# Fanchuana/OPUS-PLLM

Measured on AMD Instinct MI355X. Metric: proteins_per_sec, higher is better.
Workload: dtype f16; 1 GPU; OPUS-PLLM-llama3_8b shape: batch 64/GPU, 512-residue proteins, 89-id prompt (+8 protein tokens = 96 positions), 32 new tokens, greedy (BASELINE configs[3] per-GPU shard: batch 512 over 8 GPUs); batch_per_gpu=64, residues=512, parallelism=replicas x1 (batch-sharded), all-gather of ids

## Files before the change

include/opus_pllm.h:

```cpp
#ifndef OPUS_PLLM_H
#define OPUS_PLLM_H

#include <stdint.h>

#ifdef __cplusplus
extern "C" {
#endif

#define OPUS_ABI_VERSION 10

enum opus_status {
    OPUS_OK = 0,
    OPUS_EBADARG = -1,
    OPUS_ESHAPE = -2,
    OPUS_EHIP = -3,
    OPUS_ERCCL = -4,
    OPUS_EUNSUPPORTED = -5,
    OPUS_ESTATE = -6
};

enum opus_dtype { OPUS_F16 = 0, OPUS_F32 = 1, OPUS_I32 = 2, OPUS_I64 = 3, OPUS_U8 = 4, OPUS_F8E4M3 = 5, OPUS_I8 = 6,
                  OPUS_F4E2M1X2 = 7, OPUS_E8M0 = 8 };

typedef struct opus_config {
// ... 56 lines not shown

int opus_llama_forward(opus_ctx *ctx, const void *d_embeds, const uint8_t *d_mask, int32_t B, int32_t T, const int32_t *d_rows,
                       int32_t R, const int32_t *d_targets, float *d_logprob, void *d_logits, void *d_scratch,
                       int64_t scratch_bytes, void *stream);
int64_t opus_llama_forward_scratch_bytes(const opus_config *cfg, int32_t R, int32_t with_logits);
int opus_llama_prefix(opus_ctx *ctx, const void *d_embeds, const uint8_t *d_mask, int32_t B, int32_t T, float *d_last_logits,
                      float *d_last_rows, int64_t *epoch, void *stream);
int opus_llama_score_continuations(opus_ctx *ctx, const void *d_embeds, int32_t R, int32_t n, const int32_t *h_lens,
                                   const int32_t *h_src, const float *d_last_rows, int32_t P, int64_t epoch,
                                   const int32_t *d_targets, float *d_logprob, void *d_scratch, int64_t scratch_bytes, void *stream);
int64_t opus_llama_score_scratch_bytes(const opus_config *cfg, int32_t R, int32_t n);
int opus_debug_attn_prefix(opus_ctx *ctx, const void *d_qkv, const void *d_k_hist, const void *d_v_hist, const int32_t *d_kstart,
                           int32_t P, int32_t Tp, int32_t R, int32_t n, const int32_t *h_src, void *d_out, void *stream);
int opus_llama_score_tree(opus_ctx *ctx, const void *d_embeds, int32_t rows, const int32_t *h_src, const int32_t *h_par,
                          const int32_t *h_depth, int32_t n_score, const int32_t *h_score_src, int32_t n_edges,
                          const int32_t *h_edge_row, const int32_t *h_edge_tok, const int32_t *h_edge_slot, int32_t n_stops,
                          const int32_t *h_stop_row, const int32_t *h_stop_set, const int32_t *h_stop_slot, int32_t n_stop_ids,
                          const int32_t *h_stop_ids, int32_t n_stop_sets, const int32_t *h_stop_off, const float *d_last_rows,
                          int32_t P, int64_t epoch, float *d_node_lp, float *d_stop_lp, int64_t n_slots, void *d_scratch,
                          int64_t scratch_bytes, void *stream);
int64_t opus_llama_score_tree_scratch_bytes(const opus_config *cfg, int32_t rows, int32_t n_score, int32_t n_edges, int32_t n_stops,
                                            int32_t n_stop_ids, int32_t n_stop_sets);
int64_t opus_llama_dec_rows_cap(const opus_config *cfg);
int32_t opus_llama_tree_max_depth(void);
int opus_trie_path_sums(opus_ctx *ctx, const float *d_node_lp, const int32_t *d_trie, const int32_t *d_par, const int32_t *d_depth,
                        const int32_t *d_member_node, int32_t P, int32_t M, int32_t ld_nodes, float *d_member_lp, void *stream);
int opus_debug_attn_tree(opus_ctx *ctx, const void *d_qkv, const void *d_k_hist, const void *d_v_hist, const int32_t *d_kstart,
                         int32_t P, int32_t Tp, int32_t R, const int32_t *h_src, const int32_t *h_par, const int32_t *h_depth,
                         void *d_out, void *stream);
int opus_esm2_contacts_packed(opus_ctx *ctx, const int32_t *d_tokens, const int32_t *h_cu, int32_t B, float *d_pooled, float *d_contacts,
                              void *d_scratch, int64_t scratch_bytes, void *stream);
int64_t opus_esm2_contacts_scratch_bytes(const opus_config *cfg, const int32_t *h_cu, int32_t B);
int opus_esm2_lm_head(opus_ctx *ctx, const int32_t *d_rows, int32_t R, int32_t log_softmax, float *d_out, void *stream);
int opus_debug_esm2_lm_head(opus_ctx *ctx, const float *d_hidden, int32_t R, int32_t log_softmax, float *d_out, void *stream);
int opus_debug_contacts(opus_ctx *ctx, const void *d_q, const void *d_k, int64_t ld, const int32_t *h_cu, int32_t B, int32_t heads,
                        int32_t head_dim, const float *d_w, float *d_A, float *d_rows, float *d_cols, void *d_scratch,
                        int64_t scratch_bytes, void *stream);
int opus_debug_xent(opus_ctx *ctx, const void *d_logits, int32_t R, int32_t V, const int32_t *d_targets, float *d_logprob,
                    float *d_lse, void *stream);

int opus_generate_greedy(opus_ctx *ctx, const void *d_embeds, const uint8_t *d_mask, int32_t B, int32_t T,
                         int32_t max_new, const int32_t *eos_ids, int32_t n_eos, int32_t pad_id,
                         int32_t *d_out_ids, int32_t *n_out, void *stream);

int opus_set_stop_sequence(opus_ctx *ctx, const int32_t *ids, int32_t n);

int opus_generate_sample(opus_ctx *ctx, const void *d_embeds, const uint8_t *d_mask, int32_t B, int32_t T,
                         int32_t max_new, const int32_t *eos_ids, int32_t n_eos, int32_t pad_id, float temperature,
                         float top_p, uint64_t seed, int32_t *d_out_ids, int32_t *n_out, void *stream);
int opus_debug_sample(opus_ctx *ctx, const float *d_logits, int32_t B, float temperature, float top_p, uint64_t seed,
                      int32_t step, int32_t *d_tokens, void *stream);

int opus_generate_scored(opus_ctx *ctx, const void *d_embeds, const uint8_t *d_mask, int32_t B, int32_t T, int32_t max_new,
                         const int32_t *eos_ids, int32_t n_eos, int32_t pad_id, float temperature, float top_p, uint64_t seed,
                         int32_t *d_out_ids, int32_t *n_out, float *d_token_logprobs, float *d_scores, float *d_logits,
                         void *stream);
int opus_generate_scored_fanout(opus_ctx *ctx, const void *d_embeds, const uint8_t *d_mask, int32_t B, int32_t T, int32_t nret,
                                int32_t max_new, const int32_t *eos_ids, int32_t n_eos, int32_t pad_id, float temperature,
                                float top_p, uint64_t seed, int32_t *d_out_ids, int32_t *n_out, float *d_token_logprobs,
                                float *d_scores, float *d_logits, void *stream);

int opus_generate_scored_guided(opus_ctx *ctx, const void *d_embeds, const uint8_t *d_mask, int32_t P, int32_t T, float guidance_scale,
                                int32_t max_new, const int32_t *eos_ids, int32_t n_eos, int32_t pad_id, float temperature,
                                float top_p, uint64_t seed, int32_t *d_out_ids, int32_t *n_out, float *d_token_logprobs,
                                float *d_scores, float *d_logits, void *stream);

typedef struct opus_prefix_snap {
    const void *d_k, *d_v;
    const int32_t *d_kstart, *h_kstart;
    int32_t P, Tp;
} opus_prefix_snap;
int64_t opus_llama_prefix_bytes(const opus_config *cfg, int32_t P, int32_t Tp);
int opus_llama_prefix_export(opus_ctx *ctx, int64_t epoch, int32_t R, int32_t T, void *d_k, void *d_v, int32_t *d_kstart, void *stream);
int opus_llama_prefill_behind(opus_ctx *ctx, const opus_prefix_snap *snap, const void *d_embeds, int32_t R, int32_t n,
                              const int32_t *h_lens, const int32_t *h_src, float *d_last_logits, int64_t *epoch, void *stream);
int opus_generate_scored_behind(opus_ctx *ctx, const opus_prefix_snap *snap, const void *d_embeds, int32_t R, int32_t n,
                                const int32_t *h_lens, const int32_t *h_src, int32_t max_new, const int32_t *eos_ids, int32_t n_eos,
                                int32_t pad_id, float temperature, float top_p, uint64_t seed, int32_t *d_out_ids, int32_t *n_out,
                                float *d_token_logprobs, float *d_scores, float *d_logits, void *stream);
int opus_llama_score_continuations_detached(opus_ctx *ctx, const opus_prefix_snap *snap, const void *d_embeds, int32_t R, int32_t n,
                                            const int32_t *h_lens, const int32_t *h_src, const float *d_last_rows,
                                            const int32_t *d_targets, float *d_logprob, void *d_scratch, int64_t scratch_bytes,
                                            void *stream);
int opus_llama_score_tree_detached(opus_ctx *ctx, const opus_prefix_snap *snap, const void *d_embeds, int32_t rows,
                                   const int32_t *h_src, const int32_t *h_par, const int32_t *h_depth, int32_t n_score,
                                   const int32_t *h_score_src, int32_t n_edges, const int32_t *h_edge_row, const int32_t *h_edge_tok,
                                   const int32_t *h_edge_slot, int32_t n_stops, const int32_t *h_stop_row, const int32_t *h_stop_set,
                                   const int32_t *h_stop_slot, int32_t n_stop_ids, const int32_t *h_stop_ids, int32_t n_stop_sets,
                                   const int32_t *h_stop_off, const float *d_last_rows, float *d_node_lp, float *d_stop_lp,
                                   int64_t n_slots, void *d_scratch, int64_t scratch_bytes, void *stream);

int opus_generate_lookup(opus_ctx *ctx, const void *d_embeds, const uint8_t *d_mask, int32_t B, int32_t T, int32_t max_new,
                         const int32_t *eos_ids, int32_t n_eos, int32_t pad_id, int32_t k, int32_t max_ngram, const int32_t *d_hist,
                         int32_t Lh, const int32_t *h_hist_len, int32_t *d_out_ids, int32_t *n_out, int64_t *stats, void *stream);
int opus_llama_verify_step(opus_ctx *ctx, const int32_t *d_tokens, int32_t n, const int32_t *d_draft_len, float *d_logits_all,
                           int32_t *d_argmax, int32_t *a, void *stream);
int opus_debug_lookup_draft(opus_ctx *ctx, const int32_t *d_hist, int32_t Lh, const int32_t *d_hist_len, int32_t R, int32_t k,
                            int32_t max_ngram, int32_t *d_draft, int32_t *d_draft_len, void *stream);
int opus_debug_last_qkv(opus_ctx *ctx, void *d_out, int32_t rows, void *stream);
int opus_debug_lookup_accept(opus_ctx *ctx, const int32_t *d_argmax, const int32_t *d_tokens, const int32_t *d_draft_len, int32_t R,
                             int32_t n, int32_t pre, int32_t *d_ids, int32_t stride, int32_t *d_fin, int32_t *d_step,
                             const int32_t *eos_ids, int32_t n_eos, int32_t pad_id, const int32_t *stop_ids, int32_t n_stop,
                             int32_t *d_next, int32_t *d_nunf, int32_t *h_words, void *stream);

int opus_debug_argmax_lse(opus_ctx *ctx, const float *d_logits, int32_t B, int32_t V, int32_t *d_idx, float *d_lse, void *stream);
int opus_debug_guidance(opus_ctx *ctx, float *d_logits, int32_t P, int32_t V, float guidance_scale, void *stream);

int opus_set_logits_processors(opus_ctx *ctx, float repetition_penalty, int32_t no_repeat_ngram_size, int32_t min_new_tokens,
                               const int32_t *bad_ids, const int32_t *bad_offsets, int32_t n_bad);
int opus_debug_logits_process(opus_ctx *ctx, float *d_logits, int32_t B, int32_t V, const int32_t *d_hist, int32_t hist_stride,
                              int32_t hist_len, const int32_t *eos_ids, int32_t n_eos, float repetition_penalty,
                              int32_t no_repeat_ngram_size, int32_t min_new_tokens, const int32_t *bad_ids,
                              const int32_t *bad_offsets, int32_t n_bad, void *stream);

int opus_set_token_constraint(opus_ctx *ctx, int32_t n_states, const int32_t *edge_off, const int32_t *edge_tok,
                              const int32_t *edge_next, int32_t n_edges, const uint8_t *completing, const int32_t *end_ids,
                              int32_t n_end, const int32_t *start, int32_t n_start, void *stream);
int opus_debug_token_constraint(opus_ctx *ctx, float *d_logits, int32_t B, int32_t V, const int32_t *d_hist, int32_t hist_stride,
                                int32_t hist_len, int32_t *d_state_out, void *stream);

int opus_debug_gemm(opus_ctx *ctx, const void *d_A, const void *d_W, const float *d_bias, const float *d_residual,
                    void *d_C, int32_t M, int32_t N, int32_t K, int32_t epi, int32_t out_f32, void *stream);
int opus_debug_gemm_norm(opus_ctx *ctx, const float *d_A, const void *d_W, void *d_C, int32_t M, int32_t N, int32_t K,
                         int32_t epi, int32_t out_f32, float eps, void *stream);
int opus_debug_gemm_slabs(opus_ctx *ctx, const void *d_A, const void *d_W, float *d_slabs, int32_t M, int32_t N, int32_t K,
                          int32_t *ks, void *stream);
int opus_debug_gemm_plan(opus_ctx *ctx, int32_t *plan);
int opus_debug_gemm_w8(opus_ctx *ctx, int32_t form, const void *d_A, const void *d_W, const void *d_q8, const void *d_e8,
                       const float *d_bias, const float *d_residual, void *d_C, int32_t M, int32_t N, int32_t K, int32_t epi,
                       int32_t out_f32, float eps, int32_t *ks, int32_t *ran_w8, void *stream);
int opus_debug_gemm_w4(opus_ctx *ctx, int32_t form, const void *d_A, const void *d_W, const void *d_q4, const void *d_s4,
                       const float *d_bias, const float *d_residual, void *d_C, int32_t M, int32_t N, int32_t K, int32_t epi,
                       int32_t out_f32, float eps, int32_t *ks, int32_t *ran_w4, void *stream);
int opus_debug_knob(opus_ctx *ctx, const char *name, int32_t value);
int opus_debug_gemm_rowscale(opus_ctx *ctx, const void *d_A, const void *d_W1, float *d_X, const void *d_W2, void *d_C,
                             int32_t M, int32_t N1, int32_t K1, int32_t N2, int32_t epi, float eps, int32_t *fused,
                             void *stream);
int opus_debug_gemm_rope(opus_ctx *ctx, const void *d_A, const void *d_W, const float *d_bias, void *d_out, int32_t M,
                         int32_t D, int32_t K, int32_t T, int32_t heads, int32_t allow_fuse, int32_t *fused, void *stream);
int opus_debug_gemm_ln(opus_ctx *ctx, const void *d_A, const void *d_W1, const float *d_b1, float *d_X, float *d_part, void *d_xh,
                       float *d_stat, const void *d_W2, const float *d_c2, const float *d_colsum, void *d_C, int32_t M, int32_t N1,
                       int32_t K1, int32_t N2, int32_t epi, int32_t rms, float eps, int32_t rope_T, const int32_t *d_rope_pos,
                       int32_t *produced, int32_t *plan, void *stream);
int opus_debug_attention(opus_ctx *ctx, const void *d_Q, const void *d_K, const void *d_V, void *d_O,
                         const int32_t *d_kstart, const int32_t *d_kend, int32_t B, int32_t T, int32_t heads,
                         int32_t group, int32_t head_dim, int32_t causal, float scale, void *stream);

int opus_debug_attn_prefill(opus_ctx *ctx, const void *d_Q, const void *d_K, const void *d_V, void *d_O, int64_t q_st, int64_t k_st,
                            int64_t v_st, int64_t o_st, int64_t q_sb, int64_t k_sb, int64_t v_sb, int64_t o_sb,
                            const int32_t *d_kstart, const int32_t *d_kend, const int32_t *d_cu, int32_t B, int32_t T,
                            int32_t heads, int32_t group, int32_t head_dim, int32_t causal, int32_t q_trim, float scale,
                            int32_t *qt_used, void *stream);

int opus_debug_attn_decode(opus_ctx *ctx, const void *d_qkv, const void *d_k_hist, const void *d_v_hist, const int32_t *d_kstart,
                           int32_t B, int32_t T0, int32_t step, void *d_out, void *d_k_new, void *d_v_new, void *stream);

int opus_debug_attn_decode_form(opus_ctx *ctx, const void *d_qkv, const float *d_slabs, int32_t ks, const float *d_row_ssq,
                                int32_t row_nblk, int32_t K, float eps, const float *d_bias, const void *d_k_hist,
                                const void *d_v_hist, const int32_t *d_kstart, int32_t B, int32_t T0, int32_t step,
                                int32_t out_tiled, void *d_out, void *d_k_new, void *d_v_new, void *d_k_cache, void *d_v_cache,
                                int32_t *gp_used, void *stream);

int opus_check_error(opus_ctx *ctx, void *stream);

int opus_beam_topk(opus_ctx *ctx, const float *d_run_scores, int32_t B, int32_t K, int32_t M, float *d_scores, int32_t *d_idx,
                   void *stream);
int opus_kv_reorder(opus_ctx *ctx, const int32_t *d_src_rows, int32_t R, void *stream);
int opus_beam_sample_topk(opus_ctx *ctx, const float *d_logits, const float *d_run_scores, int32_t B, int32_t K, int32_t M,
                          float temperature, float top_p, uint64_t seed, int32_t step, float *d_scores, int32_t *d_idx, void *stream);
int opus_set_sampling_top_k(opus_ctx *ctx, int32_t k);

int32_t opus_stream_lag(void);
int opus_stream_begin(opus_ctx *ctx, const void *d_embeds, const uint8_t *d_mask, int32_t B, int32_t T, int32_t max_new,
                      const int32_t *eos_ids, int32_t n_eos, int32_t pad_id, float temperature, float top_p, uint64_t seed,
                      int32_t *d_ids, void *stream);
int opus_stream_run(opus_ctx *ctx, int32_t t_min, int32_t min_free, int32_t t_max, int32_t *t_out, int32_t *h_end, void *stream);
int opus_stream_refill(opus_ctx *ctx, const opus_prefix_snap *snap, int32_t n, const int32_t *h_rows, const int32_t *h_src,
                       const float *d_last_logits, const int32_t *h_len, void *stream);
int opus_stream_end(opus_ctx *ctx, int32_t *h_end, void *stream);
int opus_debug_stream_state(opus_ctx *ctx, int32_t *h_kstart, int32_t *h_fin, int32_t *h_start, int32_t *h_end, int64_t *epoch,
                            int32_t poison, void *stream);

int opus_last_logits(opus_ctx *ctx, float *d_out, int32_t B, void *stream);

int64_t opus_stat(opus_ctx *ctx, const char *name);

int opus_timing_enable(opus_ctx *ctx, int32_t on);
int opus_timing_reset(opus_ctx *ctx);
int opus_timing_get(opus_ctx *ctx, const char *kernel_class, const char *phase, double *ms, int64_t *launches, double *bytes,
                    double *flops);
int opus_timing_names(char *buf, int32_t cap);

#ifdef __cplusplus
}
#endif
#endif
```

opus-pllm_amd/_cabi.py:

```python
from __future__ import annotations

import ctypes as C
import os
from typing import Optional

from .config import OpusConfig

_HERE = os.path.dirname(os.path.abspath(__file__))
BF16 = os.environ.get("OPUS_DTYPE", "fp16").lower() in ("bf16", "bfloat16")
LIB_PATH = os.environ.get("OPUS_LIB_PATH") or os.path.join(_HERE, "lib", "libopus_pllm_bf16.so" if BF16 else "libopus_pllm.so")
ABI_VERSION = 10

OPUS_F16, OPUS_F32, OPUS_I32, OPUS_I64, OPUS_U8 = 0, 1, 2, 3, 4
OPUS_F8E4M3, OPUS_I8 = 5, 6
OPUS_F4E2M1X2, OPUS_E8M0 = 7, 8


def operand_dtype():
    import torch
    return torch.bfloat16 if BF16 else torch.float16


class OpusError(RuntimeError):
    def __init__(self, code: int, msg: str):
        super().__init__(f"libopus_pllm error {code}: {msg}")
        self.code = code


class CConfig(C.Structure):
    _fields_ = [
        ("enc_layers", C.c_int32), ("enc_dim", C.c_int32), ("enc_heads", C.c_int32), ("enc_ffn", C.c_int32),
        ("enc_vocab", C.c_int32), ("enc_ln_eps", C.c_float), ("enc_rope_theta", C.c_float),
        ("has_protein_projector", C.c_int32), ("proj_dim", C.c_int32), ("n_prot_tokens", C.c_int32),
        ("switch_depth", C.c_int32),
        ("dec_layers", C.c_int32), ("dec_dim", C.c_int32), ("dec_heads", C.c_int32), ("dec_kv_heads", C.c_int32),
        ("dec_head_dim", C.c_int32), ("dec_ffn", C.c_int32), ("dec_vocab", C.c_int32),
        ("dec_rms_eps", C.c_float), ("dec_rope_theta", C.c_float),
        ("max_batch", C.c_int32), ("max_enc_tokens", C.c_int32), ("max_prompt", C.c_int32),
        ("max_new_tokens", C.c_int32),
        ("dec_arch", C.c_int32), ("dec_qkv_bias", C.c_int32), ("dec_act", C.c_int32), ("dec_max_pos", C.c_int32),
    ]

    @classmethod
    def from_config(cls, cfg: OpusConfig) -> "CConfig":
        return cls(**{name: getattr(cfg, name) for name, _ in cls._fields_})


_P = C.c_void_p


class CPrefixSnap(C.Structure):
    _fields_ = [("d_k", _P), ("d_v", _P), ("d_kstart", _P), ("h_kstart", C.POINTER(C.c_int32)), ("P", C.c_int32), ("Tp", C.c_int32)]


_SNAP = C.POINTER(CPrefixSnap)
_I32P = C.POINTER(C.c_int32)
SIGNATURES = {
    "opus_llama_prefix_bytes": (C.c_int64, [C.POINTER(CConfig), C.c_int32, C.c_int32]),
    "opus_llama_prefix_export": (C.c_int, [_P, C.c_int64, C.c_int32, C.c_int32, _P, _P, _P, _P]),
    "opus_llama_prefill_behind": (C.c_int, [_P, _SNAP, _P, C.c_int32, C.c_int32, _I32P, _I32P, _P, C.POINTER(C.c_int64), _P]),
    "opus_generate_scored_behind": (C.c_int, [_P, _SNAP, _P, C.c_int32, C.c_int32, _I32P, _I32P, C.c_int32, _I32P, C.c_int32, C.c_int32,
                                              C.c_float, C.c_float, C.c_uint64, _P, _I32P, _P, _P, _P, _P]),
    "opus_llama_score_continuations_detached": (C.c_int, [_P, _SNAP, _P, C.c_int32, C.c_int32, _P, _P, _P, _P, _P, _P, C.c_int64, _P]),
    "opus_llama_score_tree_detached": (C.c_int, [_P, _SNAP, _P, C.c_int32, _P, _P, _P, C.c_int32, _P, C.c_int32, _P, _P, _P, C.c_int32, _P,
                                                 _P, _P, C.c_int32, _P, C.c_int32, _P, _P, _P, _P, C.c_int64, _P, C.c_int64, _P]),
    "opus_generate_lookup": (C.c_int, [_P, _P, _P, C.c_int32, C.c_int32, C.c_int32, _I32P, C.c_int32, C.c_int32, C.c_int32, C.c_int32, _P,
                                       C.c_int32, _I32P, _P, _I32P, C.POINTER(C.c_int64), _P]),
    "opus_llama_verify_step": (C.c_int, [_P, _P, C.c_int32, _P, _P, _P, _I32P, _P]),
    "opus_debug_last_qkv": (C.c_int, [_P, _P, C.c_int32, _P]),
    "opus_debug_lookup_draft": (C.c_int, [_P, _P, C.c_int32, _P, C.c_int32, C.c_int32, C.c_int32, _P, _P, _P]),
    "opus_debug_lookup_accept": (C.c_int, [_P, _P, _P, _P, C.c_int32, C.c_int32, C.c_int32, _P, C.c_int32, _P, _P, _I32P, C.c_int32,
                                           C.c_int32, _I32P, C.c_int32, _P, _P, _I32P, _P]),
    "opus_stream_lag": (C.c_int32, []),
    "opus_stream_begin": (C.c_int, [_P, _P, _P, C.c_int32, C.c_int32, C.c_int32, _I32P, C.c_int32, C.c_int32, C.c_float, C.c_float,
                                    C.c_uint64, _P, _P]),
    "opus_stream_run": (C.c_int, [_P, C.c_int32, C.c_int32, C.c_int32, _I32P, _I32P, _P]),
    "opus_stream_refill": (C.c_int, [_P, _SNAP, C.c_int32, _I32P, _I32P, _P, _I32P, _P]),
    "opus_stream_end": (C.c_int, [_P, _I32P, _P]),
    "opus_debug_stream_state": (C.c_int, [_P, _I32P, _I32P, _I32P, _I32P, C.POINTER(C.c_int64), C.c_int32, _P]),
    "opus_abi_version": (C.c_int, []),
    "opus_operand_dtype": (C.c_int, []),
    "opus_last_error": (C.c_char_p, []),
    "opus_workspace_bytes": (C.c_int64, [C.POINTER(CConfig)]),
    "opus_ctx_create": (C.c_int, [C.POINTER(CConfig), C.c_int, C.POINTER(_P)]),
    "opus_ctx_destroy": (C.c_int, [_P]),
    "opus_bind_weight": (C.c_int, [_P, C.c_char_p, _P, C.c_int, C.c_int, C.POINTER(C.c_int64)]),
    "opus_weights_ready": (C.c_int, [_P]),
    "opus_lora_merge": (C.c_int, [_P, _P, _P, C.c_float, C.c_int64, C.c_int64, C.c_int32, _P]),
    "opus_fill_synth": (C.c_int, [_P, C.c_int, C.c_int64, C.c_int64, C.c_uint64, C.c_float, C.c_float,
                                  C.c_int64, C.c_int64, C.c_int64, C.c_int32, C.c_uint64, C.c_float, C.c_float, _P]),
    "opus_tile_weight": (C.c_int, [_P, _P, C.c_int64, C.c_int64, _P]),
    "opus_quantize_fp8": (C.c_int, [_P, C.c_int64, C.c_int64, _P, _P, _P, _P]),
    "opus_debug_gemm_w8": (C.c_int, [_P, C.c_int32, _P, _P, _P, _P, _P, _P, _P, C.c_int32, C.c_int32, C.c_int32, C.c_int32, C.c_int32,
                                     C.c_float, C.POINTER(C.c_int32), C.POINTER(C.c_int32), _P]),
    "opus_quantize_mxfp4": (C.c_int, [_P, C.c_int64, C.c_int64, _P, _P, _P, _P]),
    "opus_debug_gemm_w4": (C.c_int, [_P, C.c_int32, _P, _P, _P, _P, _P, _P, _P, C.c_int32, C.c_int32, C.c_int32, C.c_int32, C.c_int32,
                                     C.c_float, C.POINTER(C.c_int32), C.POINTER(C.c_int32), _P]),
    "opus_esm2_encode": (C.c_int, [_P, _P, _P, C.c_int32, C.c_int32, _P, _P]),
    "opus_esm2_encode_packed": (C.c_int, [_P, _P, C.POINTER(C.c_int32), C.c_int32, _P, _P]),
    "opus_esm2_last_hidden": (C.c_int, [_P, _P, C.c_int32, C.c_int32, _P]),
    "opus_projector_forward": (C.c_int, [_P, _P, C.c_int32, _P, _P, _P]),
    "opus_protein_projector": (C.c_int, [_P, _P, C.c_int32, _P, _P]),
    "opus_switch_projector": (C.c_int, [_P, _P, C.c_int32, _P, _P]),
    "opus_splice_pad": (C.c_int, [_P, _P, _P, C.c_int32, C.c_int32, _P, C.c_int32, C.c_int32, C.c_int32,
                                  _P, _P, _P, C.POINTER(C.c_int32), _P]),
    "opus_llama_prefill": (C.c_int, [_P, _P, _P, C.c_int32, C.c_int32, _P, _P]),
    "opus_llama_decode_step": (C.c_int, [_P, _P, _P, _P]),
    "opus_generate_greedy": (C.c_int, [_P, _P, _P, C.c_int32, C.c_int32, C.c_int32, C.POINTER(C.c_int32),
                                       C.c_int32, C.c_int32, _P, C.POINTER(C.c_int32), _P]),
    "opus_debug_gemm": (C.c_int, [_P, _P, _P, _P, _P, _P, C.c_int32, C.c_int32, C.c_int32, C.c_int32, C.c_int32, _P]),
    "opus_debug_gemm_norm": (C.c_int, [_P, _P, _P, _P, C.c_int32, C.c_int32, C.c_int32, C.c_int32, C.c_int32, C.c_float, _P]),
    "opus_debug_gemm_rope": (C.c_int, [_P, _P, _P, _P, _P, C.c_int32, C.c_int32, C.c_int32, C.c_int32, C.c_int32, C.c_int32, _P, _P]),
    "opus_debug_attention": (C.c_int, [_P, _P, _P, _P, _P, _P, _P, C.c_int32, C.c_int32, C.c_int32, C.c_int32,
                                       C.c_int32, C.c_int32, C.c_float, _P]),
    "opus_debug_attn_prefill": (C.c_int, [_P, _P, _P, _P, _P, C.c_int64, C.c_int64, C.c_int64, C.c_int64, C.c_int64, C.c_int64,
                                          C.c_int64, C.c_int64, _P, _P, _P, C.c_int32, C.c_int32, C.c_int32, C.c_int32, C.c_int32,
                                          C.c_int32, C.c_int32, C.c_float, C.POINTER(C.c_int32), _P]),
    "opus_generate_sample": (C.c_int, [_P, _P, _P, C.c_int32, C.c_int32, C.c_int32, C.POINTER(C.c_int32), C.c_int32, C.c_int32,
                                       C.c_float, C.c_float, C.c_uint64, _P, C.POINTER(C.c_int32), _P]),
    "opus_debug_sample": (C.c_int, [_P, _P, C.c_int32, C.c_float, C.c_float, C.c_uint64, C.c_int32, _P, _P]),
    "opus_timing_enable": (C.c_int, [_P, C.c_int32]),
    "opus_timing_reset": (C.c_int, [_P]),
    "opus_timing_get": (C.c_int, [_P, C.c_char_p, C.c_char_p, C.POINTER(C.c_double), C.POINTER(C.c_int64),
                                  C.POINTER(C.c_double), C.POINTER(C.c_double)]),
    "opus_timing_names": (C.c_int, [C.c_char_p, C.c_int32]),
    "opus_last_logits": (C.c_int, [_P, _P, C.c_int32, _P]),
    "opus_check_error": (C.c_int, [_P, _P]),
    "opus_beam_topk": (C.c_int, [_P, _P, C.c_int32, C.c_int32, C.c_int32, _P, _P, _P]),
    "opus_kv_reorder": (C.c_int, [_P, _P, C.c_int32, _P]),
    "opus_beam_sample_topk": (C.c_int, [_P, _P, _P, C.c_int32, C.c_int32, C.c_int32, C.c_float, C.c_float, C.c_uint64, C.c_int32,
                                        _P, _P, _P]),
    "opus_set_sampling_top_k": (C.c_int, [_P, C.c_int32]),
    "opus_set_stop_sequence": (C.c_int, [_P, C.POINTER(C.c_int32), C.c_int32]),
    "opus_debug_gemm_slabs": (C.c_int, [_P, _P, _P, _P, C.c_int32, C.c_int32, C.c_int32, C.POINTER(C.c_int32), _P]),
    "opus_debug_gemm_plan": (C.c_int, [_P, C.POINTER(C.c_int32)]),
    "opus_debug_knob": (C.c_int, [_P, C.c_char_p, C.c_int32]),
    "opus_stat": (C.c_int64, [_P, C.c_char_p]),
    "opus_debug_attn_decode": (C.c_int, [_P, _P, _P, _P, _P, C.c_int32, C.c_int32, C.c_int32, _P, _P, _P, _P]),
    "opus_debug_attn_decode_form": (C.c_int, [_P, _P, _P, C.c_int32, _P, C.c_int32, C.c_int32, C.c_float, _P, _P, _P, _P, C.c_int32,
                                              C.c_int32, C.c_int32, C.c_int32, _P, _P, _P, _P, _P, C.POINTER(C.c_int32), _P]),
    "opus_llama_forward": (C.c_int, [_P, _P, _P, C.c_int32, C.c_int32, _P, C.c_int32, _P, _P, _P, _P, C.c_int64, _P]),
    "opus_llama_forward_scratch_bytes": (C.c_int64, [C.POINTER(CConfig), C.c_int32, C.c_int32]),
    "opus_llama_prefix": (C.c_int, [_P, _P, _P, C.c_int32, C.c_int32, _P, _P, C.POINTER(C.c_int64), _P]),
    "opus_llama_score_continuations": (C.c_int, [_P, _P, C.c_int32, C.c_int32, _P, _P, _P, C.c_int32, C.c_int64, _P, _P, _P,
                                                 C.c_int64, _P]),
    "opus_llama_score_scratch_bytes": (C.c_int64, [C.POINTER(CConfig), C.c_int32, C.c_int32]),
    "opus_debug_attn_prefix": (C.c_int, [_P, _P, _P, _P, _P, C.c_int32, C.c_int32, C.c_int32, C.c_int32, _P, _P, _P]),
    "opus_llama_score_tree": (C.c_int, [_P, _P, C.c_int32, _P, _P, _P, C.c_int32, _P, C.c_int32, _P, _P, _P, C.c_int32, _P, _P, _P,
                                        C.c_int32, _P, C.c_int32, _P, _P, C.c_int32, C.c_int64, _P, _P, C.c_int64, _P, C.c_int64, _P]),
    "opus_llama_score_tree_scratch_bytes": (C.c_int64, [C.POINTER(CConfig), C.c_int32, C.c_int32, C.c_int32, C.c_int32, C.c_int32,
                                                        C.c_int32]),
    "opus_llama_dec_rows_cap": (C.c_int64, [C.POINTER(CConfig)]),
    "opus_llama_tree_max_depth": (C.c_int32, []),
    "opus_trie_path_sums": (C.c_int, [_P, _P, _P, _P, _P, _P, C.c_int32, C.c_int32, C.c_int32, _P, _P]),
    "opus_debug_attn_tree": (C.c_int, [_P, _P, _P, _P, _P, C.c_int32, C.c_int32, C.c_int32, _P, _P, _P, _P, _P]),
    "opus_debug_xent": (C.c_int, [_P, _P, C.c_int32, C.c_int32, _P, _P, _P, _P]),
    "opus_esm2_contacts_packed": (C.c_int, [_P, _P, C.POINTER(C.c_int32), C.c_int32, _P, _P, _P, C.c_int64, _P]),
    "opus_esm2_contacts_scratch_bytes": (C.c_int64, [C.POINTER(CConfig), C.POINTER(C.c_int32), C.c_int32]),
    "opus_debug_contacts": (C.c_int, [_P, _P, _P, C.c_int64, C.POINTER(C.c_int32), C.c_int32, C.c_int32, C.c_int32, _P, _P, _P, _P,
                                      _P, C.c_int64, _P]),
    "opus_esm2_lm_head": (C.c_int, [_P, _P, C.c_int32, C.c_int32, _P, _P]),
    "opus_debug_esm2_lm_head": (C.c_int, [_P, _P, C.c_int32, C.c_int32, _P, _P]),
    "opus_generate_scored": (C.c_int, [_P, _P, _P, C.c_int32, C.c_int32, C.c_int32, C.POINTER(C.c_int32), C.c_int32, C.c_int32,
                                       C.c_float, C.c_float, C.c_uint64, _P, C.POINTER(C.c_int32), _P, _P, _P, _P]),
    "opus_llama_prefill_fanout": (C.c_int, [_P, _P, _P, C.c_int32, C.c_int32, C.c_int32, _P, _P]),
    "opus_generate_scored_fanout": (C.c_int, [_P, _P, _P, C.c_int32, C.c_int32, C.c_int32, C.c_int32, C.POINTER(C.c_int32), C.c_int32,
                                              C.c_int32, C.c_float, C.c_float, C.c_uint64, _P, C.POINTER(C.c_int32), _P, _P, _P, _P]),
    "opus_debug_argmax_lse": (C.c_int, [_P, _P, C.c_int32, C.c_int32, _P, _P, _P]),
    "opus_generate_scored_guided": (C.c_int, [_P, _P, _P, C.c_int32, C.c_int32, C.c_float, C.c_int32, C.POINTER(C.c_int32), C.c_int32,
                                              C.c_int32, C.c_float, C.c_float, C.c_uint64, _P, C.POINTER(C.c_int32), _P, _P, _P, _P]),
    "opus_debug_guidance": (C.c_int, [_P, _P, C.c_int32, C.c_int32, C.c_float, _P]),
    "opus_set_logits_processors": (C.c_int, [_P, C.c_float, C.c_int32, C.c_int32, C.POINTER(C.c_int32), C.POINTER(C.c_int32),
                                             C.c_int32]),
    "opus_debug_logits_process": (C.c_int, [_P, _P, C.c_int32, C.c_int32, _P, C.c_int32, C.c_int32, C.POINTER(C.c_int32), C.c_int32,
                                            C.c_float, C.c_int32, C.c_int32, C.POINTER(C.c_int32), C.POINTER(C.c_int32), C.c_int32,
                                            _P]),
    "opus_set_token_constraint": (C.c_int, [_P, C.c_int32, _P, _P, _P, C.c_int32, _P, _P, C.c_int32, _P, C.c_int32, _P]),
    "opus_debug_token_constraint": (C.c_int, [_P, _P, C.c_int32, C.c_int32, _P, C.c_int32, C.c_int32, _P, _P]),
    "opus_debug_gemm_rowscale": (C.c_int, [_P, _P, _P, _P, _P, _P, C.c_int32, C.c_int32, C.c_int32, C.c_int32, C.c_int32,
                                           C.c_float, C.POINTER(C.c_int32), _P]),
    "opus_debug_gemm_ln": (C.c_int, [_P, _P, _P, _P, _P, _P, _P, _P, _P, _P, _P, _P, C.c_int32, C.c_int32, C.c_int32, C.c_int32,
                                     C.c_int32, C.c_int32, C.c_float, C.c_int32, _P, C.POINTER(C.c_int32), C.POINTER(C.c_int32), _P]),
}

_lib: Optional[C.CDLL] = None


def lib() -> C.CDLL:
    global _lib
    if _lib is not None:
        return _lib
    if not os.path.exists(LIB_PATH):
        raise OpusError(-100, f"{LIB_PATH} not found: build it with `python opus-pllm_amd/build.py` "
                              "(hipcc --offload-arch=gfx950); this package has no CPU fallback")
    l = C.CDLL(LIB_PATH)
    for name, (res, args) in SIGNATURES.items():
        fn = getattr(l, name)
        fn.restype = res
        fn.argtypes = args
    v = l.opus_abi_version()
    if v != ABI_VERSION:
        raise OpusError(-101, f"ABI version mismatch: library {v}, binding {ABI_VERSION}")
    if l.opus_operand_dtype() != (1 if BF16 else 0):
        raise OpusError(-102, f"{LIB_PATH} was not built for {'bf16' if BF16 else 'fp16'} operands")
    _lib = l
    return l


def check(code: int) -> None:
    if code != 0:
        raise OpusError(code, lib().opus_last_error().decode("utf-8", "replace"))
```

opus-pllm_amd/build.py:

```python
from __future__ import annotations

import concurrent.futures as cf
import os
import re
import subprocess
import sys

HERE = os.path.dirname(os.path.abspath(__file__))
SRC = os.path.join(HERE, "csrc")
OBJ = os.path.join(HERE, "build")
LIB = os.path.join(HERE, "lib", "libopus_pllm.so")
LIB_BF16 = os.path.join(HERE, "lib", "libopus_pllm_bf16.so")
SOURCES = ["gemm.hip", "gemm_stream.hip", "norm.hip", "elementwise.hip", "attn_prefill.hip", "attn_prefix.hip", "kv_place.hip", "stream.hip", "attn_decode.hip", "beam.hip", "score.hip", "contact.hip", "mlm.hip", "logits_proc.hip", "constraint.hip", "guidance.hip", "quant.hip", "lookup.hip", "api.cpp"]
HIPCC = os.environ.get("HIPCC", "/opt/rocm/bin/hipcc")
FLAGS = ["--offload-arch=gfx950", "-O3", "-fPIC", "-std=c++17", "-Wall", "-Wno-unused-function",
         "-Wno-unused-variable", "-Wno-unused-but-set-variable"]
EXTRA = {"attn_prefill.hip": ["-mllvm", "-amdgpu-mfma-vgpr-form", "-fno-honor-nans"],
         "attn_prefix.hip": ["-mllvm", "-amdgpu-mfma-vgpr-form", "-fno-honor-nans"],
         "attn_decode.hip": ["-mllvm", "-amdgpu-mfma-vgpr-form"]}


NO_SCRATCH = ("gemm_pp_kernel", "gemm_stream_kernel", "gemm_wide_kernel", "gemm_skinny_kernel", "attn_prefill_kernel",
              "attn_decode_kernel", "attn_prefix_kernel", "tree_path_sums_kernel", "beam_", "kv_export_kernel", "kv_place_kernel",
              "kv_append_kernel", "guidance_", "stream_finish_kernel", "stream_refill_kernel", "stream_reset_kernel")
RU_FLAG = "-Rpass-analysis=kernel-resource-usage"


def resource_usage(text: str) -> dict:
    out, cur = {}, None
    for line in text.splitlines():
        m = re.search(r"remark: Function Name: (\S+)", line)
        if m:
            cur = out.setdefault(m.group(1), {})
            continue
        m = re.search(r"remark:\s+([\w \[\]/]+?): (-?\d+)", line)
        if m and cur is not None:
            cur[m.group(1).strip()] = int(m.group(2))
    return out


def check_resources(ru_file: str) -> None:
    bad = []
    for name, f in resource_usage(open(ru_file).read()).items():
        if any(k in name for k in NO_SCRATCH) and (f.get("ScratchSize [bytes/lane]", 0) or f.get("VGPRs Spill", 0) or f.get("SGPRs Spill", 0)):
            bad.append(f"{name}: VGPRs {f.get('VGPRs')}, scratch {f.get('ScratchSize [bytes/lane]')} B/lane, "
                       f"spilled VGPRs {f.get('VGPRs Spill')}, spilled SGPRs {f.get('SGPRs Spill')}")
    if bad:
        raise RuntimeError(f"{os.path.basename(ru_file)}: hot kernels must not spill:\n  " + "\n  ".join(bad))


def sources_sha16() -> str:
    import hashlib
    h = hashlib.sha256()
    files = sorted(os.path.join(SRC, f) for f in os.listdir(SRC) if f.endswith((".hip", ".cpp", ".h")))
    files.append(os.path.join(os.path.dirname(HERE), "include", "opus_pllm.h"))
    for f in files:
        h.update(os.path.basename(f).encode() + b"\0")
        h.update(open(f, "rb").read())
    return h.hexdigest()[:16]


def _deps_mtime() -> float:
    hdrs = [os.path.join(SRC, f) for f in os.listdir(SRC) if f.endswith(".h")]
    hdrs.append(os.path.join(os.path.dirname(HERE), "include", "opus_pllm.h"))
    return max(os.path.getmtime(h) for h in hdrs)


def _compile(src: str, force: bool, bf16: bool = False) -> str:
    obj = os.path.join(OBJ, src + (".bf16.o" if bf16 else ".o"))
    path = os.path.join(SRC, src)
    ru = obj + ".ru.txt"
    if not force and os.path.exists(obj) and os.path.exists(ru) and \
            os.path.getmtime(obj) > max(os.path.getmtime(path), _deps_mtime(), os.path.getmtime(os.path.abspath(__file__))):
        check_resources(ru)
        return obj
    cmd = [HIPCC] + FLAGS + [RU_FLAG] + EXTRA.get(src, []) + (["-DOPUS_BF16"] if bf16 else []) + \
          (["-x", "hip"] if src.endswith(".cpp") else []) + ["-c", path, "-o", obj]
    r = subprocess.run(cmd, capture_output=True, text=True)
    if r.returncode != 0:
        raise RuntimeError(f"hipcc failed on {src}:\n{r.stdout}\n{r.stderr}")
    remarks = [l for l in r.stderr.splitlines() if RU_FLAG in l]
    rest = "\n".join(l for l in r.stderr.splitlines() if RU_FLAG not in l)
    with open(ru, "w") as f:
        f.write("\n".join(remarks) + "\n")
    if rest.strip():
        sys.stderr.write(rest + "\n")
    check_resources(ru)
    return obj


def build(force: bool = False, verbose: bool = True) -> str:
    os.makedirs(OBJ, exist_ok=True)
    os.makedirs(os.path.dirname(LIB), exist_ok=True)
    jobs = [(s, b) for b in (False, True) for s in SOURCES]
    with cf.ThreadPoolExecutor(max_workers=6) as ex:
        objs = list(ex.map(lambda j: _compile(j[0], force, j[1]), jobs))
    for lib, mine in ((LIB, objs[:len(SOURCES)]), (LIB_BF16, objs[len(SOURCES):])):
        if force or not os.path.exists(lib) or any(os.path.getmtime(o) > os.path.getmtime(lib) for o in mine):
            r = subprocess.run([HIPCC, "--offload-arch=gfx950", "-shared", "-fPIC", "-o", lib] + mine, capture_output=True, text=True)
            if r.returncode != 0:
                raise RuntimeError(f"link failed:\n{r.stdout}\n{r.stderr}")
        if verbose:
            print(f"built {lib} ({os.path.getsize(lib) / 1e6:.2f} MB)")
    return LIB


LIB_ASAN = os.path.join(HERE, "lib", "libopus_pllm_asan.so")
ASAN_RT = "/opt/rocm/lib/llvm/lib/clang/22/lib/linux/libclang_rt.asan-x86_64.so"


def build_asan(verbose: bool = True) -> str:
    build(verbose=False)
    obj = os.path.join(OBJ, "api.cpp.asan.o")
    src = os.path.join(SRC, "api.cpp")
    if not os.path.exists(obj) or os.path.getmtime(obj) < max(os.path.getmtime(src), _deps_mtime()):
        cmd = [HIPCC, "--offload-arch=gfx950", "-O1", "-g", "-fPIC", "-std=c++17", "-fsanitize=address", "-fno-gpu-sanitize",
               "-shared-libsan", "-fno-omit-frame-pointer", "-x", "hip", "-c", src, "-o", obj]
        r = subprocess.run(cmd, capture_output=True, text=True)
        if r.returncode != 0:
            raise RuntimeError(f"hipcc (asan) failed on api.cpp:\n{r.stdout}\n{r.stderr}")
    objs = [os.path.join(OBJ, s + ".o") for s in SOURCES if s != "api.cpp"] + [obj]
    if not os.path.exists(LIB_ASAN) or any(os.path.getmtime(o) > os.path.getmtime(LIB_ASAN) for o in objs):
        r = subprocess.run([HIPCC, "--offload-arch=gfx950", "-shared", "-fPIC", "-fsanitize=address", "-fno-gpu-sanitize",
                            "-shared-libsan", "-o", LIB_ASAN] + objs, capture_output=True, text=True)
        if r.returncode != 0:
            raise RuntimeError(f"link (asan) failed:\n{r.stdout}\n{r.stderr}")
    if verbose:
        print(f"built {LIB_ASAN} ({os.path.getsize(LIB_ASAN) / 1e6:.2f} MB); run under LD_PRELOAD={ASAN_RT}")
    return LIB_ASAN


if __name__ == "__main__":
    if "--asan" in sys.argv:
        build_asan()
    else:
        build(force="--force" in sys.argv)
```

opus-pllm_amd/csrc/api.cpp:

```cpp
#include "../../include/opus_pllm.h"
#include "common.h"

#include <cmath>
#include <cstdarg>
#include <cstdio>
#include <cstdlib>
#include <cstring>
#include <algorithm>
#include <atomic>
#include <map>
#include <string>
#include <vector>

using namespace opus;

static thread_local char g_err[512] = "";
static int fail(int code, const char *fmt, ...) {
    va_list ap;
    va_start(ap, fmt);
    vsnprintf(g_err, sizeof(g_err), fmt, ap);
    va_end(ap);
    return code;
}
#define HIPC(expr)                                                                                   \
// ... 1069 lines not shown
}

static int switch_projector_rows(opus_ctx *c, hipStream_t s, const half_t *in, int B, half_t *d_out) {
    const opus_config &g = c->cfg;
    const int SW = g.dec_dim * g.n_prot_tokens;
    int din = g.has_protein_projector ? g.proj_dim : g.enc_dim;
    for (int i = 0; i < g.switch_depth; ++i) {
        const bool last = i + 1 == g.switch_depth;
        half_t *o = last ? d_out : c->p_z[i & 1];
        OPC(gemm(c, s, in, din, c->sw_w[i], B, SW, din, c->sw_b[i], last ? EPI_NONE : EPI_GELU, nullptr, o, SW, 0));
        in = o;
        din = SW;
    }
    return OPUS_OK;
}

extern "C" int opus_protein_projector(opus_ctx *c, const float *d_pooled, int32_t B, void *d_out, void *stream) {
    OPC(need_ready(c));
    if (!d_pooled || !d_out) return fail(OPUS_EBADARG, "protein_projector: null pointer");
    if (B < 1) return fail(OPUS_ESHAPE, "protein_projector: B=%d", B);
    const opus_config &g = c->cfg;
    const int64_t din = g.enc_dim, dout = g.has_protein_projector ? g.proj_dim : g.enc_dim;
    c->phase = PH_PROJECT;
    OPC(ensure_proj_rows(c, B));
    for (int r0 = 0; r0 < B; r0 += c->proj_rows) {
        const int n = B - r0 < c->proj_rows ? B - r0 : c->proj_rows;
        OPC(protein_projector_rows(c, (hipStream_t)stream, d_pooled + r0 * din, n, (half_t *)d_out + r0 * dout));
    }
    return OPUS_OK;
}

extern "C" int opus_switch_projector(opus_ctx *c, const void *d_in, int32_t B, void *d_out, void *stream) {
    OPC(need_ready(c));
    if (!d_in || !d_out) return fail(OPUS_EBADARG, "switch_projector: null pointer");
    if (B < 1) return fail(OPUS_ESHAPE, "switch_projector: B=%d", B);
    const opus_config &g = c->cfg;
    const int64_t din = g.has_protein_projector ? g.proj_dim : g.enc_dim, SW = (int64_t)g.dec_dim * g.n_prot_tokens;
    c->phase = PH_PROJECT;
    OPC(ensure_proj_rows(c, B));
    for (int r0 = 0; r0 < B; r0 += c->proj_rows) {
        const int n = B - r0 < c->proj_rows ? B - r0 : c->proj_rows;
        OPC(switch_projector_rows(c, (hipStream_t)stream, (const half_t *)d_in + r0 * din, n, (half_t *)d_out + r0 * SW));
    }
    return OPUS_OK;
}

extern "C" int opus_projector_forward(opus_ctx *c, const float *d_pooled, int32_t B, void *d_out, void *d_proj_out,
                                      void *stream) {
    OPC(need_ready(c));
    if (!d_pooled || !d_out) return fail(OPUS_EBADARG, "projector_forward: null pointer");
    if (B < 1) return fail(OPUS_ESHAPE, "projector_forward: B=%d", B);
    const opus_config &g = c->cfg;
    hipStream_t s = (hipStream_t)stream;
    const int64_t din = g.enc_dim, dmid = g.has_protein_projector ? g.proj_dim : g.enc_dim, SW = (int64_t)g.dec_dim * g.n_prot_tokens;
    c->phase = PH_PROJECT;
    OPC(ensure_proj_rows(c, B));
    for (int r0 = 0; r0 < B; r0 += c->proj_rows) {
        const int n = B - r0 < c->proj_rows ? B - r0 : c->proj_rows;
        OPC(protein_projector_rows(c, s, d_pooled + r0 * din, n, c->p_y));
        if (d_proj_out)
            HIPC(hipMemcpyAsync((half_t *)d_proj_out + r0 * dmid, c->p_y, (size_t)n * dmid * sizeof(half_t), hipMemcpyDeviceToDevice, s));
        OPC(switch_projector_rows(c, s, c->p_y, n, (half_t *)d_out + r0 * SW));
    }
    return OPUS_OK;
}

extern "C" int opus_splice_pad(opus_ctx *c, const int64_t *d_ids, const uint8_t *d_mask, int32_t B, int32_t Tt,
                               const void *d_prot, int32_t n_prot, int32_t inference_mode, int32_t max_length,
                               void *d_embeds, uint8_t *d_mask_out, int32_t *d_pos_out, int32_t *T_out, void *stream) {
    OPC(need_ready(c));
    if (!d_ids || !d_prot || !d_embeds || !d_mask_out || !d_pos_out || !T_out) return fail(OPUS_EBADARG, "splice_pad: null pointer");
    const opus_config &g = c->cfg;
    if (B < 1 || B > g.max_batch || Tt < 1) return fail(OPUS_ESHAPE, "splice_pad: B=%d T_text=%d out of range", B, Tt);
    hipStream_t s = (hipStream_t)stream;
    c->phase = PH_SPLICE;
    KL(KC_OTHER, 9.0 * B * Tt, launch_splice_plan(d_ids, d_mask, B, Tt, g.n_prot_tokens, max_length, g.dec_vocab, c->d_plan, s));
    int32_t tail[3];
    HIPC(hipMemcpyAsync(tail, c->d_plan + 4 * B, sizeof(tail), hipMemcpyDeviceToHost, s));
    HIPC(hipStreamSynchronize(s));
    if (tail[2]) return fail(OPUS_EBADARG, "splice_pad: token id outside [0, vocab) (and not -200)");
    if (tail[1] > n_prot) return fail(OPUS_ESHAPE, "splice_pad: rows consume %d protein blocks, %d supplied", tail[1], n_prot);
    if (tail[0] > g.max_prompt) return fail(OPUS_ESHAPE, "splice_pad: spliced length %d exceeds max_prompt=%d", tail[0], g.max_prompt);
    if (tail[0] < 1) return fail(OPUS_ESHAPE, "splice_pad: every row is empty");
    *T_out = tail[0];
    KL(KC_OTHER, 2.0 * B * tail[0] * g.dec_dim * 2,
       launch_splice_fill(d_ids, d_mask, B, Tt, (const half_t *)d_prot, g.n_prot_tokens, g.dec_dim, g.dec_vocab, c->dec_emb,
                          c->d_plan, tail[0], inference_mode ? 1 : 0, (half_t *)d_embeds, d_mask_out, d_pos_out, s));
    return OPUS_OK;
}

static int lm_head(opus_ctx *c, hipStream_t s, ResidShadow &sh, int B, float *out = nullptr) {
    const opus_config &g = c->cfg;
    return gemm_norm(c, s, sh, c->d_xl, g.dec_rms_eps, c->d_xln, c->lm_head, B, g.dec_vocab, g.dec_dim, EPI_NONE, out ? out : c->d_logits,
                     g.dec_vocab, 1);
}

static int fanout_rows(opus_ctx *c, hipStream_t s, int B, int nret) {
    const opus_config &g = c->cfg;
    KL(KC_OTHER, 4.0 * (B + B * nret) * g.dec_vocab, launch_row_fanout(c->d_probs, c->d_logits, g.dec_vocab, B, nret, c->d_kstart, s));
    return OPUS_OK;
}


static int reset_step(opus_ctx *c, hipStream_t s, int T0, int step = 0) {
    const int32_t v[2] = {step, T0};
    HIPC(launch_upload_i32(v, 2, c->d_step, s));
    return OPUS_OK;
}

template <class Head>
static int finish_prefill(opus_ctx *c, hipStream_t s, int B, int T, int nret, bool have_last, Head head) {
    const int H = c->cfg.dec_dim;
    if (!have_last) KL(KC_OTHER, 8.0 * B * H, launch_take_last(c->d_x, B, T, H, c->d_xl, s));
    OPC(head(nret > 1 ? c->d_probs : nullptr));
    if (nret > 1) OPC(fanout_rows(c, s, B, nret));
    OPC(reset_step(c, s, T));
    c->cur_B = B * nret;
    c->cur_T = T;
    c->prefilled = true;
    return OPUS_OK;
}

static int attn_decode(opus_ctx *c, hipStream_t s, const ResidShadow &sh, int l, int B, int T, int slab_ks = 0, const float *bias = nullptr,
                       int out_tiled = 0) {
    const opus_config &g = c->cfg;
    AttnDecodeParams a;
    a.qkv = c->d_qkv; a.slabs = nullptr; a.ks = 0; a.slab_stride = 0; a.row_ssq = nullptr; a.row_nblk = 0; a.eps = 0.f; a.K = 0;
    a.bias = nullptr;
    if (slab_ks > 0) {
        const int64_t QKVd = (int64_t)(g.dec_heads + 2 * g.dec_kv_heads) * g.dec_head_dim;
        a.qkv = nullptr; a.slabs = c->gemm_ws; a.ks = slab_ks; a.slab_stride = (int64_t)B * QKVd;
        a.row_ssq = c->d_ssq; a.row_nblk = sh.ssq_nblk; a.eps = g.dec_rms_eps; a.K = g.dec_dim; a.bias = bias;
    }
    a.cs_row = c->cs_row; a.kstart = c->d_kstart; a.step = c->d_step; a.T0 = -1; a.nh = g.dec_heads; a.nkv = g.dec_kv_heads;
    a.kc = c->kc + l * c->cache_sl; a.vc = c->vc + l * c->cache_sl; a.cache_sb = c->cache_sb; a.cache_sh = c->cache_sh;
    a.ctx_cap = g.max_prompt + g.max_new_tokens; a.scale = 1.0f / sqrtf((float)g.dec_head_dim); a.out = c->d_ctx;
    a.out_tiled = out_tiled;
    const double bytes = 4.0 * B * g.dec_kv_heads * g.dec_head_dim * (T + 1) + 2.0 * B * (2.0 * g.dec_heads + 2.0 * g.dec_kv_heads) * g.dec_head_dim;
    KL(KC_ATTN_DECODE, bytes, launch_attn_decode(a, B, g.dec_head_dim, s));
    return OPUS_OK;
}

static int attn_prefix(opus_ctx *c, hipStream_t s, const ContRows &cr, int l, int M) {
    const opus_config &g = c->cfg;
    AttnPrefixParams a = cr.attn;
    a.kc = cr.snap_k ? cr.snap_k + l * cr.snap_sl : c->kc + l * c->cache_sl;
    a.vc = cr.snap_v ? cr.snap_v + l * cr.snap_sl : c->vc + l * c->cache_sl;
    const int QKV = (g.dec_heads + 2 * g.dec_kv_heads) * g.dec_head_dim, QD = g.dec_heads * g.dec_head_dim;
    KLF(KC_ATTN_PREFILL, 2.0 * M * (QKV + QD) + 4.0 * cr.nblocks * g.dec_kv_heads * g.dec_head_dim * a.Tp,
        4.0 * M * (double)QD * (a.Tp + a.n), launch_attn_prefix(a, cr.nblocks, s));
    return OPUS_OK;
}

static int attn_prefill(opus_ctx *c, hipStream_t s, int l, int B, int T, const ContRows *cont, int nret) {
    const opus_config &g = c->cfg;
    const int nh = g.dec_heads, nkv = g.dec_kv_heads, hd = g.dec_head_dim, QKV = (nh + 2 * nkv) * hd, QD = nh * hd, M = B * T;
    if (cont) {
        KL(KC_OTHER, 4.0 * M * QKV, launch_dec_rope_cache(c->d_qkv, c->cs_dec, cont->nkst, B, T, nh, nkv, hd, nullptr, nullptr, 0, 0, s));
        if (cont->app_lens)
            KL(KC_OTHER, 8.0 * M * nkv * hd, launch_kv_append(c->d_qkv, cont->app_lens, B, T, nh, nkv, hd, cont->attn.Tp, c->kc + l * c->cache_sl,
                                                              c->vc + l * c->cache_sl, c->cache_sb, c->cache_sh, s));
        return attn_prefix(c, s, *cont, l, M);
    }
    KL(KC_OTHER, 4.0 * M * QKV,
       launch_dec_rope_cache(c->d_qkv, c->cs_dec, c->d_kstart, B, T, nh, nkv, hd, c->kc + l * c->cache_sl,
                             c->vc + l * c->cache_sl, c->cache_sb, c->cache_sh, s, nret));
    AttnParams a;
    a.Q = c->d_qkv; a.K = c->d_qkv + QD; a.V = c->d_qkv + QD + nkv * hd;
    a.q_sb = a.k_sb = a.v_sb = (int64_t)T * QKV;
    a.q_st = a.k_st = a.v_st = QKV;
    a.O = c->d_ctx; a.o_sb = (int64_t)T * QD; a.o_st = QD;
    a.kstart = c->d_kstart; a.kend = nullptr;
    a.B = B; a.T = T; a.heads = nh; a.group = nh / nkv; a.head_dim = hd; a.causal = 1;
    a.scale = 1.0f / sqrtf((float)hd);
    KLF(KC_ATTN_PREFILL, 2.0 * M * (QKV + QD), 2.0 * B * (double)T * T * QD, launch_attn_prefill(a, s));
    return OPUS_OK;
}

static int opt_layer(opus_ctx *c, hipStream_t s, const DecLayer &L, int l, float *x, half_t *xn, int M, int B, int T, bool decode,
                     const ContRows *cont = nullptr, int nret = 1) {
    const opus_config &g = c->cfg;
    const int H = g.dec_dim, F = g.dec_ffn;
    const int QKV = (g.dec_heads + 2 * g.dec_kv_heads) * g.dec_head_dim, QD = g.dec_heads * g.dec_head_dim;
    KL(KC_NORM, 6.0 * M * H, launch_layernorm(x, L.ln1w, L.ln1b, g.dec_rms_eps, M, H, xn, nullptr, s));
    OPC(gemm(c, s, xn, H, L.wqkv, M, QKV, H, L.bqkv, EPI_NONE, nullptr, c->d_qkv, QKV, 0));
    if (decode) OPC(attn_decode(c, s, ResidShadow(), l, B, T));
    else OPC(attn_prefill(c, s, l, B, T, cont, nret));
    OPC(gemm(c, s, c->d_ctx, QD, L.wo, M, H, QD, L.bo, EPI_NONE, x, x, H, 1));
    KL(KC_NORM, 6.0 * M * H, launch_layernorm(x, L.ln2w, L.ln2b, g.dec_rms_eps, M, H, xn, nullptr, s));
    if (g.dec_act == 0) {
        OPC(gemm(c, s, xn, H, L.w1, M, F, H, L.b1, EPI_GELU, nullptr, c->d_act, F, 0));
    } else {
        OPC(gemm(c, s, xn, H, L.w1, M, F, H, L.b1, EPI_NONE, nullptr, c->d_act, F, 0));
        KL(KC_OTHER, 4.0 * M * F, launch_relu_h(c->d_act, (int64_t)M * F, s));
    }
    OPC(gemm(c, s, c->d_act, F, L.w2, M, H, F, L.b2, EPI_NONE, x, x, H, 1));
    return OPUS_OK;
}

static int lm_head_opt(opus_ctx *c, hipStream_t s, int B, float *out = nullptr) {
    const opus_config &g = c->cfg;
    KL(KC_NORM, 6.0 * B * g.dec_dim, launch_layernorm(c->d_xl, c->dec_lnfw, c->dec_lnfb, g.dec_rms_eps, B, g.dec_dim, c->d_xln, nullptr, s));
    return gemm(c, s, c->d_xln, g.dec_dim, c->lm_head, B, g.dec_vocab, g.dec_dim, nullptr, EPI_NONE, nullptr, out ? out : c->d_logits,
                g.dec_vocab, 1);
}

static int prefill_opt(opus_ctx *c, hipStream_t s, const half_t *embeds, const uint8_t *mask, int B, int T, bool all_rows,
                       const ContRows *cont, int nret) {
    const opus_config &g = c->cfg;
    const int H = g.dec_dim, M = B * T;
    HIPC(hipMemsetAsync(c->d_cnt, 0, HANDOFF_ERR * sizeof(int32_t), s));
    if (!cont) KL(KC_OTHER, 1.0 * M, launch_mask_to_kstart(mask, B, T, c->d_kstart, s));
    KL(KC_OTHER, 6.0 * M * H, launch_h2f(embeds, c->d_x, (int64_t)M * H, s));
    KL(KC_OTHER, 10.0 * M * H, launch_add_pos(c->d_x, c->dec_pos, cont ? cont->nkst : c->d_kstart, nullptr, 0, B, T, H, g.dec_max_pos + 1, s));
    for (int l = 0; l < g.dec_layers; ++l) OPC(opt_layer(c, s, c->dec[l], l, c->d_x, c->d_xn, M, B, T, false, cont, nret));
    if (all_rows) return OPUS_OK;
    return finish_prefill(c, s, B, T, nret, false, [&](float *out) { return lm_head_opt(c, s, B, out); });
}

static int decode_step_opt(opus_ctx *c, hipStream_t s) {
    const opus_config &g = c->cfg;
    const int B = c->cur_B, T = c->cur_T, H = g.dec_dim;
    KL(KC_OTHER, 10.0 * B * H, launch_add_pos(c->d_xl, c->dec_pos, c->d_kstart, c->d_step, -1, B, 1, H, g.dec_max_pos + 1, s));
    for (int l = 0; l < g.dec_layers; ++l) OPC(opt_layer(c, s, c->dec[l], l, c->d_xl, c->d_xln, B, B, T, true));
    OPC(lm_head_opt(c, s, B));
    KL(KC_OTHER, 8.0, launch_step_advance(c->d_step, s));
    return OPUS_OK;
}

static int prefill(opus_ctx *c, hipStream_t s, const half_t *embeds, const uint8_t *mask, int B, int T, bool all_rows = false,
                   const ContRows *cont = nullptr, int nret = 1) {
    c->phase = cont && !cont->app_lens ? PH_SCORE : PH_PREFILL;
    if (cont && cont->w8) c->phase = PH_DECODE;
    if (cont) {
        all_rows = true;
    } else {
        new_epoch(c);
        if (all_rows) {
            c->prefilled = false;
            c->cur_B = 0;
        }
    }
    if (c->cfg.dec_arch == 1) return prefill_opt(c, s, embeds, mask, B, T, all_rows, cont, nret);
    const opus_config &g = c->cfg;
    const int H = g.dec_dim, F = g.dec_ffn, nh = g.dec_heads, nkv = g.dec_kv_heads, hd = g.dec_head_dim;
    const int QKV = (nh + 2 * nkv) * hd, QD = nh * hd;
    const int M = B * T;
    HIPC(hipMemsetAsync(c->d_cnt, 0, HANDOFF_ERR * sizeof(int32_t), s));
    if (!cont) KL(KC_OTHER, 1.0 * M, launch_mask_to_kstart(mask, B, T, c->d_kstart, s));
    KL(KC_OTHER, 6.0 * M * H, launch_h2f(embeds, c->d_x, (int64_t)M * H, s));
    static const bool no_ln_env = getenv("OPUS_NO_LN_FUSION") != nullptr;
    const bool no_ln_fusion = no_ln_env || g_knobs.no_ln_fusion;
    const bool qkv_pp = !no_ln_fusion && (H & 255) == 0 && (QKV & 255) == 0 && gemm_goes_pp(M, QKV);
    const bool gu_pp = !no_ln_fusion && (H & 255) == 0 && (F & 127) == 0 && gemm_goes_pp(M, 2 * F);
    bool have_stat = false, last_rows_done = false;
    auto finalize = [&]() -> int {
        KL(KC_NORM, 8.0 * M * (H / 64) + 8.0 * M, launch_ln_finalize(c->d_part, M, H / 64, H, g.dec_rms_eps, 1, c->d_stat, s));
        return OPUS_OK;
    };
    ResidShadow sh;
    GemmGot got;
    const bool w8 = cont && cont->w8;
    auto ask8 = [&](GemmAsk a, const uint8_t *q, const int8_t *e, const uint8_t *q4, const uint8_t *s4) { return w8 ? a.w8(q, e).w4(q4, s4) : a; };
    for (int l = 0; l < g.dec_layers; ++l) {
        const DecLayer &L = c->dec[l];
        if (have_stat && qkv_pp) {
            OPC(gemm(c, s, c->d_xn, H, L.wqkv, M, QKV, H, L.bqkv, EPI_NONE, nullptr, c->d_qkv, QKV, 0, GemmAsk().ln_consume(c->d_stat, nullptr)));
        } else {
            OPC(gemm_norm(c, s, sh, c->d_x, g.dec_rms_eps, c->d_xn, L.wqkv, M, QKV, H, EPI_NONE, c->d_qkv, QKV, 0, L.bqkv,
                          ask8(GemmAsk(), L.q8_qkv, L.e8_qkv, L.q4_qkv, L.s4_qkv)));
        }
        OPC(attn_prefill(c, s, l, B, T, cont, nret));
        if (l + 1 == g.dec_layers && T > 1 && !all_rows && !g_knobs.misc[7]) {
            half_t *ctx_last = c->d_qkv;
            KL(KC_OTHER, 4.0 * B * QD, launch_take_last(reinterpret_cast<const float *>(c->d_ctx), B, T, QD / 2, reinterpret_cast<float *>(ctx_last), s));
            KL(KC_OTHER, 8.0 * B * H, launch_take_last(c->d_x, B, T, H, c->d_xl, s));
            const GemmAsk copy_xl = GemmAsk().copy16(fuse_rows() && B <= 96 ? c->d_xln : nullptr);
            OPC(gemm(c, s, ctx_last, QD, L.wo, B, H, QD, nullptr, EPI_NONE, c->d_xl, c->d_xl, H, 1, copy_xl, &got));
            sh.produced(c->d_xl, got);
            OPC(gemm_norm(c, s, sh, c->d_xl, g.dec_rms_eps, c->d_xln, L.wgu, B, 2 * F, H, EPI_SILU_GU16, c->d_act, F, 0));
            OPC(gemm(c, s, c->d_act, F, L.wd, B, H, F, nullptr, EPI_NONE, c->d_xl, c->d_xl, H, 1, copy_xl, &got));
            sh.produced(c->d_xl, got);
            last_rows_done = true;
            break;
        }
        GemmAsk wo;
        if (gu_pp) wo.ln_produce(c->d_part, c->d_xn);
        else if (fuse_rows() && M <= 96) wo.copy16(c->d_xn);
        OPC(gemm(c, s, c->d_ctx, QD, L.wo, M, H, QD, nullptr, EPI_NONE, c->d_x, c->d_x, H, 1, ask8(wo, L.q8_o, L.e8_o, L.q4_o, L.s4_o), &got));
        sh.produced(c->d_x, got);
        have_stat = got.ln_done != 0;
        if (have_stat) {
            OPC(finalize());
            OPC(gemm(c, s, c->d_xn, H, L.wgu, M, 2 * F, H, nullptr, EPI_SILU_GU16, nullptr, c->d_act, F, 0, GemmAsk().ln_consume(c->d_stat, nullptr)));
        } else {
            OPC(gemm_norm(c, s, sh, c->d_x, g.dec_rms_eps, c->d_xn, L.wgu, M, 2 * F, H, EPI_SILU_GU16, c->d_act, F, 0, nullptr,
                          ask8(GemmAsk(), L.q8_gu, L.e8_gu, L.q4_gu, L.s4_gu)));
        }
        const bool next_pp = qkv_pp && l + 1 < g.dec_layers;
        OPC(gemm(c, s, c->d_act, F, L.wd, M, H, F, nullptr, EPI_NONE, c->d_x, c->d_x, H, 1, ask8(GemmAsk().ln_produce(next_pp ? c->d_part : nullptr, c->d_xn), L.q8_d, L.e8_d, L.q4_d, L.s4_d), &got));
        have_stat = got.ln_done != 0;
        if (have_stat) OPC(finalize());
    }
    if (all_rows) return OPUS_OK;
    return finish_prefill(c, s, B, T, nret, last_rows_done, [&](float *out) { return lm_head(c, s, sh, B, out); });
}

static int decode_step(opus_ctx *c, hipStream_t s, const int32_t *d_tok) {
    c->phase = PH_DECODE;
    const opus_config &g = c->cfg;
    const int B = c->cur_B, T = c->cur_T;
    const int H = g.dec_dim, F = g.dec_ffn, nh = g.dec_heads, nkv = g.dec_kv_heads, hd = g.dec_head_dim;
    const int QKV = (nh + 2 * nkv) * hd, QD = nh * hd;
    const int ctx_cap = g.max_prompt + g.max_new_tokens;
    const bool rowscale = g.dec_arch == 0 && fuse_rows() && B > SKINNY_MAX_M && B <= MID_MAX_M && (H & 255) == 0;
    const bool qkv_tiled = rowscale && gemm_stream_would(B, QKV, H, 1, 1, 1, c->gemm_ws_bytes);
    const bool wo_tiled = rowscale && gemm_stream_would(B, H, QD, 0, 1, 0, c->gemm_ws_bytes);
    const bool down_tiled = rowscale && (F & 63) == 0 && gemm_stream_would(B, H, F, 0, 1, 0, c->gemm_ws_bytes);
    KL(KC_OTHER, 6.0 * B * H, launch_embed_tokens(d_tok, c->dec_emb, B, H, g.dec_vocab, c->d_xl, rowscale ? c->d_xln : nullptr,
                                                  rowscale ? c->d_ssq : nullptr, qkv_tiled ? 1 : 0, c->cs_dec, c->d_kstart, c->d_step, -1,
                                                  hd / 2, c->cs_row, c->d_cnt, HANDOFF_ERR, s));
    if (g.dec_arch == 1) return decode_step_opt(c, s);
    ResidShadow sh;
    if (rowscale) { sh.xh_src = c->d_xl; sh.ssq_nblk = H >> 8; sh.xln_tiled = qkv_tiled; }
    GemmGot got;
    half_t *const copy_xl = fuse_rows() && B <= 96 ? c->d_xln : nullptr;
    for (int l = 0; l < g.dec_layers; ++l) {
        const DecLayer &L = c->dec[l];
        if (rowscale && sh.xh_src == c->d_xl) {
// ... 1894 lines not shown
        if (got.ks > 1 && Cp)
            HIPC(hipMemcpyAsync(Cp, c->gemm_ws, (size_t)got.ks * M * N * sizeof(float), hipMemcpyDeviceToDevice, s));
    }
    *ran_w8 = *ran;
    return OPUS_OK;
}
extern "C" int opus_debug_gemm_w8(opus_ctx *c, int32_t form, const void *A, const void *W, const void *q8, const void *e8,
                                  const float *bias, const float *residual, void *Cp, int32_t M, int32_t N, int32_t K, int32_t epi,
                                  int32_t out_f32, float eps, int32_t *ks, int32_t *ran_w8, void *stream) {
    if (!c || !A || !W || !q8 || !e8 || !ran_w8) return fail(OPUS_EBADARG, "debug_gemm_w8: null pointer");
    if (form < 0 || form > 2) return fail(OPUS_EBADARG, "debug_gemm_w8: form 0, 1 or 2");
    if ((((uintptr_t)q8) & 15) || (((uintptr_t)e8) & 3)) return fail(OPUS_EBADARG, "debug_gemm_w8: d_q8 must be 16-byte, d_e8 4-byte aligned");
    return debug_gemm_wq(c, form, A, W, GemmAsk().w8((const uint8_t *)q8, (const int8_t *)e8), &c->gemm_w8, bias, residual, Cp, M, N, K,
                         epi, out_f32, eps, ks, ran_w8, stream);
}
extern "C" int opus_debug_gemm_w4(opus_ctx *c, int32_t form, const void *A, const void *W, const void *q4, const void *s4,
                                  const float *bias, const float *residual, void *Cp, int32_t M, int32_t N, int32_t K, int32_t epi,
                                  int32_t out_f32, float eps, int32_t *ks, int32_t *ran_w4, void *stream) {
    if (!c || !A || !W || !q4 || !s4 || !ran_w4) return fail(OPUS_EBADARG, "debug_gemm_w4: null pointer");
    if (form < 0 || form > 2) return fail(OPUS_EBADARG, "debug_gemm_w4: form 0, 1 or 2");
    if ((((uintptr_t)q4) & 15) || (((uintptr_t)s4) & 15)) return fail(OPUS_EBADARG, "debug_gemm_w4: d_q4 and d_s4 must be 16-byte aligned");
    return debug_gemm_wq(c, form, A, W, GemmAsk().w4((const uint8_t *)q4, (const uint8_t *)s4), &c->gemm_w4, bias, residual, Cp, M, N, K,
                         epi, out_f32, eps, ks, ran_w4, stream);
}

extern "C" int opus_debug_gemm_plan(opus_ctx *c, int32_t *plan) {
    if (!c || !plan) return fail(OPUS_EBADARG, "debug_gemm_plan: null pointer");
    for (int i = 0; i < GEMM_PLAN_WORDS; ++i) plan[i] = c->gemm_plan[i];
    return OPUS_OK;
}

extern "C" int opus_beam_topk(opus_ctx *c, const float *d_run_scores, int32_t B, int32_t K, int32_t M, float *d_scores,
                              int32_t *d_idx, void *stream) {
    if (!c || !d_run_scores || !d_scores || !d_idx) return fail(OPUS_EBADARG, "beam_topk: null pointer");
    if (!c->prefilled) return fail(OPUS_ESTATE, "beam_topk before prefill");
    if (B < 1 || K < 1 || B * K != c->cur_B) return fail(OPUS_ESHAPE, "beam_topk: B=%d x K=%d rows, the last step had %d", B, K, c->cur_B);
    if (M < 1 || M > 16) return fail(OPUS_ESHAPE, "beam_topk: 1 <= M <= 16 candidates per row (got %d)", M);
    HIPC(hipSetDevice(c->device));
    hipStream_t s = (hipStream_t)stream;
    c->phase = PH_DECODE;
    KL(KC_OTHER, 12.0 * c->cur_B * c->cfg.dec_vocab,
       launch_beam_topk(c->d_logits, d_run_scores, B, K, c->cfg.dec_vocab, M, c->d_zpart, d_scores, d_idx, s));
    return OPUS_OK;
}

extern "C" int opus_beam_sample_topk(opus_ctx *c, const float *d_logits, const float *d_run_scores, int32_t B, int32_t K, int32_t M,
                                     float temperature, float top_p, uint64_t seed, int32_t step, float *d_scores, int32_t *d_idx,
                                     void *stream) {
    if (!c || !d_run_scores || !d_scores || !d_idx) return fail(OPUS_EBADARG, "beam_sample_topk: null pointer");
    if (!d_logits && !c->prefilled) return fail(OPUS_ESTATE, "beam_sample_topk before prefill");
    if (B < 1 || K < 1 || B * K > c->cfg.max_batch || (!d_logits && B * K != c->cur_B))
        return fail(OPUS_ESHAPE, "beam_sample_topk: B=%d x K=%d rows (the last step had %d, the context holds %d)", B, K, c->cur_B, c->cfg.max_batch);
    if (M < 1 || M > 16) return fail(OPUS_ESHAPE, "beam_sample_topk: 1 <= M <= 16 candidates per row (got %d)", M);
    if (!(temperature > 0.f) || top_p <= 0.f || top_p > 1.f) return fail(OPUS_EBADARG, "beam_sample_topk: temperature > 0, 0 < top_p <= 1");
    HIPC(hipSetDevice(c->device));
    hipStream_t s = (hipStream_t)stream;
    const float *lg = d_logits ? d_logits : c->d_logits;
    const int V = c->cfg.dec_vocab, R = B * K;
    c->phase = PH_DECODE;
    const int min_keep = M / K > 1 ? M / K : 1;
    const int top_k = c->samp_top_k > 0 && c->samp_top_k < min_keep ? min_keep : c->samp_top_k;
    KL(KC_OTHER, 4.0 * 4 * R * V,
       launch_sample_select(lg, R, V, temperature, top_p, top_k, nullptr, nullptr, c->d_pval, c->d_pidx, c->d_probs, c->d_cand_i,
                            c->d_cand_n, c->d_zpart, c->d_spart, nullptr, c->d_bthr, nullptr, nullptr, s));
    KL(KC_OTHER, 12.0 * R * V,
       launch_beam_sample(lg, d_run_scores, B, K, V, M, temperature, c->d_pval, c->d_bthr, min_keep, c->d_probs, c->d_cand_i, seed, step,
                          c->d_blse, d_scores, d_idx, s));
    return OPUS_OK;
}

extern "C" int opus_set_sampling_top_k(opus_ctx *c, int32_t k) {
    if (!c || k < 0) return fail(OPUS_EBADARG, "set_sampling_top_k: k >= 0");
    if (k != c->samp_top_k) drop_graphs(c);
    c->samp_top_k = k;
    return OPUS_OK;
}

extern "C" int opus_kv_reorder(opus_ctx *c, const int32_t *d_src_rows, int32_t R, void *stream) {
    if (!c || !d_src_rows) return fail(OPUS_EBADARG, "kv_reorder: null pointer");
    if (!c->prefilled || R != c->cur_B) return fail(OPUS_ESHAPE, "kv_reorder: R=%d but the last prefill had %d rows", R, c->prefilled ? c->cur_B : 0);
    HIPC(hipSetDevice(c->device));
    hipStream_t s = (hipStream_t)stream;
    const opus_config &g = c->cfg;
    const size_t row = (size_t)c->cache_sb, layer = row * g.max_batch;
    if (!c->kv_tmp) HIPC(hipMalloc((void **)&c->kv_tmp, 2 * layer * sizeof(half_t)));
    c->phase = PH_DECODE;
    new_epoch(c);
    const int nkv = g.dec_kv_heads, hd = g.dec_head_dim, T0 = c->cur_T;
    for (int l = 0; l < g.dec_layers; ++l) {
        half_t *kc = c->kc + l * c->cache_sl, *vc = c->vc + l * c->cache_sl;
        KL(KC_OTHER, 8.0 * R * nkv * hd * T0, launch_kv_gather_rows(kc, c->kv_tmp, d_src_rows, R, (int64_t)row, nkv, c->cache_sh, c->d_step, T0, hd, 0, s));
        HIPC(launch_kv_gather_rows(vc, c->kv_tmp + layer, d_src_rows, R, (int64_t)row, nkv, c->cache_sh, c->d_step, T0, hd, 0, s));
        HIPC(launch_kv_gather_rows(kc, c->kv_tmp, d_src_rows, R, (int64_t)row, nkv, c->cache_sh, c->d_step, T0, hd, 1, s));
        HIPC(launch_kv_gather_rows(vc, c->kv_tmp + layer, d_src_rows, R, (int64_t)row, nkv, c->cache_sh, c->d_step, T0, hd, 1, s));
    }
    return OPUS_OK;
}

extern "C" int opus_last_logits(opus_ctx *c, float *d_out, int32_t B, void *stream) {
    if (!c || !d_out) return fail(OPUS_EBADARG, "last_logits: null pointer");
    if (!c->prefilled) return fail(OPUS_ESTATE, "last_logits before prefill");
    if (B < 1 || B > c->cur_B) return fail(OPUS_ESHAPE, "last_logits: B=%d but the last prefill had %d rows", B, c->cur_B);
    HIPC(hipSetDevice(c->device));
    HIPC(hipMemcpyAsync(d_out, c->d_logits, (size_t)B * c->cfg.dec_vocab * sizeof(float), hipMemcpyDeviceToDevice, (hipStream_t)stream));
    return OPUS_OK;
}

extern "C" int opus_debug_attention(opus_ctx *c, const void *Q, const void *K, const void *V, void *O,
                                    const int32_t *kstart, const int32_t *kend, int32_t B, int32_t T, int32_t heads,
                                    int32_t group, int32_t hd, int32_t causal, float scale, void *stream) {
    if (!c || !Q || !K || !V || !O) return fail(OPUS_EBADARG, "debug_attention: null pointer");
    if (B < 1 || T < 1 || heads < 1 || group < 1 || heads % group) return fail(OPUS_ESHAPE, "debug_attention: shape");
    HIPC(hipSetDevice(c->device));
    hipStream_t s = (hipStream_t)stream;
    AttnParams a;
    const int kvh = heads / group;
    a.Q = (const half_t *)Q; a.K = (const half_t *)K; a.V = (const half_t *)V; a.O = (half_t *)O;
    a.q_st = (int64_t)heads * hd; a.q_sb = a.q_st * T;
    a.k_st = a.v_st = (int64_t)kvh * hd; a.k_sb = a.v_sb = a.k_st * T;
    a.o_st = a.q_st; a.o_sb = a.q_sb;
    a.kstart = kstart; a.kend = kend; a.B = B; a.T = T; a.heads = heads; a.group = group; a.head_dim = hd;
    a.causal = causal; a.scale = scale;
    KLF(KC_ATTN_PREFILL, 2.0 * B * T * hd * (2.0 * heads + 2.0 * kvh), (causal ? 2.0 : 4.0) * B * (double)T * T * heads * hd,
        launch_attn_prefill(a, s));
    return OPUS_OK;
}

extern "C" int opus_debug_attn_prefill(opus_ctx *c, const void *Q, const void *K, const void *V, void *O, int64_t q_st, int64_t k_st,
                                       int64_t v_st, int64_t o_st, int64_t q_sb, int64_t k_sb, int64_t v_sb, int64_t o_sb,
                                       const int32_t *kstart, const int32_t *kend, const int32_t *cu, int32_t B, int32_t T,
                                       int32_t heads, int32_t group, int32_t hd, int32_t causal, int32_t q_trim, float scale,
                                       int32_t *qt_used, void *stream) {
    if (qt_used) *qt_used = 0;
    if (!c || !Q || !K || !V || !O || !qt_used) return fail(OPUS_EBADARG, "debug_attn_prefill: null pointer");
    if (B < 1 || T < 1 || heads < 1 || group < 1 || heads % group || hd < 1) return fail(OPUS_ESHAPE, "debug_attn_prefill: shape");
    if (q_st < 1 || k_st < 1 || v_st < 1 || o_st < 1) return fail(OPUS_ESHAPE, "debug_attn_prefill: token strides must be positive");
    if (causal && cu) return fail(OPUS_EUNSUPPORTED, "debug_attn_prefill: no causal token-packed form");
    if (q_trim && (!cu || T <= 2)) return fail(OPUS_ESHAPE, "debug_attn_prefill: q_trim needs cu and T > 2");
    HIPC(hipSetDevice(c->device));
    hipStream_t s = (hipStream_t)stream;
    AttnParams a;
    a.Q = (const half_t *)Q; a.K = (const half_t *)K; a.V = (const half_t *)V; a.O = (half_t *)O;
    a.q_st = q_st; a.k_st = k_st; a.v_st = v_st; a.o_st = o_st;
    a.q_sb = cu ? 0 : q_sb; a.k_sb = cu ? 0 : k_sb; a.v_sb = cu ? 0 : v_sb; a.o_sb = cu ? 0 : o_sb;
    a.kstart = kstart; a.kend = kend; a.cu = cu; a.q_trim = q_trim ? 1 : 0;
    a.B = B; a.T = T; a.heads = heads; a.group = group; a.head_dim = hd; a.causal = causal ? 1 : 0; a.scale = scale;
    const int kvh = heads / group;
    KLF(KC_ATTN_PREFILL, 2.0 * B * T * hd * (2.0 * heads + 2.0 * kvh), (causal ? 2.0 : 4.0) * B * (double)T * T * heads * hd,
        launch_attn_prefill(a, s));
    *qt_used = attn_prefill_query_tiles(a);
    return OPUS_OK;
}

struct DecodeForm {
    const void *qkv = nullptr;
    const float *slabs = nullptr, *row_ssq = nullptr, *bias = nullptr;
    int ks = 0, row_nblk = 0, K = 0, out_tiled = 0;
    float eps = 0.f;
    void *k_cache = nullptr, *v_cache = nullptr;
    int32_t *gp_used = nullptr;
};
static int debug_attn_decode_check(opus_ctx *c, const char *who, const void *d_k_hist, const void *d_v_hist, int B, int T0, int step) {
    const opus_config &g = c->cfg;
    if (B < 1 || B > g.max_batch || T0 < 1 || T0 > g.max_prompt || step < 0 || step >= g.max_new_tokens)
        return fail(OPUS_ESHAPE, "%s: B=%d T0=%d step=%d exceed the context (%d, %d, %d)", who, B, T0, step, g.max_batch,
                    g.max_prompt, g.max_new_tokens);
    if (T0 + step > 0 && (!d_k_hist || !d_v_hist)) return fail(OPUS_EBADARG, "%s: history is null", who);
    return OPUS_OK;
}
static int debug_attn_decode_launch(opus_ctx *c, const DecodeForm &f, const void *d_k_hist, const void *d_v_hist, const int32_t *d_kstart,
                                    int B, int T0, int step, void *d_out, void *d_k_new, void *d_v_new, void *stream) {
    const opus_config &g = c->cfg;
    const int L = T0 + step, nkv = g.dec_kv_heads, hd = g.dec_head_dim, ctx_cap = g.max_prompt + g.max_new_tokens;
    HIPC(hipSetDevice(c->device));
    hipStream_t s = (hipStream_t)stream;
    const size_t pitch = (size_t)c->cache_sh * sizeof(half_t);
    OPC(seed_cache(c, s, d_k_hist, d_v_hist, d_kstart, B, L));
    OPC(reset_step(c, s, T0, step));
    HIPC(launch_embed_tokens(c->d_next, nullptr, B, 0, 1, c->d_xl, nullptr, nullptr, 0, c->cs_dec, c->d_kstart, c->d_step, -1, hd / 2,
                             c->cs_row, nullptr, 0, s));
    AttnDecodeParams a;
    a.qkv = (const half_t *)f.qkv; a.slabs = nullptr; a.ks = 0; a.slab_stride = 0; a.row_ssq = nullptr; a.row_nblk = 0; a.eps = 0.f; a.K = 0;
    a.bias = nullptr;
    if (f.slabs) {
        a.qkv = nullptr; a.slabs = f.slabs; a.ks = f.ks; a.slab_stride = (int64_t)B * (g.dec_heads + 2 * nkv) * hd;
        a.row_ssq = f.row_ssq; a.row_nblk = f.row_nblk; a.eps = f.eps; a.K = f.K; a.bias = f.bias;
    }
    a.cs_row = c->cs_row; a.kstart = c->d_kstart; a.step = c->d_step; a.T0 = -1; a.nh = g.dec_heads; a.nkv = nkv;
    a.kc = c->kc; a.vc = c->vc; a.cache_sb = c->cache_sb; a.cache_sh = c->cache_sh;
    a.ctx_cap = ctx_cap; a.scale = 1.0f / sqrtf((float)hd); a.out = (half_t *)d_out; a.out_tiled = f.out_tiled;
    c->phase = PH_DECODE;
    KL(KC_ATTN_DECODE, 4.0 * B * nkv * hd * (L + 1), launch_attn_decode(a, B, hd, s));
    if (f.gp_used) *f.gp_used = attn_decode_group(B, g.dec_heads, nkv);
    const size_t one = (size_t)hd * sizeof(half_t);
    if (d_k_new) HIPC(hipMemcpy2DAsync(d_k_new, one, c->kc + (size_t)L * hd, pitch, one, (size_t)B * nkv, hipMemcpyDeviceToDevice, s));
    if (d_v_new) HIPC(hipMemcpy2DAsync(d_v_new, one, c->vc + (size_t)L * hd, pitch, one, (size_t)B * nkv, hipMemcpyDeviceToDevice, s));
    const size_t all = (size_t)ctx_cap * hd * sizeof(half_t);
    if (f.k_cache) HIPC(hipMemcpy2DAsync(f.k_cache, all, c->kc, pitch, all, (size_t)B * nkv, hipMemcpyDeviceToDevice, s));
    if (f.v_cache) HIPC(hipMemcpy2DAsync(f.v_cache, all, c->vc, pitch, all, (size_t)B * nkv, hipMemcpyDeviceToDevice, s));
    c->prefilled = false;
    new_epoch(c);
    return OPUS_OK;
}

extern "C" int opus_debug_attn_decode(opus_ctx *c, const void *d_qkv, const void *d_k_hist, const void *d_v_hist,
                                      const int32_t *d_kstart, int32_t B, int32_t T0, int32_t step, void *d_out, void *d_k_new,
                                      void *d_v_new, void *stream) {
    if (!c || !d_qkv || !d_kstart || !d_out) return fail(OPUS_EBADARG, "debug_attn_decode: null pointer");
    OPC(debug_attn_decode_check(c, "debug_attn_decode", d_k_hist, d_v_hist, B, T0, step));
    DecodeForm f;
    f.qkv = d_qkv;
    return debug_attn_decode_launch(c, f, d_k_hist, d_v_hist, d_kstart, B, T0, step, d_out, d_k_new, d_v_new, stream);
}

extern "C" int opus_debug_attn_decode_form(opus_ctx *c, const void *d_qkv, const float *d_slabs, int32_t ks, const float *d_row_ssq,
                                           int32_t row_nblk, int32_t K, float eps, const float *d_bias, const void *d_k_hist,
                                           const void *d_v_hist, const int32_t *d_kstart, int32_t B, int32_t T0, int32_t step,
                                           int32_t out_tiled, void *d_out, void *d_k_new, void *d_v_new, void *d_k_cache,
                                           void *d_v_cache, int32_t *gp_used, void *stream) {
    if (gp_used) *gp_used = 0;
    if (!c || !d_kstart || !d_out || !gp_used) return fail(OPUS_EBADARG, "debug_attn_decode_form: null pointer");
    if ((d_qkv != nullptr) == (d_slabs != nullptr))
        return fail(OPUS_EBADARG, "debug_attn_decode_form: exactly one of d_qkv and d_slabs must be given");
    OPC(debug_attn_decode_check(c, "debug_attn_decode_form", d_k_hist, d_v_hist, B, T0, step));
    if (d_slabs) {
        if (ks < 1 || ks > 8) return fail(OPUS_ESHAPE, "debug_attn_decode_form: ks=%d outside 1 .. 8", ks);
        if (row_nblk < 1 || K < 1) return fail(OPUS_ESHAPE, "debug_attn_decode_form: row_nblk=%d K=%d must be positive", row_nblk, K);
        if (!d_row_ssq) return fail(OPUS_ESHAPE, "debug_attn_decode_form: slabs come with the rows' sums of squares (d_row_ssq)");
    }
    if (out_tiled && (int64_t)c->cfg.dec_heads * c->cfg.dec_head_dim % 64)
        return fail(OPUS_ESHAPE, "debug_attn_decode_form: out_tiled needs heads * head_dim = %d to be a multiple of 64",
                    c->cfg.dec_heads * c->cfg.dec_head_dim);
    DecodeForm f;
    f.qkv = d_qkv; f.slabs = d_slabs; f.row_ssq = d_row_ssq; f.bias = d_slabs ? d_bias : nullptr;
    f.ks = ks; f.row_nblk = row_nblk; f.K = K; f.eps = eps; f.out_tiled = out_tiled ? 1 : 0;
    f.k_cache = d_k_cache; f.v_cache = d_v_cache; f.gp_used = gp_used;
    return debug_attn_decode_launch(c, f, d_k_hist, d_v_hist, d_kstart, B, T0, step, d_out, d_k_new, d_v_new, stream);
}

extern "C" int opus_debug_knob(opus_ctx *c, const char *name, int32_t value) {
    if (!name) return fail(OPUS_EBADARG, "debug_knob: null name");
    if (c) drop_graphs(c);
    if (!strcmp(name, "no_stream")) g_knobs.no_stream = value;
    else if (!strcmp(name, "debug_a_tiled")) g_knobs.debug_a_tiled = value;
    else if (!strcmp(name, "no_ln_fusion")) g_knobs.no_ln_fusion = value;
    else if (!strcmp(name, "enc_full_last_layer")) g_knobs.enc_full_last_layer = value;
    else if (!strcmp(name, "poison_handoff")) {
        if (!c) return fail(OPUS_EBADARG, "poison_handoff needs a context");
        std::vector<int32_t> h(HANDOFF_ERR, 0);
        if (value) for (int i = 0; i < HANDOFF_ERR; ++i) h[i] = i < 512 ? value : ((i & 1) ? 0 : 1);
        HIPC(hipSetDevice(c->device));
        HIPC(hipDeviceSynchronize());
        HIPC(hipMemcpy(c->d_cnt, h.data(), h.size() * sizeof(int32_t), hipMemcpyHostToDevice));
    }
    else if (!strcmp(name, "pp_gm")) { if (value < 1 || value > 64) return fail(OPUS_EBADARG, "pp_gm out of range"); g_knobs.pp_gm = value; }
    else if (!strncmp(name, "misc", 4) && name[4] >= '0' && name[4] <= '7' && !name[5]) g_knobs.misc[name[4] - '0'] = value;
    else return fail(OPUS_EBADARG, "debug_knob: unknown knob '%s'", name);
    return OPUS_OK;
}

extern "C" int64_t opus_stat(opus_ctx *c, const char *name) {
    if (!c || !name) return -1;
    if (!strcmp(name, "graph_instantiations")) return c->graph_instantiations;
    if (!strcmp(name, "graph_replays")) return c->graph_replays;
    if (!strcmp(name, "graphs_cached")) return (int64_t)c->graphs.size();
    if (!strcmp(name, "decode_steps")) return c->decode_steps;
    if (!strcmp(name, "w8_gemms")) return c->w8_gemms;
    if (!strcmp(name, "w4_gemms")) return c->w4_gemms;
    if (!strcmp(name, "prefills_behind")) return c->prefills_behind;
    if (!strcmp(name, "stream_steps")) return c->stream_steps;
    if (!strcmp(name, "stream_refills")) return c->stream_refills;
    if (!strcmp(name, "stream_graph")) return c->stream_graph.exec ? 1 : 0;
    if (!strcmp(name, "lookup_passes")) return c->lookup_passes;
    return -1;
}

extern "C" int opus_timing_enable(opus_ctx *c, int32_t on) {
    if (!c) return fail(OPUS_EBADARG, "ctx is null");
    c->timing = on != 0;
    return OPUS_OK;
}
extern "C" int opus_timing_reset(opus_ctx *c) {
    if (!c) return fail(OPUS_EBADARG, "ctx is null");
    HIPC(hipDeviceSynchronize());
    timing_clear(c);
    return OPUS_OK;
}
static const char *kclass_names[KC_COUNT] = {"gemm_skinny", "gemm_mid", "gemm_wide", "gemm_ring", "gemm_pp", "gemm_tile", "splitk_reduce",
                                            "attn_prefill", "attn_decode", "norm", "other", "gemm_stream", "contact", "constraint", "guidance", "mlm", "logitproc",
                                            "xent"};
static const char *phase_names[PH_COUNT] = {"encode", "project", "splice", "prefill", "decode", "other", "score"};

extern "C" int opus_timing_get(opus_ctx *c, const char *kernel_class, const char *phase, double *ms, int64_t *launches,
                               double *bytes, double *flops) {
    if (!c || !kernel_class || !phase || !ms || !launches || !bytes || !flops) return fail(OPUS_EBADARG, "null argument");
    int k = -1, ph = -1;
    const bool any_k = !strcmp(kernel_class, "*"), any_p = !strcmp(phase, "*");
    for (int i = 0; i < KC_COUNT; ++i) if (!strcmp(kclass_names[i], kernel_class)) k = i;
    for (int i = 0; i < PH_COUNT; ++i) if (!strcmp(phase_names[i], phase)) ph = i;
    if (k < 0 && !any_k) return fail(OPUS_EBADARG, "unknown kernel class '%s'", kernel_class);
    if (ph < 0 && !any_p) return fail(OPUS_EBADARG, "unknown phase '%s'", phase);
    HIPC(hipDeviceSynchronize());
    double t = 0, b = 0, f = 0;
    int64_t n = 0;
    for (auto &r : c->recs) {
        if ((!any_k && r.klass != k) || (!any_p && r.phase != ph)) continue;
        float e = 0;
        HIPC(hipEventElapsedTime(&e, r.e0, r.e1));
        t += e;
        b += r.bytes;
        f += r.flops;
        ++n;
    }
    *ms = t;
    *launches = n;
    *bytes = b;
    *flops = f;
    return OPUS_OK;
}

extern "C" int opus_timing_names(char *buf, int32_t cap) {
    if (!buf || cap < 1) return fail(OPUS_EBADARG, "null buffer");
    std::string out;
    for (int i = 0; i < KC_COUNT; ++i) { out += kclass_names[i]; out += i + 1 < KC_COUNT ? "," : ";"; }
    for (int i = 0; i < PH_COUNT; ++i) { out += phase_names[i]; if (i + 1 < PH_COUNT) out += ","; }
    if ((int)out.size() + 1 > cap) return fail(OPUS_ESHAPE, "buffer too small (%zu needed)", out.size() + 1);
    memcpy(buf, out.c_str(), out.size() + 1);
    return OPUS_OK;
}
```

opus-pllm_amd/csrc/attn_prefill.hip:

```cpp
#include "common.h"
#include <type_traits>

namespace opus {

constexpr int KB = 64;

template <int HDP>
__device__ __forceinline__ int kswz(int row, int chunk) {
    if (HDP == 128) return chunk ^ (row & 15);
    if (HDP == 64) return chunk ^ ((row >> 1) & 7);
    return chunk;
}
template <int HD>
__device__ __forceinline__ int vswz(int row) {
    if (HD == 128) return (row & 7) << 1;
    if (HD == 64) return ((row >> 1) & 3) << 1;
    if (HD == 32) return ((row >> 2) & 1) << 1;
    return 0;
}

typedef float f2 __attribute__((ext_vector_type(2)));
__device__ __forceinline__ float max3(float a, float b, float c) {
    float r;
    asm("v_max3_f32 %0, %1, %2, %3" : "=v"(r) : "v"(a), "v"(b), "v"(c));
    return r;
}
__device__ __forceinline__ float xor16_max(float x) {
    float a = x, b = x, r;
    asm volatile("s_nop 1\n\tv_permlane16_swap_b32 %0, %1" : "+v"(a), "+v"(b));
    asm("v_max_f32 %0, %1, %2" : "=v"(r) : "v"(a), "v"(b));
    return r;
}
__device__ __forceinline__ void xor32_pair(float x, float &a, float &b) {
    a = x;
    b = x;
    asm volatile("s_nop 1\n\tv_permlane32_swap_b32 %0, %1" : "+v"(a), "+v"(b));
}

typedef short s4v __attribute__((ext_vector_type(4)));
typedef short s8v __attribute__((ext_vector_type(8)));

template <int HD, bool CAUSAL, int QT>
__global__ __launch_bounds__(256) void attn_prefill_kernel(AttnParams p) {
    constexpr int QW = 16 * QT, QB = 4 * QW;
    constexpr int HDP = HD < 32 ? 32 : HD;
    constexpr int KS = HDP / 32;
    constexpr int NO = HD / 16;
    constexpr int CH = HDP / 8;
    constexpr int VC = HD / 8;
    __shared__ __attribute__((aligned(16))) half_t sK[2][KB * HDP];
    __shared__ __attribute__((aligned(16))) half_t sV[2][KB * HD];

    const int tid = threadIdx.x, lane = tid & 63;
    const int wave = __builtin_amdgcn_readfirstlane(tid >> 6);
    const int g = lane >> 4, li = lane & 15;
    const int qtrim = (p.q_trim && p.cu) ? 1 : 0;
    const int nqb = (p.T - 2 * qtrim + QB - 1) / QB;
    const int id = blockIdx.x, slot = id >> 3;
    const int bh = (slot / nqb) * 8 + (id & 7);
    if (bh >= p.B * p.heads) return;
    const int b = bh / p.heads, h = bh % p.heads, hk = h / p.group;
    const int q0 = (slot % nqb) * QB + qtrim, qw = q0 + wave * QW;
    int T = p.T, Tq = p.T;
    int64_t qb_off = (int64_t)b * p.q_sb, kb_off = (int64_t)b * p.k_sb, vb_off = (int64_t)b * p.v_sb, ob_off = (int64_t)b * p.o_sb;
    if (p.cu) {
        const int r0 = p.cu[b];
        T = p.cu[b + 1] - r0;
        Tq = T - qtrim;
        if (q0 >= Tq) return;
        qb_off = (int64_t)r0 * p.q_st; kb_off = (int64_t)r0 * p.k_st; vb_off = (int64_t)r0 * p.v_st; ob_off = (int64_t)r0 * p.o_st;
    }
    const int kstart = (p.kstart && !p.cu) ? p.kstart[b] : 0;
    const int kend = (p.kend && !p.cu) ? p.kend[b] : T;

    const half_t *Qb = p.Q + qb_off + (int64_t)h * HD;
    const half_t *Kb = p.K + kb_off + (int64_t)hk * HD;
    const half_t *Vb = p.V + vb_off + (int64_t)hk * HD;

    h8 qf[QT][KS];
#pragma unroll
    for (int t = 0; t < QT; ++t) {
        int qr = qw + 16 * t + li;
        qr = qr < Tq ? qr : Tq - 1;
        const half_t *src = Qb + (int64_t)qr * p.q_st;
#pragma unroll
        for (int s = 0; s < KS; ++s) {
            const int d = 32 * s + 8 * g;
            qf[t][s] = d < HD ? *reinterpret_cast<const h8 *>(src + d) : h8{0, 0, 0, 0, 0, 0, 0, 0};
        }
    }
    f4 o[QT][NO];
    float mrow[QT], lrow[QT];
#pragma unroll
    for (int t = 0; t < QT; ++t) {
        mrow[t] = -INFINITY;
        lrow[t] = 0.f;
#pragma unroll
        for (int n = 0; n < NO; ++n) o[t][n] = f4{0.f, 0.f, 0.f, 0.f};
    }

    int k_lo = kstart / KB * KB;
    int k_hi = kend;
    if (CAUSAL) {
        const int last_q = (q0 + QB - 1 < T - 1 ? q0 + QB - 1 : T - 1);
        k_hi = k_hi < last_q + 1 ? k_hi : last_q + 1;
    }
    const float sc = p.scale * 1.4426950408889634f;
    const bool wave_live = qw < Tq;

    constexpr int KL = KB * CH / 256;
    constexpr int VN = KB * VC;
    constexpr int VL = VN >= 256 ? VN / 256 : 1;
    static_assert(KL >= 1, "tile too small for 256 threads");
    h8 kreg[KL], vreg[VL];
    const __amdgpu_buffer_rsrc_t krs = __builtin_amdgcn_make_buffer_rsrc((void *)Kb, 0, (int)(((int64_t)(T - 1) * p.k_st + HD) * 2), 0x00020000);
    const __amdgpu_buffer_rsrc_t vrs = __builtin_amdgcn_make_buffer_rsrc((void *)Vb, 0, (int)(((int64_t)(T - 1) * p.v_st + HD) * 2), 0x00020000);
    int koff[KL], voff[VL];
#pragma unroll
    for (int u = 0; u < KL; ++u) {
        const int i = tid + 256 * u, r = i / CH, c = i % CH;
        koff[u] = c * 8 < HD ? (int)((r * p.k_st + c * 8) * 2) : 0x7ffffff0;
    }
#pragma unroll
    for (int u = 0; u < VL; ++u) {
        const int i = tid + 256 * u, r = i / VC, c = i % VC;
        voff[u] = i < VN ? (int)((r * p.v_st + c * 8) * 2) : 0x7ffffff0;
    }
    auto load_tile = [&](int kt) {
        const int kb = kt * (int)p.k_st * 2, vb = kt * (int)p.v_st * 2;
#pragma unroll
        for (int u = 0; u < KL; ++u) kreg[u] = __builtin_bit_cast(h8, __builtin_amdgcn_raw_buffer_load_b128(krs, koff[u] + kb, 0, 0));
#pragma unroll
        for (int u = 0; u < VL; ++u) vreg[u] = __builtin_bit_cast(h8, __builtin_amdgcn_raw_buffer_load_b128(vrs, voff[u] + vb, 0, 0));
    };
    auto store_tile = [&](int buf) {
#pragma unroll
        for (int u = 0; u < KL; ++u) {
            const int i = tid + 256 * u, r = i / CH, c = i % CH;
            *reinterpret_cast<h8 *>(&sK[buf][r * HDP + kswz<HDP>(r, c) * 8]) = kreg[u];
        }
#pragma unroll
        for (int u = 0; u < VL; ++u) {
            const int i = tid + 256 * u, r = i / VC, c = i % VC;
            if (i < VN) *reinterpret_cast<h8 *>(&sV[buf][r * HD + (c ^ vswz<HD>(r)) * 8]) = vreg[u];
        }
    };

    if (k_lo < k_hi) {
        load_tile(k_lo);
        store_tile(0);
        if (k_lo + KB < k_hi) load_tile(k_lo + KB);
    }
    __syncthreads();
    auto tile_body = [&](auto nsub_tag, int kt, int buf) {
        {
            constexpr int NSUB = decltype(nsub_tag)::value, NJ = (NSUB + 1) / 2;
            const half_t *tK = sK[buf], *tV = sV[buf];
            f4 s[QT][4];
#pragma unroll
            for (int n = 0; n < NSUB; ++n) {
                const int r = 16 * n + li;
                h8 kf[KS];
#pragma unroll
                for (int ks = 0; ks < KS; ++ks) kf[ks] = *reinterpret_cast<const h8 *>(tK + r * HDP + kswz<HDP>(r, 4 * ks + g) * 8);
#pragma unroll
                for (int t = 0; t < QT; ++t) {
                    s[t][n] = f4{0.f, 0.f, 0.f, 0.f};
#pragma unroll
                    for (int ks = 0; ks < KS; ++ks) s[t][n] = mfma16(kf[ks], qf[t][ks], s[t][n]);
                }
            }
            const bool interior = kt >= kstart && kt + KB <= kend && (!CAUSAL || kt + KB - 1 <= qw);
            if (__builtin_expect(!interior, 0)) {
#pragma unroll
                for (int t = 0; t < QT; ++t) {
                    const int qi = qw + 16 * t + li;
#pragma unroll
                    for (int n = 0; n < NSUB; ++n)
#pragma unroll
                        for (int r = 0; r < 4; ++r) {
                            const int kj = kt + 16 * n + 4 * g + r;
                            bool vis = kj >= kstart && kj < kend;
                            if (CAUSAL) vis = vis && kj <= qi;
                            s[t][n][r] = vis ? s[t][n][r] : -INFINITY;
                        }
                }
            }
            h8 pf[QT][2];
#pragma unroll
            for (int t = 0; t < QT; ++t) {
                float mx = fmaxf(fmaxf(s[t][0][0], s[t][0][1]), fmaxf(s[t][0][2], s[t][0][3]));
#pragma unroll
                for (int n = 1; n < NSUB; ++n) mx = fmaxf(fmaxf(mx, fmaxf(s[t][n][0], s[t][n][1])), fmaxf(s[t][n][2], s[t][n][3]));
                float ma, mb;
                mx = xor16_max(mx);
                xor32_pair(mx, ma, mb);
                const float mnew = max3(mrow[t], ma, mb);
                const float msafe = mnew == -INFINITY ? 0.f : mnew;
                const float msc = msafe * sc;
                if (!__all(mnew == mrow[t])) {
                    const float alpha = __builtin_amdgcn_exp2f((mrow[t] - msafe) * sc);
                    lrow[t] *= alpha;
#pragma unroll
                    for (int n = 0; n < NO; ++n) o[t][n] *= alpha;
                    mrow[t] = mnew;
                }
                const f2 sc2 = f2{sc, sc}, msc2 = f2{msc, msc};
                f2 rs2 = f2{0.f, 0.f};
#pragma unroll
                for (int n = 0; n < NSUB; ++n)
#pragma unroll
                    for (int r = 0; r < 4; r += 2) {
                        const f2 a = f2{s[t][n][r], s[t][n][r + 1]} * sc2 - msc2;
                        const f2 e = f2{__builtin_amdgcn_exp2f(a[0]), __builtin_amdgcn_exp2f(a[1])};
                        s[t][n][r] = e[0];
                        s[t][n][r + 1] = e[1];
                        rs2 += e;
                    }
                lrow[t] += rs2[0] + rs2[1];
#pragma unroll
                for (int j = 0; j < NJ; ++j) {
                    const bool two = 2 * j + 1 < NSUB;
                    pf[t][j] = h8{(half_t)s[t][2 * j][0], (half_t)s[t][2 * j][1], (half_t)s[t][2 * j][2], (half_t)s[t][2 * j][3],
                                  two ? (half_t)s[t][two ? 2 * j + 1 : 0][0] : (half_t)0.f, two ? (half_t)s[t][two ? 2 * j + 1 : 0][1] : (half_t)0.f,
                                  two ? (half_t)s[t][two ? 2 * j + 1 : 0][2] : (half_t)0.f, two ? (half_t)s[t][two ? 2 * j + 1 : 0][3] : (half_t)0.f};
                }
            }
#pragma unroll
            for (int n = 0; n < NO; ++n)
#pragma unroll
                for (int j = 0; j < NJ; ++j) {
                    const int r0 = 16 * (2 * j) + 4 * g + (li >> 2), r1 = r0 + 16;
                    const int cc = 2 * n + ((li & 3) >> 1), off = (li & 1) * 4;
                    const s4v lo = __builtin_amdgcn_ds_read_tr16_b64_v4i16(
                        (__attribute__((address_space(3))) s4v *)(tV + r0 * HD + (cc ^ vswz<HD>(r0)) * 8 + off));
                    const s4v hi = __builtin_amdgcn_ds_read_tr16_b64_v4i16(
                        (__attribute__((address_space(3))) s4v *)(tV + r1 * HD + (cc ^ vswz<HD>(r1)) * 8 + off));
                    const s8v both = s8v{lo[0], lo[1], lo[2], lo[3], hi[0], hi[1], hi[2], hi[3]};
                    const h8 vf = __builtin_bit_cast(h8, both);
#pragma unroll
                    for (int t = 0; t < QT; ++t) o[t][n] = mfma16(vf, pf[t][j], o[t][n]);
                }
        }
    };
    auto run = [&](auto live_tag) {
        constexpr bool LIVE = decltype(live_tag)::value;
        int kt = k_lo, buf = 0;
        for (; k_hi - kt > 32; kt += KB, buf ^= 1) {
            if constexpr (LIVE) tile_body(std::integral_constant<int, 4>{}, kt, buf);
            if (kt + KB < k_hi) {
                store_tile(buf ^ 1);
                if (kt + 2 * KB < k_hi) load_tile(kt + 2 * KB);
            }
            __syncthreads();
        }
        if constexpr (LIVE) {
            if (kt < k_hi) {
                if (k_hi - kt > 16) tile_body(std::integral_constant<int, 2>{}, kt, buf);
                else tile_body(std::integral_constant<int, 1>{}, kt, buf);
            }
        }
    };
    if (wave_live) run(std::true_type{});
    else run(std::false_type{});

    if (!wave_live) return;
#pragma unroll
    for (int t = 0; t < QT; ++t) {
        float l = lrow[t];
        l += __shfl_xor(l, 16, 64);
        l += __shfl_xor(l, 32, 64);
        const int qi = qw + 16 * t + li;
        if (qi >= Tq) continue;
        const float inv = l > 0.f ? 1.0f / l : 0.f;
        half_t *dst = p.O + ob_off + (int64_t)qi * p.o_st + (int64_t)h * HD;
#pragma unroll
        for (int n = 0; n < NO; ++n)
            *reinterpret_cast<h4 *>(dst + 16 * n + 4 * g) =
                h4{(half_t)(o[t][n][0] * inv), (half_t)(o[t][n][1] * inv), (half_t)(o[t][n][2] * inv), (half_t)(o[t][n][3] * inv)};
    }
}

template <int HD, int QT>
static hipError_t launch_qt(const AttnParams &p, hipStream_t s) {
    const int nqb = cdiv(p.T - ((p.q_trim && p.cu) ? 2 : 0), 64 * QT);
    dim3 grid(((p.B * p.heads + 7) / 8) * 8 * nqb);
    if (p.causal) OPUS_LAUNCH(KC_ATTN_PREFILL, (attn_prefill_kernel<HD, true, QT>), grid, dim3(256), 0, s, p);
    else OPUS_LAUNCH(KC_ATTN_PREFILL, (attn_prefill_kernel<HD, false, QT>), grid, dim3(256), 0, s, p);
    return hipGetLastError();
}
int attn_prefill_query_tiles(const AttnParams &p) {
    bool one = !(p.head_dim <= 64 && (int64_t)p.B * p.heads * cdiv(p.T, 128) >= 512);
    if (g_knobs.misc[3]) one = !one;
    return one ? 1 : 2;
}
template <int HD>
static hipError_t launch_hd(const AttnParams &p, hipStream_t s) {
    return attn_prefill_query_tiles(p) == 1 ? launch_qt<HD, 1>(p, s) : launch_qt<HD, 2>(p, s);
}

hipError_t launch_attn_prefill(const AttnParams &p, hipStream_t s) {
    if (p.T <= 0 || p.B <= 0) return hipErrorInvalidValue;
    if ((p.o_st & 3) || (p.o_sb & 3) || (p.q_st & 7) || (p.k_st & 7) || (p.v_st & 7) || (p.q_sb & 7) || (p.k_sb & 7) || (p.v_sb & 7))
        return hipErrorInvalidValue;
    if ((int64_t)p.T * (p.k_st > p.v_st ? p.k_st : p.v_st) * 2 >= (1ll << 31)) return hipErrorInvalidValue;
    switch (p.head_dim) {
        case 16: return launch_hd<16>(p, s);
        case 32: return launch_hd<32>(p, s);
        case 64: return launch_hd<64>(p, s);
        case 128: return launch_hd<128>(p, s);
    }
    return hipErrorInvalidValue;
}

}
```

opus-pllm_amd/csrc/common.h:

```cpp
#pragma once
#include <hip/hip_runtime.h>
#include <hip/hip_ext.h>
#include <stdint.h>

namespace opus {

#ifdef OPUS_BF16
typedef __bf16 half_t;
typedef __bf16 h8 __attribute__((ext_vector_type(8)));
typedef __bf16 h4 __attribute__((ext_vector_type(4)));
typedef __bf16 h2 __attribute__((ext_vector_type(2)));
#else
typedef _Float16 half_t;
typedef _Float16 h8 __attribute__((ext_vector_type(8)));
typedef _Float16 h4 __attribute__((ext_vector_type(4)));
typedef _Float16 h2 __attribute__((ext_vector_type(2)));
#endif
typedef float f4 __attribute__((ext_vector_type(4)));
__device__ __forceinline__ f4 mfma16(h8 a, h8 b, f4 c) {
#ifdef OPUS_BF16
    return __builtin_amdgcn_mfma_f32_16x16x32_bf16(a, b, c, 0, 0, 0);
#else
    return __builtin_amdgcn_mfma_f32_16x16x32_f16(a, b, c, 0, 0, 0);
#endif
}

enum Epi { EPI_NONE = 0, EPI_GELU = 1, EPI_SILU_GU16 = 2 };
__device__ __forceinline__ int kpart_begin(int n, int part, int parts) {
    return parts == 1 ? (part ? n : 0) : (int)((unsigned)(n * part) / (unsigned)parts);
}
#define OPUS_ARGS_ONE_BATCH(p)                                                                                                        \
    asm volatile("" ::"s"((p).A), "s"((p).Af), "s"((p).W), "s"((p).C), "s"((p).bias), "s"((p).residual), "s"((p).ws), "s"((p).xh_out),  \
                 "s"((p).ssq_out), "s"((p).row_ssq), "s"((p).lda), "s"((p).ldc), "s"((p).ldr), "s"((p).M), "s"((p).N), "s"((p).K),     \
                 "s"((p).out_f32), "s"((p).norm_eps), "s"((p).row_nblk), "s"((p).no_rot), "s"((p).c_tiled))
constexpr int SKINNY_MAX_M_CAP = 16;
int skinny_max_m();
#define SKINNY_MAX_M skinny_max_m()
constexpr int MID_MAX_M = 64;
enum KClass { KC_SKINNY = 0, KC_MID, KC_WIDE, KC_RING, KC_PP, KC_TILE, KC_REDUCE, KC_ATTN_PREFILL, KC_ATTN_DECODE, KC_NORM,
              KC_OTHER, KC_STREAM, KC_CONTACT, KC_CONSTRAINT, KC_GUIDANCE, KC_MLM, KC_LOGITPROC, KC_XENT, KC_COUNT };
enum Phase { PH_ENCODE = 0, PH_PROJECT, PH_SPLICE, PH_PREFILL, PH_DECODE, PH_OTHER, PH_SCORE, PH_COUNT };

struct LaunchEvents {
    hipEvent_t main0 = nullptr, main1 = nullptr, aux0 = nullptr, aux1 = nullptr;
    int main_class = -1;
    bool main_used = false, aux_used = false;
    double aux_bytes = 0.0;
};
extern thread_local LaunchEvents *tl_launch_ev;
#define OPUS_LAUNCH(klass, kernel, grid, block, lds, stream, ...)                                                        \
    do {                                                                                                                  \
        ::opus::LaunchEvents *ev_ = ::opus::tl_launch_ev;                                                                 \
        if (ev_ && (klass) != ::opus::KC_REDUCE && !ev_->main_used) {                                                     \
            ev_->main_used = true;                                                                                        \
            ev_->main_class = (klass);                                                                                    \
            hipExtLaunchKernelGGL(kernel, grid, block, lds, stream, ev_->main0, ev_->main1, 0, __VA_ARGS__);              \
        } else if (ev_ && (klass) == ::opus::KC_REDUCE && !ev_->aux_used) {                                               \
            ev_->aux_used = true;                                                                                         \
            hipExtLaunchKernelGGL(kernel, grid, block, lds, stream, ev_->aux0, ev_->aux1, 0, __VA_ARGS__);                \
        } else {                                                                                                          \
            hipLaunchKernelGGL(kernel, grid, block, lds, stream, __VA_ARGS__);                                            \
        }                                                                                                                 \
    } while (0)
hipError_t ensure_dyn_lds(const void *fn, size_t bytes);

__device__ __forceinline__ void rotate_pair(float a, float b, float c, float sn, float &lo, float &hi) {
    lo = __builtin_fmaf(a, c, -__fmul_rn(b, sn));
    hi = __builtin_fmaf(b, c, __fmul_rn(a, sn));
    asm volatile("" : "+v"(lo), "+v"(hi));
}

__host__ __device__ __forceinline__ int64_t tiled_off(int row, int k, int K) {
    return ((int64_t)(row >> 4) * (K >> 6) + (k >> 6)) * 1024 + ((k & 63) >> 5) * 512 + ((((k & 31) >> 3) << 4) + (row & 15)) * 8 + (k & 7);
}

__host__ __device__ __forceinline__ int64_t fp8_tiled_off(int64_t n, int64_t k, int64_t K) {
    return ((n >> 4) * (K >> 6) + (k >> 6)) * 1024 + ((((k & 31) >> 3) << 4) + (n & 15)) * 16 + ((k & 63) >> 5) * 8 + (k & 7);
}
constexpr int W8_EXP_MIN = -120;
#ifdef OPUS_BF16
constexpr int OPERAND_MIN_EXP = -126, OPERAND_MAX_EXP = 127;
#else
constexpr int OPERAND_MIN_EXP = -14, OPERAND_MAX_EXP = 15;
#endif
typedef unsigned int u32x4 __attribute__((ext_vector_type(4)));
__device__ __forceinline__ void fp8x16_to_h8(u32x4 q, h8 &lo, h8 &hi) {
#ifdef OPUS_BF16
#define OPUS_CVT_FP8(w, sel) __builtin_amdgcn_cvt_scalef32_pk_bf16_fp8((int)(w), 1.0f, sel)
#else
#define OPUS_CVT_FP8(w, sel) __builtin_amdgcn_cvt_scalef32_pk_f16_fp8((int)(w), 1.0f, sel)
#endif
    const h2 a0 = OPUS_CVT_FP8(q[0], false), a1 = OPUS_CVT_FP8(q[0], true), a2 = OPUS_CVT_FP8(q[1], false), a3 = OPUS_CVT_FP8(q[1], true);
    const h2 b0 = OPUS_CVT_FP8(q[2], false), b1 = OPUS_CVT_FP8(q[2], true), b2 = OPUS_CVT_FP8(q[3], false), b3 = OPUS_CVT_FP8(q[3], true);
#undef OPUS_CVT_FP8
    lo = h8{a0[0], a0[1], a1[0], a1[1], a2[0], a2[1], a3[0], a3[1]};
    hi = h8{b0[0], b0[1], b1[0], b1[1], b2[0], b2[1], b3[0], b3[1]};
}
__device__ __forceinline__ float exp2_i8(int e) { return __builtin_bit_cast(float, (uint32_t)(e + 127) << 23); }
hipError_t launch_quantize_fp8(const half_t *src, int64_t N, int64_t K, uint8_t *q8, int8_t *e8, half_t *dq, int *bad, hipStream_t s);

__host__ __device__ __forceinline__ int64_t mx4_code_off(int64_t n, int64_t k, int64_t K) {
    return ((n >> 4) * (K >> 6) + (k >> 6)) * 512 + ((((k & 31) >> 3) << 4) + (n & 15)) * 8 + ((k & 63) >> 5) * 4 + ((k & 7) >> 1);
}
__host__ __device__ __forceinline__ int64_t mx4_scale_off(int64_t n, int64_t kb, int64_t K) {
    return ((n >> 4) * (K >> 6) + (kb >> 1)) * 32 + (n & 15) * 2 + (kb & 1);
}
constexpr int W4_EXP_MIN = W8_EXP_MIN;
typedef unsigned int u32x2 __attribute__((ext_vector_type(2)));
__device__ __forceinline__ void mx4x16_to_h8(u32x2 q, uint32_t s2, h8 &lo, h8 &hi) {
    const float s0 = __builtin_bit_cast(float, (s2 & 0xffu) << 23), s1 = __builtin_bit_cast(float, (s2 & 0xff00u) << 15);
#ifdef OPUS_BF16
#define OPUS_CVT_FP4(w, sc, sel) __builtin_amdgcn_cvt_scalef32_pk_bf16_fp4((w), (sc), sel)
#else
#define OPUS_CVT_FP4(w, sc, sel) __builtin_amdgcn_cvt_scalef32_pk_f16_fp4((w), (sc), sel)
#endif
    const h2 a0 = OPUS_CVT_FP4(q[0], s0, 0), a1 = OPUS_CVT_FP4(q[0], s0, 1), a2 = OPUS_CVT_FP4(q[0], s0, 2), a3 = OPUS_CVT_FP4(q[0], s0, 3);
    const h2 b0 = OPUS_CVT_FP4(q[1], s1, 0), b1 = OPUS_CVT_FP4(q[1], s1, 1), b2 = OPUS_CVT_FP4(q[1], s1, 2), b3 = OPUS_CVT_FP4(q[1], s1, 3);
#undef OPUS_CVT_FP4
    lo = h8{a0[0], a0[1], a1[0], a1[1], a2[0], a2[1], a3[0], a3[1]};
    hi = h8{b0[0], b0[1], b1[0], b1[1], b2[0], b2[1], b3[0], b3[1]};
}
struct mx4reg { u32x2 q; uint32_t s; };
struct mx4ptr { const uint8_t *q, *s; };
__device__ __forceinline__ mx4reg q_load(mx4ptr qp, int64_t c) {
    return mx4reg{__builtin_nontemporal_load(reinterpret_cast<const u32x2 *>(qp.q + c * 512)),
                  __builtin_nontemporal_load(reinterpret_cast<const uint16_t *>(qp.s + c * 32))};
}
__device__ __forceinline__ void q_to_h8(mx4reg q, h8 &lo, h8 &hi) { mx4x16_to_h8(q.q, q.s, lo, hi); }
hipError_t launch_quantize_mxfp4(const half_t *src, int64_t N, int64_t K, uint8_t *q4, uint8_t *s4, half_t *dq, int *bad, hipStream_t s);

constexpr int HANDOFF_WORDS = 1024, HANDOFF_ERR = 1023;
constexpr int HANDOFF_SPIN_LIMIT = 1 << 19;

struct GemmParams {
    const half_t *A;
    const float *Af;
    float norm_eps;
    int64_t lda;
    const half_t *W;
    int M, N, K;
    const float *bias;
    const float *residual;
    int64_t ldr;
    void *C;
    int64_t ldc;
    int out_f32;
    int epi;
    float *ws;
    int64_t ws_bytes;
    half_t *xh_out;
    float *ssq_out;
    int *fused_done;
    const float *row_ssq;
    int row_nblk;
    int64_t ssq_cap = 0;
    int *nblk_out = nullptr;
    int slab_only = 0;
    int *ks_out = nullptr;
    int force_wide = 0;
    const float *rope_cs = nullptr;
    const int32_t *rope_pos = nullptr;
    int rope_T = 0, rope_cols = 0, rope_qcols = 0;
    float rope_qscale = 1.0f;
    int *rope_done = nullptr;
    int a_tiled = 0, xh_tiled = 0, c_tiled = 0;
    int *combine_cnt = nullptr;
    float *ln_part = nullptr;
    int *ln_done = nullptr;
    const float *ln_stat = nullptr;
    const float *ln_colsum = nullptr;
    int pp_gm = 8;
    int stagger = 0;
    int no_rot = 0;
    long long *trace = nullptr;
    int *pp_plan = nullptr;
    int *plan = nullptr;
    const uint8_t *q8 = nullptr;
    const int8_t *e8 = nullptr;
    int *ran_w8 = nullptr;
    const uint8_t *q4 = nullptr;
    const uint8_t *s4 = nullptr;
    int *ran_w4 = nullptr;
};
constexpr int PP_PLAN_WORDS = 5;
enum PpTail { PP_TAIL_NONE = 0, PP_TAIL_PAIR = 1, PP_TAIL_REDUCE = 2 };
constexpr int GEMM_PLAN_WORDS = 8;
enum GemmCombine { GC_NONE = 0, GC_REDUCE = 1, GC_REDUCE4 = 2, GC_IN_LAUNCH = 3, GC_PP_PAIR = 4, GC_PP_REDUCE = 5, GC_SLABS = 6 };
inline void gemm_plan_set(const GemmParams &p, int klass, int mt, int tn, int ns, int alds, int P, int ks, int combine) {
    if (!p.plan) return;
    const int v[GEMM_PLAN_WORDS] = {klass, mt, tn, ns, alds, P, ks, combine};
    for (int i = 0; i < GEMM_PLAN_WORDS; ++i) p.plan[i] = v[i];
}

struct AttnParams {
    const half_t *Q, *K, *V;
    int64_t q_sb, q_st, k_sb, k_st, v_sb, v_st;
    half_t *O;
    int64_t o_sb, o_st;
    const int32_t *kstart;
    const int32_t *kend;
    int B, T, heads, group, head_dim, causal;
    float scale;
    const int32_t *cu = nullptr;
    int q_trim = 0;
};

hipError_t launch_gemm(const GemmParams &p, hipStream_t s, int *klass);
hipError_t launch_splitk_reduce(const GemmParams &p, int ks, hipStream_t s);
bool gemm_stream_ok(const GemmParams &p);
bool gemm_stream_would(int M, int N, int K, int slab_only, int a_tiled, int row_scale, int64_t ws_bytes);
hipError_t launch_gemm_stream(const GemmParams &p, hipStream_t s);
struct Knobs {
    int no_stream = 0;
    int no_ln_fusion = 0;
    int debug_a_tiled = 0;
    int pp_gm = 8;
    int enc_full_last_layer = 0;
    int misc[8] = {0, 0, 0, 0, 0, 0, 0, 0};
};
extern Knobs g_knobs;
template <int NWAVES, int ROWS>
__device__ __forceinline__ void block_row_rstd(const float *__restrict__ ssq, int M, int nblk, float inv_k, float eps, float *out,
                                               int wave, int lane) {
    constexpr int RW = (ROWS + NWAVES - 1) / NWAVES;
    float part[RW];
#pragma unroll
    for (int r = 0; r < RW; ++r) part[r] = 0.f;
    for (int j0 = 0; j0 < nblk; j0 += 256) {
        float t[RW][4];
#pragma unroll
        for (int r = 0; r < RW; ++r) {
            int row = wave + NWAVES * r;
            row = row < M ? row : M - 1;
#pragma unroll
            for (int u = 0; u < 4; ++u) {
                const int j = j0 + 64 * u + lane;
                t[r][u] = ssq[(int64_t)row * nblk + (j < nblk ? j : nblk - 1)];
                t[r][u] = j < nblk ? t[r][u] : 0.f;
            }
        }
#pragma unroll
        for (int r = 0; r < RW; ++r) part[r] += (t[r][0] + t[r][1]) + (t[r][2] + t[r][3]);
    }
#pragma unroll
    for (int r = 0; r < RW; ++r) {
        float q = part[r];
#pragma unroll
        for (int o = 32; o > 0; o >>= 1) q += __shfl_xor(q, o, 64);
        const int row = wave + NWAVES * r;
        if (lane == 0 && row < ROWS) out[row] = rsqrtf(q * inv_k + eps);
    }
}
bool gemm_goes_wide(int M, int N);
bool gemm_goes_pp(int M, int N);
hipError_t launch_attn_prefill(const AttnParams &p, hipStream_t s);
int attn_prefill_query_tiles(const AttnParams &p);
struct AttnPrefixParams {
    const half_t *kc, *vc;
    int64_t cache_sb, cache_sh;
    const int32_t *kstart;
    int Tp;
    const half_t *qkv;
    int n;
    const int32_t *list, *off, *blocks;
    half_t *out;
    int nh, nkv, hd;
    float scale;
    const int32_t *par = nullptr;
};
int attn_prefix_blocks(const int32_t *off, int P, int G, int n, int32_t *blocks);
int attn_prefix_max_blocks(int R, int P, int G, int n);
hipError_t launch_attn_prefix(const AttnPrefixParams &p, int nblocks, hipStream_t s);

hipError_t launch_kv_export(const half_t *kc, const half_t *vc, int64_t cache_sl, int64_t cache_sb, int64_t cache_sh, int layers, int R,
                            int nkv, int T, int hd, half_t *snap_k, half_t *snap_v, hipStream_t s);
struct KvPlaceParams {
    const half_t *snap_k, *snap_v;
    const int32_t *kstart;
    int P, Tp;
    half_t *kc, *vc;
    int64_t cache_sl, cache_sb, cache_sh;
    const int32_t *list, *off;
    const int32_t *new_kstart;
    int layers, nkv, hd;
};
hipError_t launch_kv_place(const KvPlaceParams &p, hipStream_t s);
hipError_t launch_kv_append(const half_t *qkv, const int32_t *lens, int R, int n, int nh, int nkv, int hd, int Tp, half_t *kc, half_t *vc,
                            int64_t cache_sb, int64_t cache_sh, hipStream_t s);

hipError_t launch_stream_finish(const int32_t *step, const int32_t *start, int32_t *fin, int32_t *poll, int B, int max_new, hipStream_t s);
hipError_t launch_stream_refill(const int32_t *rows, const int32_t *src, const int32_t *nks, int n, const float *logits_in, float *logits,
                                int V, int32_t *kstart, int32_t *start, int32_t *fin, int32_t *poll, int32_t *ids, int S, int t,
                                hipStream_t s);
hipError_t launch_stream_reset(int32_t *start, int32_t *poll, int B, hipStream_t s);

struct ContactParams {
    const half_t *Q, *K;
    int64_t ld;
    const int32_t *cu;
    int B, heads;
    const float *w;
    float *A;
    int accumulate;
    float *rows;
    int64_t vld;
    int c0;
    float *part;
};
size_t contact_accum_lds(int heads);
hipError_t launch_esm_contact_accum(const ContactParams &p, int head_dim, int max_n, hipStream_t s);
hipError_t launch_esm_contact_colsum(const float *part, const int32_t *cu, int B, int heads, int max_n, float *vec, int64_t vld, int c0,
                                     int add, hipStream_t s);
hipError_t launch_esm_contact_scale(const float *vec, const int32_t *cu, int B, int C, const float *w, float *sw, hipStream_t s);
hipError_t launch_esm_contact_finish(const float *A, const float *vec, const float *sw, const int32_t *cu, int B, int C, int max_n,
                                     const float *bias, float *out, hipStream_t s);

hipError_t launch_mlm_gather(const float *src, int64_t src_rows, const int32_t *idx, int R, int Mg, int D, half_t *dst, hipStream_t s);
hipError_t launch_mlm_head(const half_t *y, const float *lnw, const float *lnb, float eps, const half_t *We, const float *bias,
                           int64_t R, int D, int V, int log_softmax, float *out, hipStream_t s);
hipError_t launch_layernorm(const float *x, const float *w, const float *b, float eps, int64_t rows, int D,
                            half_t *out_h, float *out_f, hipStream_t s);
hipError_t launch_ln_finalize(const float *part, int64_t rows, int nslab, int D, float eps, int rms, float *stat, hipStream_t s);
hipError_t launch_rmsnorm(const float *x, const float *w, float eps, int64_t rows, int D, half_t *out,
                          hipStream_t s);
hipError_t launch_l2norm(const float *x, int64_t rows, int D, half_t *out, hipStream_t s);
hipError_t launch_f2h(const float *x, int64_t n, half_t *out, hipStream_t s);
hipError_t launch_masked_mean(const float *h, const int32_t *lens, int B, int T, int D, float *out,
                              hipStream_t s);
hipError_t launch_masked_mean_packed(const float *h, const int32_t *cu, int B, int D, float *out, hipStream_t s);
hipError_t launch_esm_embed_packed(const int32_t *tok, const half_t *emb, const int32_t *cu, int B, int Tmax, int D, float *x,
                                   int32_t *pos, hipStream_t s);

hipError_t launch_esm_embed(const int32_t *tok, const half_t *emb, int B, int T, int D, float *x, hipStream_t s);
hipError_t launch_esm_rope(half_t *qkv, const float *cs, int B, int T, int heads, int hd, float qscale,
                           hipStream_t s, const int32_t *pos = nullptr);
hipError_t launch_dec_rope_cache(half_t *qkv, const float *cs, const int32_t *kstart, int B, int T, int nh,
                                 int nkv, int hd, half_t *kc, half_t *vc, int64_t cache_sb, int64_t cache_sh,
                                 hipStream_t s, int nret = 1);
hipError_t launch_row_fanout(const float *src, float *dst, int V, int B, int nret, int32_t *kstart, hipStream_t s);
hipError_t launch_h2f(const half_t *in, float *out, int64_t n, hipStream_t s);
hipError_t launch_embed_tokens(const int32_t *tok, const half_t *emb, int B, int H, int V, float *x, half_t *xh, float *ssq,
                               int xh_tiled, const float *cs, const int32_t *kstart, const int32_t *step, int T0, int half,
                               float *cs_row, int *cnt, int ncnt, hipStream_t s);
hipError_t launch_add_pos(float *x, const half_t *pos, const int32_t *kstart, const int32_t *step, int t0, int B, int Tq,
                          int H, int max_idx, hipStream_t s);
hipError_t launch_take_last(const float *x, int B, int T, int H, float *out, hipStream_t s);
hipError_t launch_gather_rows(const float *x, const int32_t *rows, int R, int64_t n_src, int H, float *out, hipStream_t s);
hipError_t launch_gather_rows2(const float *x, int64_t n_x, const float *y, int64_t n_y, const int32_t *rows, int R, int H, float *out,
                               hipStream_t s);
hipError_t launch_xent(const half_t *logits, int64_t ld, int R, int V, const int32_t *targets, float *logprob, float *lse,
                       hipStream_t s);
hipError_t launch_tree_edges(const half_t *logits, int64_t ld, const float *lse, int row0, const int32_t *erow, const int32_t *etok,
                             const int32_t *eslot, int n_edges, float *node_lp, const int32_t *srow, const int32_t *sset,
                             const int32_t *sslot, int n_stops, const int32_t *ids, const int32_t *soff, float *stop_lp, hipStream_t s);
hipError_t launch_tree_path_sums(const float *node_lp, const int32_t *trie, const int32_t *par, const int32_t *depth,
                                 const int32_t *mnode, int P, int M, int ld_nodes, float *member_lp, hipStream_t s);
hipError_t launch_relu_h(half_t *x, int64_t n, hipStream_t s);
hipError_t launch_fill_synth(void *dst, int dtype, int64_t rows, int64_t cols, uint64_t seed, float std,
                             float mean, int64_t rb, int64_t rs, int64_t ro, int tiled, uint64_t fold_seed,
                             float fold_std, float fold_mean, hipStream_t s);
hipError_t launch_argmax_partial(const float *logits, int B, int V, float *pval, int32_t *pidx, hipStream_t s);
hipError_t launch_tile_weight(const half_t *src, half_t *dst, int64_t N, int64_t K, hipStream_t s);
hipError_t launch_lora_merge(half_t *W, const half_t *A, const half_t *B, float scale, int64_t out_f,
                             int64_t in_f, int r, hipStream_t s);
hipError_t launch_splice_plan(const int64_t *ids, const uint8_t *mask, int B, int Tt, int n_tok, int max_len,
                              int V, int32_t *plan, hipStream_t s);
hipError_t launch_splice_fill(const int64_t *ids, const uint8_t *mask, int B, int Tt, const half_t *prot,
                              int n_tok, int H, int V, const half_t *emb, const int32_t *plan, int Tout,
                              int left_pad, half_t *out, uint8_t *mask_out, int32_t *pos_out, hipStream_t s);
hipError_t launch_sample_select(const float *logits, int B, int V, float temperature, float top_p, int top_k, const uint64_t *seed,
                                const int32_t *step, float *pmax, int32_t *pidx, float *cand_p, int32_t *cand_i,
                                int32_t *cand_n, float *zpart, float *spart, int32_t *chosen, float *thr_out, float *psum,
                                float *thr_keep, hipStream_t s);
constexpr int APART = 64;
__device__ __forceinline__ uint64_t splitmix64(uint64_t x) {
    x += 0x9E3779B97F4A7C15ull;
    x = (x ^ (x >> 30)) * 0xBF58476D1CE4E5B9ull;
    x = (x ^ (x >> 27)) * 0x94D049BB133111EBull;
    return x ^ (x >> 31);
}
hipError_t launch_argmax_step(const float *pval, const int32_t *pidx, const int32_t *chosen, int B, const int32_t *eos, int n_eos, int pad_id,
                              int32_t *finished, int32_t *out_ids, int max_new, const int32_t *step,
                              int32_t *next_tok, int32_t *n_unfinished, const int32_t *stop, int n_stop, hipStream_t s);
hipError_t launch_step_advance(int32_t *step, hipStream_t s);
struct GenOutDesc {
    float *token_lp;
    float *scores;
    float *logits;
    float *unused;
};
hipError_t launch_argmax_lse_partial(const float *logits, int B, int V, float *pval, int32_t *pidx, float *psum, hipStream_t s);
hipError_t launch_argmax_lse_step(const float *pval, const int32_t *pidx, const float *psum, const int32_t *chosen, int B,
                                  const int32_t *eos, int n_eos, int pad_id, int32_t *finished, int32_t *out_ids, int max_new,
                                  const int32_t *step, int32_t *next_tok, int32_t *n_unfinished, const int32_t *stop, int n_stop,
                                  const float *logits, int V, const GenOutDesc *out, hipStream_t s);
hipError_t launch_argmax_lse_final(const float *pval, const int32_t *pidx, const float *psum, int B, int32_t *idx, float *lse,
                                   hipStream_t s);
hipError_t launch_argmax_rawlp_step(const float *pval, const int32_t *pidx, const float *lse, const float *raw_hist,
                                    const int32_t *chosen, int B, const int32_t *eos, int n_eos, int pad_id, int32_t *finished,
                                    int32_t *out_ids, int max_new, const int32_t *step, int32_t *next_tok, int32_t *n_unfinished,
                                    const int32_t *stop, int n_stop, const float *logits, int V, const GenOutDesc *out,
                                    hipStream_t s);
hipError_t launch_gen_scores(const float *logits, int B, int V, const GenOutDesc *out, const int32_t *step, int max_new,
                             float temperature, float top_p, const float *pmax, const float *thr, hipStream_t s);
constexpr int LP_MAX_BAD = 256, LP_MAX_BAD_LEN = 8, LP_MAX_BAD_IDS = 1024, LP_MAX_HIST = 2048;
struct LogitsProcDesc {
    float penalty;
    int32_t ngram;
// ... 90 lines not shown
```

opus-pllm_amd/csrc/elementwise.hip:

```cpp
#include "common.h"

namespace opus {

__global__ __launch_bounds__(256) void esm_embed_kernel(const int32_t *__restrict__ tok, const half_t *__restrict__ emb,
                                                        int T, int D, float *__restrict__ x, const int32_t *__restrict__ cu,
                                                        int32_t *__restrict__ pos) {
    __shared__ int s_cnt[2];
    const int b = blockIdx.y;
    int64_t r0 = (int64_t)b * T;
    if (cu) {
        r0 = cu[b];
        T = cu[b + 1] - cu[b];
        if ((int)blockIdx.x * 16 >= T) return;
    }
    const int32_t *row = tok + r0;
    if (threadIdx.x < 2) s_cnt[threadIdx.x] = 0;
    __syncthreads();
    int nm = 0, nv = 0;
    for (int t = threadIdx.x; t < T; t += 256) {
        const int v = row[t];
        nm += (v == 32);
        nv += (v != 1);
    }
    atomicAdd(&s_cnt[0], nm);
    atomicAdd(&s_cnt[1], nv);
    __syncthreads();
    const float scale = (1.0f - 0.15f * 0.8f) / (1.0f - (float)s_cnt[0] / (float)s_cnt[1]);
    const int t0 = blockIdx.x * 16;
    const int nvec = D >> 3;
    for (int i = threadIdx.x; i < 16 * nvec; i += 256) {
        const int t = t0 + i / nvec, c = i % nvec;
        if (t >= T) break;
        const int v = row[t];
        float o[8];
        if (v == 1 || v == 32) {
#pragma unroll
            for (int j = 0; j < 8; ++j) o[j] = 0.f;
        } else {
            const h8 e = *reinterpret_cast<const h8 *>(emb + (int64_t)v * D + c * 8);
#pragma unroll
            for (int j = 0; j < 8; ++j) o[j] = (float)e[j] * scale;
        }
        float4 *dst = reinterpret_cast<float4 *>(x + (r0 + t) * D + c * 8);
        dst[0] = make_float4(o[0], o[1], o[2], o[3]);
        dst[1] = make_float4(o[4], o[5], o[6], o[7]);
        if (pos && c == 0) pos[r0 + t] = t;
    }
}

hipError_t launch_esm_embed(const int32_t *tok, const half_t *emb, int B, int T, int D, float *x, hipStream_t s) {
    hipLaunchKernelGGL(esm_embed_kernel, dim3(cdiv(T, 16), B), dim3(256), 0, s, tok, emb, T, D, x, nullptr, nullptr);
    return hipGetLastError();
}
hipError_t launch_esm_embed_packed(const int32_t *tok, const half_t *emb, const int32_t *cu, int B, int Tmax, int D, float *x,
                                   int32_t *pos, hipStream_t s) {
    if (!cu || !pos) return hipErrorInvalidValue;
    hipLaunchKernelGGL(esm_embed_kernel, dim3(cdiv(Tmax, 16), B), dim3(256), 0, s, tok, emb, Tmax, D, x, cu, pos);
    return hipGetLastError();
}

__device__ __forceinline__ void rope8(half_t *base, int half, const float *cs, float scale) {
    h8 lo = *reinterpret_cast<h8 *>(base);
    h8 hi = *reinterpret_cast<h8 *>(base + half);
    h8 olo, ohi;
#pragma unroll
    for (int j = 0; j < 8; ++j) {
        const float c = cs[2 * j], sn = cs[2 * j + 1];
        const float a = (float)lo[j] * scale, b = (float)hi[j] * scale;
        float rl, rh;
        rotate_pair(a, b, c, sn, rl, rh);
        olo[j] = (half_t)rl;
        ohi[j] = (half_t)rh;
    }
    *reinterpret_cast<h8 *>(base) = olo;
    *reinterpret_cast<h8 *>(base + half) = ohi;
}

__global__ __launch_bounds__(256) void esm_rope_kernel(half_t *__restrict__ qkv, const float *__restrict__ cs, int T,
                                                       int heads, int hd, float qscale, int64_t total, const int32_t *__restrict__ pos) {
    const int64_t i = (int64_t)blockIdx.x * 256 + threadIdx.x;
    if (i >= total) return;
    const int half = hd >> 1, vph = half >> 3;
    const int v = (int)(i % vph);
    int64_t r = i / vph;
    const int h = (int)(r % heads); r /= heads;
    const int which = (int)(r & 1);
    const int64_t row = r >> 1;
    const int t = pos ? pos[row] : (int)(row % T);
    const int D = heads * hd;
    half_t *base = qkv + row * (3 * (int64_t)D) + which * D + h * hd + v * 8;
    rope8(base, half, cs + ((int64_t)t * half + v * 8) * 2, which == 0 ? qscale : 1.0f);
}

hipError_t launch_esm_rope(half_t *qkv, const float *cs, int B, int T, int heads, int hd, float qscale, hipStream_t s, const int32_t *pos) {
    if (hd & 15) return hipErrorInvalidValue;
    const int64_t total = (int64_t)B * T * 2 * heads * (hd >> 4);
    hipLaunchKernelGGL(esm_rope_kernel, dim3(cdiv(total, 256)), dim3(256), 0, s, qkv, cs, T, heads, hd, qscale, total, pos);
    return hipGetLastError();
}

template <bool FAN>
__device__ __forceinline__ void dec_rope_cache_body(half_t *__restrict__ qkv, const float *__restrict__ cs,
                                                    const int32_t *__restrict__ kstart, int T, int nh, int nkv, int hd,
                                                    half_t *__restrict__ kc, half_t *__restrict__ vc, int64_t cache_sb,
                                                    int64_t cache_sh, int64_t total, int nret) {
    const int64_t i = (int64_t)blockIdx.x * 256 + threadIdx.x;
    if (i >= total) return;
    const int half = hd >> 1, vph = half >> 3;
    const int v = (int)(i % vph);
    int64_t r = i / vph;
    const int hh = (int)(r % (nh + nkv)); r /= (nh + nkv);
    const int64_t row = r;
    const int b = (int)(row / T), t = (int)(row % T);
    int pos = t - kstart[b];
    pos = pos < 0 ? 0 : pos;
    const int64_t ld = (int64_t)(nh + 2 * nkv) * hd;
    half_t *base = qkv + row * ld + (int64_t)hh * hd + v * 8;
    rope8(base, half, cs + ((int64_t)pos * half + v * 8) * 2, 1.0f);
    if (hh >= nh && kc) {
        const int kh = hh - nh;
        const half_t *vs = base + (int64_t)nkv * hd;
        if constexpr (!FAN) {
            half_t *kd = kc + b * cache_sb + kh * cache_sh + (int64_t)t * hd + v * 8;
            half_t *vd = vc + b * cache_sb + kh * cache_sh + (int64_t)t * hd + v * 8;
            *reinterpret_cast<h8 *>(kd) = *reinterpret_cast<h8 *>(base);
            *reinterpret_cast<h8 *>(kd + half) = *reinterpret_cast<h8 *>(base + half);
            *reinterpret_cast<h8 *>(vd) = *reinterpret_cast<const h8 *>(vs);
            *reinterpret_cast<h8 *>(vd + half) = *reinterpret_cast<const h8 *>(vs + half);
        } else {
            const h8 k0 = *reinterpret_cast<h8 *>(base), k1 = *reinterpret_cast<h8 *>(base + half);
            const h8 v0 = *reinterpret_cast<const h8 *>(vs), v1 = *reinterpret_cast<const h8 *>(vs + half);
            const int64_t off = kh * cache_sh + (int64_t)t * hd + v * 8;
            for (int j = 0; j < nret; ++j) {
                const int64_t o = ((int64_t)b * nret + j) * cache_sb + off;
                *reinterpret_cast<h8 *>(kc + o) = k0;
                *reinterpret_cast<h8 *>(kc + o + half) = k1;
                *reinterpret_cast<h8 *>(vc + o) = v0;
                *reinterpret_cast<h8 *>(vc + o + half) = v1;
            }
        }
    }
}

__global__ __launch_bounds__(256) void dec_rope_cache_kernel(half_t *__restrict__ qkv, const float *__restrict__ cs,
                                                             const int32_t *__restrict__ kstart, int T, int nh, int nkv,
                                                             int hd, half_t *__restrict__ kc, half_t *__restrict__ vc,
                                                             int64_t cache_sb, int64_t cache_sh, int64_t total) {
    dec_rope_cache_body<false>(qkv, cs, kstart, T, nh, nkv, hd, kc, vc, cache_sb, cache_sh, total, 1);
}

__global__ __launch_bounds__(256) void dec_rope_cache_fan_kernel(half_t *__restrict__ qkv, const float *__restrict__ cs,
                                                                 const int32_t *__restrict__ kstart, int T, int nh, int nkv,
                                                                 int hd, half_t *__restrict__ kc, half_t *__restrict__ vc,
                                                                 int64_t cache_sb, int64_t cache_sh, int64_t total, int nret) {
    dec_rope_cache_body<true>(qkv, cs, kstart, T, nh, nkv, hd, kc, vc, cache_sb, cache_sh, total, nret);
}

hipError_t launch_dec_rope_cache(half_t *qkv, const float *cs, const int32_t *kstart, int B, int T, int nh, int nkv,
                                 int hd, half_t *kc, half_t *vc, int64_t cache_sb, int64_t cache_sh, hipStream_t s, int nret) {
    if (hd & 15) return hipErrorInvalidValue;
    const int64_t total = (int64_t)B * T * (nh + nkv) * (hd >> 4);
    if (nret > 1 && kc)
        hipLaunchKernelGGL(dec_rope_cache_fan_kernel, dim3(cdiv(total, 256)), dim3(256), 0, s, qkv, cs, kstart, T, nh, nkv, hd,
                           kc, vc, cache_sb, cache_sh, total, nret);
    else
        hipLaunchKernelGGL(dec_rope_cache_kernel, dim3(cdiv(total, 256)), dim3(256), 0, s, qkv, cs, kstart, T, nh, nkv, hd,
                           kc, vc, cache_sb, cache_sh, total);
    return hipGetLastError();
}

__global__ __launch_bounds__(256) void h2f_kernel(const half_t *__restrict__ in, float *__restrict__ out, int64_t n8) {
    const int64_t i = (int64_t)blockIdx.x * 256 + threadIdx.x;
    if (i >= n8) return;
    const h8 v = reinterpret_cast<const h8 *>(in)[i];
    float4 *o = reinterpret_cast<float4 *>(out) + 2 * i;
    o[0] = make_float4((float)v[0], (float)v[1], (float)v[2], (float)v[3]);
    o[1] = make_float4((float)v[4], (float)v[5], (float)v[6], (float)v[7]);
}
hipError_t launch_h2f(const half_t *in, float *out, int64_t n, hipStream_t s) {
    if (n & 7) return hipErrorInvalidValue;
    hipLaunchKernelGGL(h2f_kernel, dim3(cdiv(n >> 3, 256)), dim3(256), 0, s, in, out, n >> 3);
    return hipGetLastError();
}

__global__ __launch_bounds__(256) void add_pos_kernel(float *__restrict__ x, const half_t *__restrict__ pos,
                                                      const int32_t *__restrict__ kstart, const int32_t *__restrict__ step,
                                                      int t0, int Tq, int H, int max_idx) {
    const int row = blockIdx.x, b = row / Tq, tq = row % Tq;
    const int slot = (t0 >= 0 ? t0 : step[1]) + (step ? step[0] : 0) + tq;
    int idx = slot >= kstart[b] ? slot - kstart[b] + 2 : 1;
    idx = idx > max_idx ? max_idx : idx;
    for (int c = threadIdx.x; c < (H >> 3); c += 256) {
        const h8 e = *reinterpret_cast<const h8 *>(pos + (int64_t)idx * H + c * 8);
        float4 *o = reinterpret_cast<float4 *>(x + (int64_t)row * H + c * 8);
        float4 a = o[0], d = o[1];
        a.x += (float)e[0]; a.y += (float)e[1]; a.z += (float)e[2]; a.w += (float)e[3];
        d.x += (float)e[4]; d.y += (float)e[5]; d.z += (float)e[6]; d.w += (float)e[7];
        o[0] = a;
        o[1] = d;
    }
}
hipError_t launch_add_pos(float *x, const half_t *pos, const int32_t *kstart, const int32_t *step, int t0, int B, int Tq,
                          int H, int max_idx, hipStream_t s) {
    if (H & 7) return hipErrorInvalidValue;
    hipLaunchKernelGGL(add_pos_kernel, dim3(B * Tq), dim3(256), 0, s, x, pos, kstart, step, t0, Tq, H, max_idx);
    return hipGetLastError();
}

__global__ __launch_bounds__(256) void embed_tokens_kernel(const int32_t *__restrict__ tok, const half_t *__restrict__ emb,
                                                           int H, int V, float *__restrict__ x, half_t *__restrict__ xh,
                                                           float *__restrict__ ssq, int xh_tiled, const float *__restrict__ cs,
                                                           const int32_t *__restrict__ kstart, const int32_t *__restrict__ step,
                                                           int T0, int half, float *__restrict__ cs_row, int *__restrict__ cnt, int ncnt) {
    const int b = blockIdx.x;
    if (cnt && b == 0)
        for (int i = threadIdx.x; i < ncnt; i += 256) cnt[i] = 0;
    if (cs) {
        const int pos = (T0 >= 0 ? T0 : step[1]) + step[0] - kstart[b];
        for (int d = threadIdx.x; d < half; d += 256)
            reinterpret_cast<float2 *>(cs_row)[(int64_t)b * half + d] = reinterpret_cast<const float2 *>(cs)[(int64_t)pos * half + d];
    }
    int id = tok[b];
    id = id < 0 ? 0 : (id >= V ? V - 1 : id);
    for (int c = threadIdx.x; c < (H >> 3); c += 256) {
        const h8 e = *reinterpret_cast<const h8 *>(emb + (int64_t)id * H + c * 8);
        float4 *o = reinterpret_cast<float4 *>(x + (int64_t)b * H + c * 8);
// ... 887 lines not shown
```

opus-pllm_amd/csrc/gemm.hip:

```cpp
#include "common.h"
#include <cstdlib>
#include <map>
#include <type_traits>
#include <mutex>
#include <utility>

namespace opus {

thread_local LaunchEvents *tl_launch_ev = nullptr;
static Knobs knobs_from_env() {
    Knobs k;
    for (int i = 0; i < 8; ++i) {
        char name[32];
        snprintf(name, sizeof(name), "OPUS_KNOB_MISC%d", i);
        if (const char *v = getenv(name)) k.misc[i] = atoi(v);
    }
    return k;
}
Knobs g_knobs = knobs_from_env();

hipError_t ensure_dyn_lds(const void *fn, size_t bytes) {
    static std::mutex mu;
    static std::map<std::pair<int, const void *>, size_t> done;
    int dev = 0;
    hipError_t e = hipGetDevice(&dev);
    if (e != hipSuccess) return e;
    std::lock_guard<std::mutex> lock(mu);
    size_t &have = done[std::make_pair(dev, fn)];
    if (bytes <= have) return hipSuccess;
    e = hipFuncSetAttribute(fn, hipFuncAttributeMaxDynamicSharedMemorySize, (int)bytes);
    if (e == hipSuccess) have = bytes;
    return e;
}

__device__ __forceinline__ float gelu_erf(float x) {
    const float z = fabsf(x) * 0.70710678118654752f;
    const float t = __builtin_amdgcn_rcpf(1.0f + 0.3275911f * z);
    const float poly = t * (0.254829592f + t * (-0.284496736f + t * (1.421413741f + t * (-1.453152027f + t * 1.061405429f))));
    const float erf_abs = 1.0f - poly * __expf(-z * z);
    return 0.5f * x * (1.0f + copysignf(erf_abs, x));
}
__device__ __forceinline__ float silu(float x) { return x * __builtin_amdgcn_rcpf(1.0f + __expf(-x)); }

template <int MT, int EPI, bool NORM, bool ALDS, bool W8 = false, bool W4 = false>
__global__ __launch_bounds__(1024) void gemm_skinny_kernel(GemmParams p) {
    static_assert(!(W8 && W4), "one quantised form at a time");
    extern __shared__ __attribute__((aligned(16))) float red[];
    OPUS_ARGS_ONE_BATCH(p);
    constexpr int PB = EPI == EPI_SILU_GU16 ? 2 : 1;
    const int tid = threadIdx.x;
    const int lane = tid & 63;
    const int wave = __builtin_amdgcn_readfirstlane(tid >> 6);
    const int nwaves = blockDim.x >> 6;
    const int wpp = nwaves / PB;
    const int pl = PB == 1 ? 0 : wave / wpp, kpart = wave - pl * wpp;
    const int chunks = p.K >> 6;
    const int npanels = (p.N + 15) >> 4;
    int panel = blockIdx.x * PB + pl;
    panel = panel < npanels ? panel : npanels - 1;
    const int c0 = kpart_begin(chunks, kpart, wpp);
    const int c1 = kpart_begin(chunks, kpart + 1, wpp);
    const int g = lane >> 4, li = lane & 15;
    float *rss = red + nwaves * MT * 256;
    float *wss = rss + nwaves * MT * 16;
    half_t *xs = reinterpret_cast<half_t *>(wss + 256);

    const half_t *wp = p.W + ((int64_t)panel * chunks) * 1024 + lane * 8;
    f4 acc[MT];
    float ssq[MT];
#pragma unroll
    for (int i = 0; i < MT; ++i) { acc[i] = f4{0.f, 0.f, 0.f, 0.f}; ssq[i] = 0.f; }

    if constexpr (W4) {
        static_assert(!W4 || MT == 1, "the MXFP4 form is built for M <= 16");
        constexpr int U = (NORM && !ALDS) ? 2 : 4;
        typedef mx4reg qreg_t;
        const mx4ptr qp{p.q4 + ((int64_t)panel * chunks) * 512 + lane * 8, p.s4 + ((int64_t)panel * chunks) * 32 + li * 2};
        const int nck = c1 - c0;
        const int rot = (ALDS && !p.no_rot && nck >= 2) ? (int)((wave * 3u) % (unsigned)nck) : 0;
        auto phys = [&](int c) { const int q = c + rot; return q < c1 ? q : q - nck; };
        auto qload = [&](qreg_t (&q)[U], int c) {
#pragma unroll
            for (int u = 0; u < U; ++u) {
                if (c + u < c1) q[u] = q_load(qp, phys(c + u));
                else q[u] = qreg_t{};
            }
        };
        if constexpr (ALDS) {
            qreg_t qA[U], qB[U];
            qload(qA, c0);
            const int nthr = blockDim.x;
            for (int m = 0; m < p.M; ++m) {
                if (NORM) {
                    const float4 *src = reinterpret_cast<const float4 *>(p.Af + (int64_t)m * p.lda);
                    float s = 0.f;
                    for (int i = tid; i < (p.K >> 2); i += nthr) {
                        const float4 v = src[i];
                        s += (v.x * v.x + v.y * v.y) + (v.z * v.z + v.w * v.w);
                        *reinterpret_cast<h4 *>(xs + (int64_t)m * p.K + 4 * i) = h4{(half_t)v.x, (half_t)v.y, (half_t)v.z, (half_t)v.w};
                    }
#pragma unroll
                    for (int o = 32; o > 0; o >>= 1) s += __shfl_xor(s, o, 64);
                    if (lane == 0) wss[m * 16 + wave] = s;
                } else {
                    const h8 *src = reinterpret_cast<const h8 *>(p.A + (int64_t)m * p.lda);
                    for (int i = tid; i < (p.K >> 3); i += nthr)
                        *reinterpret_cast<h8 *>(xs + (int64_t)m * p.K + 8 * i) = src[i];
                }
            }
            __syncthreads();
            const int mr = li < p.M ? li : p.M - 1;
            const h8 *xr = reinterpret_cast<const h8 *>(xs + (int64_t)mr * p.K + g * 8);
            auto compute = [&](const qreg_t (&q)[U], int c) {
#pragma unroll
                for (int u = 0; u < U; ++u) {
                    const int cc = phys(c + u < c1 ? c + u : c1 - 1);
                    const h8 al = xr[cc * 8], ah = xr[cc * 8 + 4];
                    h8 wl, wh;
                    q_to_h8(q[u], wl, wh);
                    acc[0] = mfma16(al, wl, acc[0]);
                    acc[0] = mfma16(ah, wh, acc[0]);
                }
            };
            for (int c = c0; c < c1; c += 2 * U) {
                if (c + U < c1) qload(qB, c + U);
                compute(qA, c);
                if (c + U < c1) {
                    if (c + 2 * U < c1) qload(qA, c + 2 * U);
                    compute(qB, c + U);
                }
            }
        } else {
            constexpr int ESZ = NORM ? 4 : 2;
            const __amdgpu_buffer_rsrc_t arsrc = __builtin_amdgcn_make_buffer_rsrc(
                NORM ? (void *)p.Af : (void *)p.A, 0, (int)((int64_t)((p.M - 1) * p.lda + p.K) * ESZ), 0x00020000);
            const int aoff = li < p.M ? (int)((li * p.lda + g * 8) * ESZ) : 0x40000000;
            struct ARaw { u32x4 v[NORM ? 4 : 2]; };
            auto load_a = [&](int c, ARaw &r) {
                const int o = aoff + c * 64 * ESZ;
                if (NORM) {
                    r.v[0] = __builtin_amdgcn_raw_buffer_load_b128(arsrc, o, 0, 0);
                    r.v[1] = __builtin_amdgcn_raw_buffer_load_b128(arsrc, o + 16, 0, 0);
                    r.v[2] = __builtin_amdgcn_raw_buffer_load_b128(arsrc, o + 128, 0, 0);
                    r.v[3] = __builtin_amdgcn_raw_buffer_load_b128(arsrc, o + 144, 0, 0);
                } else {
                    r.v[0] = __builtin_amdgcn_raw_buffer_load_b128(arsrc, o, 0, 0);
                    r.v[1] = __builtin_amdgcn_raw_buffer_load_b128(arsrc, o + 64, 0, 0);
                }
            };
            auto conv_a = [&](const ARaw &r, h8 &lo, h8 &hi) {
                if (NORM) {
                    const float4 a0 = __builtin_bit_cast(float4, r.v[0]), a1 = __builtin_bit_cast(float4, r.v[1]);
                    const float4 b0 = __builtin_bit_cast(float4, r.v[2]), b1 = __builtin_bit_cast(float4, r.v[3]);
                    ssq[0] += (a0.x * a0.x + a0.y * a0.y) + (a0.z * a0.z + a0.w * a0.w) + (a1.x * a1.x + a1.y * a1.y) +
                              (a1.z * a1.z + a1.w * a1.w) + (b0.x * b0.x + b0.y * b0.y) + (b0.z * b0.z + b0.w * b0.w) +
                              (b1.x * b1.x + b1.y * b1.y) + (b1.z * b1.z + b1.w * b1.w);
                    lo = h8{(half_t)a0.x, (half_t)a0.y, (half_t)a0.z, (half_t)a0.w, (half_t)a1.x, (half_t)a1.y, (half_t)a1.z, (half_t)a1.w};
                    hi = h8{(half_t)b0.x, (half_t)b0.y, (half_t)b0.z, (half_t)b0.w, (half_t)b1.x, (half_t)b1.y, (half_t)b1.z, (half_t)b1.w};
                } else {
                    lo = __builtin_bit_cast(h8, r.v[0]);
                    hi = __builtin_bit_cast(h8, r.v[1]);
                }
            };
            auto step = [&](qreg_t q, const ARaw &r) {
                h8 al, ah, wl, wh;
                conv_a(r, al, ah);
                q_to_h8(q, wl, wh);
                acc[0] = mfma16(al, wl, acc[0]);
                acc[0] = mfma16(ah, wh, acc[0]);
// ... 2378 lines not shown
```

Before: 258.9 proteins/s.

## Fuse RoPE, KV-cache write and GQA prefill attention into one kernel

Adds a prefill attention kernel that runs one block per (batch, kv-head). It applies RoPE to K and Q in-kernel, writes K/V to the cache, stages the whole K/V sequence in LDS, and serves every query head in the GQA group from that shared copy. This replaces the separate rope+cache kernel and the per-head attention kernel for single-return prefill, cutting a launch and the repeated K/V global reads. The trade-off is up to 128KB of dynamic LDS per block, which limits occupancy, and grid parallelism of only B*nkv blocks.

After: 260.5 proteins/s (median of 6 runs). No clear change (+0.6%).

```diff
diff --git a/include/opus_pllm.h b/include/opus_pllm.h
--- a/include/opus_pllm.h
+++ b/include/opus_pllm.h
@@ -232,6 +232,10 @@
                             int32_t heads, int32_t group, int32_t head_dim, int32_t causal, int32_t q_trim, float scale,
                             int32_t *qt_used, void *stream);
 
+int opus_debug_attn_prefill_gqa(opus_ctx *ctx, const void *d_qkv, const float *d_cs, const int32_t *d_kstart, int32_t B, int32_t T,
+                                int32_t heads, int32_t group, int32_t head_dim, float scale, void *d_out, void *d_k_new,
+                                void *d_v_new, int32_t *fused_used, void *stream);
+
 int opus_debug_attn_decode(opus_ctx *ctx, const void *d_qkv, const void *d_k_hist, const void *d_v_hist, const int32_t *d_kstart,
                            int32_t B, int32_t T0, int32_t step, void *d_out, void *d_k_new, void *d_v_new, void *stream);
 
diff --git a/opus-pllm_amd/_cabi.py b/opus-pllm_amd/_cabi.py
--- a/opus-pllm_amd/_cabi.py
+++ b/opus-pllm_amd/_cabi.py
@@ -116,6 +116,8 @@
     "opus_debug_attn_prefill": (C.c_int, [_P, _P, _P, _P, _P, C.c_int64, C.c_int64, C.c_int64, C.c_int64, C.c_int64, C.c_int64,
                                           C.c_int64, C.c_int64, _P, _P, _P, C.c_int32, C.c_int32, C.c_int32, C.c_int32, C.c_int32,
                                           C.c_int32, C.c_int32, C.c_float, C.POINTER(C.c_int32), _P]),
+    "opus_debug_attn_prefill_gqa": (C.c_int, [_P, _P, _P, _P, C.c_int32, C.c_int32, C.c_int32, C.c_int32, C.c_int32, C.c_float, _P, _P,
+                                              _P, C.POINTER(C.c_int32), _P]),
     "opus_generate_sample": (C.c_int, [_P, _P, _P, C.c_int32, C.c_int32, C.c_int32, C.POINTER(C.c_int32), C.c_int32, C.c_int32,
                                        C.c_float, C.c_float, C.c_uint64, _P, C.POINTER(C.c_int32), _P]),
     "opus_debug_sample": (C.c_int, [_P, _P, C.c_int32, C.c_float, C.c_float, C.c_uint64, C.c_int32, _P, _P]),
diff --git a/opus-pllm_amd/build.py b/opus-pllm_amd/build.py
--- a/opus-pllm_amd/build.py
+++ b/opus-pllm_amd/build.py
@@ -20,7 +20,7 @@
          "attn_decode.hip": ["-mllvm", "-amdgpu-mfma-vgpr-form"]}
 
 
-NO_SCRATCH = ("gemm_pp_kernel", "gemm_stream_kernel", "gemm_wide_kernel", "gemm_skinny_kernel", "attn_prefill_kernel",
+NO_SCRATCH = ("gemm_pp_kernel", "gemm_stream_kernel", "gemm_wide_kernel", "gemm_skinny_kernel", "attn_prefill_kernel", "attn_prefill_gqa_kernel",
               "attn_decode_kernel", "attn_prefix_kernel", "tree_path_sums_kernel", "beam_", "kv_export_kernel", "kv_place_kernel",
               "kv_append_kernel", "guidance_", "stream_finish_kernel", "stream_refill_kernel", "stream_reset_kernel")
 RU_FLAG = "-Rpass-analysis=kernel-resource-usage"
diff --git a/opus-pllm_amd/csrc/api.cpp b/opus-pllm_amd/csrc/api.cpp
--- a/opus-pllm_amd/csrc/api.cpp
+++ b/opus-pllm_amd/csrc/api.cpp
@@ -1245,9 +1245,43 @@
     return OPUS_OK;
 }
 
+static int attn_prefill_plain(opus_ctx *c, hipStream_t s, int l, int B, int T, int nret, half_t *qkv, const float *cs, float scale,
+                              half_t *O, int *fused) {
+    const opus_config &g = c->cfg;
+    const int nh = g.dec_heads, nkv = g.dec_kv_heads, hd = g.dec_head_dim, QKV = (nh + 2 * nkv) * hd, QD = nh * hd, M = B * T;
+    if (fused) *fused = 0;
+    if (nret == 1) {
+        AttnGqaParams f;
+        f.qkv = qkv; f.ld = QKV; f.cs = cs; f.kstart = c->d_kstart;
+        f.kc = c->kc + l * c->cache_sl; f.vc = c->vc + l * c->cache_sl; f.cache_sb = c->cache_sb; f.cache_sh = c->cache_sh;
+        f.O = O; f.o_st = QD; f.B = B; f.T = T; f.nh = nh; f.nkv = nkv; f.head_dim = hd; f.scale = scale;
+        if (attn_prefill_gqa_takes(f)) {
+            bool taken = false;
+            KLF(KC_ATTN_PREFILL, 2.0 * M * QKV + 4.0 * M * nkv * hd + 2.0 * M * QD, 2.0 * B * (double)T * T * QD,
+                launch_attn_prefill_gqa(f, s, &taken));
+            if (!taken) return fail(OPUS_EHIP, "attn_prefill: the fused launcher refused a shape it had accepted");
+            if (fused) *fused = 1;
+            return OPUS_OK;
+        }
+    }
+    KL(KC_OTHER, 4.0 * M * QKV,
+       launch_dec_rope_cache(qkv, cs, c->d_kstart, B, T, nh, nkv, hd, c->kc + l * c->cache_sl,
+                             c->vc + l * c->cache_sl, c->cache_sb, c->cache_sh, s, nret));
+    AttnParams a;
+    a.Q = qkv; a.K = qkv + QD; a.V = qkv + QD + nkv * hd;
+    a.q_sb = a.k_sb = a.v_sb = (int64_t)T * QKV;
+    a.q_st = a.k_st = a.v_st = QKV;
+    a.O = O; a.o_sb = (int64_t)T * QD; a.o_st = QD;
+    a.kstart = c->d_kstart; a.kend = nullptr;
+    a.B = B; a.T = T; a.heads = nh; a.group = nh / nkv; a.head_dim = hd; a.causal = 1;
+    a.scale = scale;
+    KLF(KC_ATTN_PREFILL, 2.0 * M * (QKV + QD), 2.0 * B * (double)T * T * QD, launch_attn_prefill(a, s));
+    return OPUS_OK;
+}
+
 static int attn_prefill(opus_ctx *c, hipStream_t s, int l, int B, int T, const ContRows *cont, int nret) {
     const opus_config &g = c->cfg;
-    const int nh = g.dec_heads, nkv = g.dec_kv_heads, hd = g.dec_head_dim, QKV = (nh + 2 * nkv) * hd, QD = nh * hd, M = B * T;
+    const int nh = g.dec_heads, nkv = g.dec_kv_heads, hd = g.dec_head_dim, QKV = (nh + 2 * nkv) * hd, M = B * T;
     if (cont) {
         KL(KC_OTHER, 4.0 * M * QKV, launch_dec_rope_cache(c->d_qkv, c->cs_dec, cont->nkst, B, T, nh, nkv, hd, nullptr, nullptr, 0, 0, s));
         if (cont->app_lens)
@@ -1255,19 +1289,7 @@
                                                               c->vc + l * c->cache_sl, c->cache_sb, c->cache_sh, s));
         return attn_prefix(c, s, *cont, l, M);
     }
-    KL(KC_OTHER, 4.0 * M * QKV,
-       launch_dec_rope_cache(c->d_qkv, c->cs_dec, c->d_kstart, B, T, nh, nkv, hd, c->kc + l * c->cache_sl,
-                             c->vc + l * c->cache_sl, c->cache_sb, c->cache_sh, s, nret));
-    AttnParams a;
-    a.Q = c->d_qkv; a.K = c->d_qkv + QD; a.V = c->d_qkv + QD + nkv * hd;
-    a.q_sb = a.k_sb = a.v_sb = (int64_t)T * QKV;
-    a.q_st = a.k_st = a.v_st = QKV;
-    a.O = c->d_ctx; a.o_sb = (int64_t)T * QD; a.o_st = QD;
-    a.kstart = c->d_kstart; a.kend = nullptr;
-    a.B = B; a.T = T; a.heads = nh; a.group = nh / nkv; a.head_dim = hd; a.causal = 1;
-    a.scale = 1.0f / sqrtf((float)hd);
-    KLF(KC_ATTN_PREFILL, 2.0 * M * (QKV + QD), 2.0 * B * (double)T * T * QD, launch_attn_prefill(a, s));
-    return OPUS_OK;
+    return attn_prefill_plain(c, s, l, B, T, nret, c->d_qkv, c->cs_dec, 1.0f / sqrtf((float)hd), c->d_ctx, nullptr);
 }
 
 static int opt_layer(opus_ctx *c, hipStream_t s, const DecLayer &L, int l, float *x, half_t *xn, int M, int B, int T, bool decode,
@@ -3468,6 +3490,35 @@
     return OPUS_OK;
 }
 
+extern "C" int opus_debug_attn_prefill_gqa(opus_ctx *c, const void *d_qkv, const float *d_cs, const int32_t *d_kstart, int32_t B, int32_t T,
+                                           int32_t heads, int32_t group, int32_t hd, float scale, void *d_out, void *d_k_new,
+                                           void *d_v_new, int32_t *fused_used, void *stream) {
+    if (fused_used) *fused_used = 0;
+    if (!c || !d_qkv || !d_kstart || !d_out || !fused_used) return fail(OPUS_EBADARG, "debug_attn_prefill_gqa: null pointer");
+    const opus_config &g = c->cfg;
+    if (group < 1 || heads != g.dec_heads || heads != group * g.dec_kv_heads || hd != g.dec_head_dim)
+        return fail(OPUS_ESHAPE, "debug_attn_prefill_gqa: heads=%d group=%d hd=%d, the context has %d / %d / %d", heads, group, hd,
+                    g.dec_heads, g.dec_heads / g.dec_kv_heads, g.dec_head_dim);
+    if (B < 1 || B > g.max_batch || T < 1 || T > g.max_prompt)
+        return fail(OPUS_ESHAPE, "debug_attn_prefill_gqa: B=%d T=%d exceed the context (%d, %d)", B, T, g.max_batch, g.max_prompt);
+    HIPC(hipSetDevice(c->device));
+    hipStream_t s = (hipStream_t)stream;
+    const int nkv = g.dec_kv_heads;
+    const size_t QKV = (size_t)(heads + 2 * nkv) * hd;
+    HIPC(hipMemcpyAsync(c->d_qkv, d_qkv, (size_t)B * T * QKV * sizeof(half_t), hipMemcpyDeviceToDevice, s));
+    HIPC(hipMemcpyAsync(c->d_kstart, d_kstart, (size_t)B * sizeof(int32_t), hipMemcpyDeviceToDevice, s));
+    c->phase = PH_PREFILL;
+    int fused = 0;
+    OPC(attn_prefill_plain(c, s, 0, B, T, 1, c->d_qkv, d_cs ? d_cs : c->cs_dec, scale, (half_t *)d_out, &fused));
+    *fused_used = fused;
+    const size_t pitch = (size_t)c->cache_sh * sizeof(half_t), roww = (size_t)T * hd * sizeof(half_t);
+    if (d_k_new) HIPC(hipMemcpy2DAsync(d_k_new, roww, c->kc, pitch, roww, (size_t)B * nkv, hipMemcpyDeviceToDevice, s));
+    if (d_v_new) HIPC(hipMemcpy2DAsync(d_v_new, roww, c->vc, pitch, roww, (size_t)B * nkv, hipMemcpyDeviceToDevice, s));
+    c->prefilled = false;
+    new_epoch(c);
+    return OPUS_OK;
+}
+
 struct DecodeForm {
     const void *qkv = nullptr;
     const float *slabs = nullptr, *row_ssq = nullptr, *bias = nullptr;
@@ -3561,6 +3612,7 @@
     else if (!strcmp(name, "debug_a_tiled")) g_knobs.debug_a_tiled = value;
     else if (!strcmp(name, "no_ln_fusion")) g_knobs.no_ln_fusion = value;
     else if (!strcmp(name, "enc_full_last_layer")) g_knobs.enc_full_last_layer = value;
+    else if (!strcmp(name, "no_prefill_attn_fusion")) g_knobs.no_prefill_attn_fusion = value;
     else if (!strcmp(name, "poison_handoff")) {
         if (!c) return fail(OPUS_EBADARG, "poison_handoff needs a context");
         std::vector<int32_t> h(HANDOFF_ERR, 0);
diff --git a/opus-pllm_amd/csrc/attn_prefill.hip b/opus-pllm_amd/csrc/attn_prefill.hip
--- a/opus-pllm_amd/csrc/attn_prefill.hip
+++ b/opus-pllm_amd/csrc/attn_prefill.hip
@@ -39,6 +39,99 @@
 
 typedef short s4v __attribute__((ext_vector_type(4)));
 typedef short s8v __attribute__((ext_vector_type(8)));
+
+template <int HD, bool CAUSAL, int QT, int NSUB>
+__device__ __forceinline__ void attn_tile(const half_t *tK, const half_t *tV, const h8 (&qf)[QT][(HD < 32 ? 32 : HD) / 32],
+                                          f4 (&o)[QT][HD / 16], float (&mrow)[QT], float (&lrow)[QT], int kt, int kstart, int kend,
+                                          int qw, float sc, int g, int li) {
+    constexpr int HDP = HD < 32 ? 32 : HD, KS = HDP / 32, NO = HD / 16;
+    constexpr int NJ = (NSUB + 1) / 2;
+    f4 s[QT][4];
+#pragma unroll
+    for (int n = 0; n < NSUB; ++n) {
+        const int r = 16 * n + li;
+        h8 kf[KS];
+#pragma unroll
+        for (int ks = 0; ks < KS; ++ks) kf[ks] = *reinterpret_cast<const h8 *>(tK + r * HDP + kswz<HDP>(r, 4 * ks + g) * 8);
+#pragma unroll
+        for (int t = 0; t < QT; ++t) {
+            s[t][n] = f4{0.f, 0.f, 0.f, 0.f};
+#pragma unroll
+            for (int ks = 0; ks < KS; ++ks) s[t][n] = mfma16(kf[ks], qf[t][ks], s[t][n]);
+        }
+    }
+    const bool interior = kt >= kstart && kt + KB <= kend && (!CAUSAL || kt + KB - 1 <= qw);
+    if (__builtin_expect(!interior, 0)) {
+#pragma unroll
+        for (int t = 0; t < QT; ++t) {
+            const int qi = qw + 16 * t + li;
+#pragma unroll
+            for (int n = 0; n < NSUB; ++n)
+#pragma unroll
+                for (int r = 0; r < 4; ++r) {
+                    const int kj = kt + 16 * n + 4 * g + r;
+                    bool vis = kj >= kstart && kj < kend;
+                    if (CAUSAL) vis = vis && kj <= qi;
+                    s[t][n][r] = vis ? s[t][n][r] : -INFINITY;
+                }
+        }
+    }
+    h8 pf[QT][2];
+#pragma unroll
+    for (int t = 0; t < QT; ++t) {
+        float mx = fmaxf(fmaxf(s[t][0][0], s[t][0][1]), fmaxf(s[t][0][2], s[t][0][3]));
+#pragma unroll
+        for (int n = 1; n < NSUB; ++n) mx = fmaxf(fmaxf(mx, fmaxf(s[t][n][0], s[t][n][1])), fmaxf(s[t][n][2], s[t][n][3]));
+        float ma, mb;
+        mx = xor16_max(mx);
+        xor32_pair(mx, ma, mb);
+        const float mnew = max3(mrow[t], ma, mb);
+        const float msafe = mnew == -INFINITY ? 0.f : mnew;
+        const float msc = msafe * sc;
+        if (!__all(mnew == mrow[t])) {
+            const float alpha = __builtin_amdgcn_exp2f((mrow[t] - msafe) * sc);
+            lrow[t] *= alpha;
+#pragma unroll
+            for (int n = 0; n < NO; ++n) o[t][n] *= alpha;
+            mrow[t] = mnew;
+        }
+        const f2 sc2 = f2{sc, sc}, msc2 = f2{msc, msc};
+        f2 rs2 = f2{0.f, 0.f};
+#pragma unroll
+        for (int n = 0; n < NSUB; ++n)
+#pragma unroll
+            for (int r = 0; r < 4; r += 2) {
+                const f2 a = f2{s[t][n][r], s[t][n][r + 1]} * sc2 - msc2;
+                const f2 e = f2{__builtin_amdgcn_exp2f(a[0]), __builtin_amdgcn_exp2f(a[1])};
+                s[t][n][r] = e[0];
+                s[t][n][r + 1] = e[1];
+                rs2 += e;
+            }
+        lrow[t] += rs2[0] + rs2[1];
+#pragma unroll
+        for (int j = 0; j < NJ; ++j) {
+            const bool two = 2 * j + 1 < NSUB;
+            pf[t][j] = h8{(half_t)s[t][2 * j][0], (half_t)s[t][2 * j][1], (half_t)s[t][2 * j][2], (half_t)s[t][2 * j][3],
+                          two ? (half_t)s[t][two ? 2 * j + 1 : 0][0] : (half_t)0.f, two ? (half_t)s[t][two ? 2 * j + 1 : 0][1] : (half_t)0.f,
+                          two ? (half_t)s[t][two ? 2 * j + 1 : 0][2] : (half_t)0.f, two ? (half_t)s[t][two ? 2 * j + 1 : 0][3] : (half_t)0.f};
+        }
+    }
+#pragma unroll
+    for (int n = 0; n < NO; ++n)
+#pragma unroll
+        for (int j = 0; j < NJ; ++j) {
+            const int r0 = 16 * (2 * j) + 4 * g + (li >> 2), r1 = r0 + 16;
+            const int cc = 2 * n + ((li & 3) >> 1), off = (li & 1) * 4;
+            const s4v lo = __builtin_amdgcn_ds_read_tr16_b64_v4i16(
+                (__attribute__((address_space(3))) s4v *)(tV + r0 * HD + (cc ^ vswz<HD>(r0)) * 8 + off));
+            const s4v hi = __builtin_amdgcn_ds_read_tr16_b64_v4i16(
+                (__attribute__((address_space(3))) s4v *)(tV + r1 * HD + (cc ^ vswz<HD>(r1)) * 8 + off));
+            const s8v both = s8v{lo[0], lo[1], lo[2], lo[3], hi[0], hi[1], hi[2], hi[3]};
+            const h8 vf = __builtin_bit_cast(h8, both);
+#pragma unroll
+            for (int t = 0; t < QT; ++t) o[t][n] = mfma16(vf, pf[t][j], o[t][n]);
+        }
+}
 
 template <int HD, bool CAUSAL, int QT>
 __global__ __launch_bounds__(256) void attn_prefill_kernel(AttnParams p) {
@@ -153,95 +246,7 @@
     }
     __syncthreads();
     auto tile_body = [&](auto nsub_tag, int kt, int buf) {
-        {
-            constexpr int NSUB = decltype(nsub_tag)::value, NJ = (NSUB + 1) / 2;
-            const half_t *tK = sK[buf], *tV = sV[buf];
-            f4 s[QT][4];
-#pragma unroll
-            for (int n = 0; n < NSUB; ++n) {
-                const int r = 16 * n + li;
-                h8 kf[KS];
-#pragma unroll
-                for (int ks = 0; ks < KS; ++ks) kf[ks] = *reinterpret_cast<const h8 *>(tK + r * HDP + kswz<HDP>(r, 4 * ks + g) * 8);
-#pragma unroll
-                for (int t = 0; t < QT; ++t) {
-                    s[t][n] = f4{0.f, 0.f, 0.f, 0.f};
-#pragma unroll
-                    for (int ks = 0; ks < KS; ++ks) s[t][n] = mfma16(kf[ks], qf[t][ks], s[t][n]);
-                }
-            }
-            const bool interior = kt >= kstart && kt + KB <= kend && (!CAUSAL || kt + KB - 1 <= qw);
-            if (__builtin_expect(!interior, 0)) {
-#pragma unroll
-                for (int t = 0; t < QT; ++t) {
-                    const int qi = qw + 16 * t + li;
-#pragma unroll
-                    for (int n = 0; n < NSUB; ++n)
-#pragma unroll
-                        for (int r = 0; r < 4; ++r) {
-                            const int kj = kt + 16 * n + 4 * g + r;
-                            bool vis = kj >= kstart && kj < kend;
-                            if (CAUSAL) vis = vis && kj <= qi;
-                            s[t][n][r] = vis ? s[t][n][r] : -INFINITY;
-                        }
-                }
-            }
-            h8 pf[QT][2];
-#pragma unroll
-            for (int t = 0; t < QT; ++t) {
-                float mx = fmaxf(fmaxf(s[t][0][0], s[t][0][1]), fmaxf(s[t][0][2], s[t][0][3]));
-#pragma unroll
-                for (int n = 1; n < NSUB; ++n) mx = fmaxf(fmaxf(mx, fmaxf(s[t][n][0], s[t][n][1])), fmaxf(s[t][n][2], s[t][n][3]));
-                float ma, mb;
-                mx = xor16_max(mx);
-                xor32_pair(mx, ma, mb);
-                const float mnew = max3(mrow[t], ma, mb);
-                const float msafe = mnew == -INFINITY ? 0.f : mnew;
-                const float msc = msafe * sc;
-                if (!__all(mnew == mrow[t])) {
-                    const float alpha = __builtin_amdgcn_exp2f((mrow[t] - msafe) * sc);
-                    lrow[t] *= alpha;
-#pragma unroll
-                    for (int n = 0; n < NO; ++n) o[t][n] *= alpha;
-                    mrow[t] = mnew;
-                }
-                const f2 sc2 = f2{sc, sc}, msc2 = f2{msc, msc};
-                f2 rs2 = f2{0.f, 0.f};
-#pragma unroll
-                for (int n = 0; n < NSUB; ++n)
-#pragma unroll
-                    for (int r = 0; r < 4; r += 2) {
-                        const f2 a = f2{s[t][n][r], s[t][n][r + 1]} * sc2 - msc2;
-                        const f2 e = f2{__builtin_amdgcn_exp2f(a[0]), __builtin_amdgcn_exp2f(a[1])};
-                        s[t][n][r] = e[0];
-                        s[t][n][r + 1] = e[1];
-                        rs2 += e;
-                    }
-                lrow[t] += rs2[0] + rs2[1];
-#pragma unroll
-                for (int j = 0; j < NJ; ++j) {
-                    const bool two = 2 * j + 1 < NSUB;
-                    pf[t][j] = h8{(half_t)s[t][2 * j][0], (half_t)s[t][2 * j][1], (half_t)s[t][2 * j][2], (half_t)s[t][2 * j][3],
-                                  two ? (half_t)s[t][two ? 2 * j + 1 : 0][0] : (half_t)0.f, two ? (half_t)s[t][two ? 2 * j + 1 : 0][1] : (half_t)0.f,
-                                  two ? (half_t)s[t][two ? 2 * j + 1 : 0][2] : (half_t)0.f, two ? (half_t)s[t][two ? 2 * j + 1 : 0][3] : (half_t)0.f};
-                }
-            }
-#pragma unroll
-            for (int n = 0; n < NO; ++n)
-#pragma unroll
-                for (int j = 0; j < NJ; ++j) {
-                    const int r0 = 16 * (2 * j) + 4 * g + (li >> 2), r1 = r0 + 16;
-                    const int cc = 2 * n + ((li & 3) >> 1), off = (li & 1) * 4;
-                    const s4v lo = __builtin_amdgcn_ds_read_tr16_b64_v4i16(
-                        (__attribute__((address_space(3))) s4v *)(tV + r0 * HD + (cc ^ vswz<HD>(r0)) * 8 + off));
-                    const s4v hi = __builtin_amdgcn_ds_read_tr16_b64_v4i16(
-                        (__attribute__((address_space(3))) s4v *)(tV + r1 * HD + (cc ^ vswz<HD>(r1)) * 8 + off));
-                    const s8v both = s8v{lo[0], lo[1], lo[2], lo[3], hi[0], hi[1], hi[2], hi[3]};
-                    const h8 vf = __builtin_bit_cast(h8, both);
-#pragma unroll
-                    for (int t = 0; t < QT; ++t) o[t][n] = mfma16(vf, pf[t][j], o[t][n]);
-                }
-        }
+        attn_tile<HD, CAUSAL, QT, decltype(nsub_tag)::value>(sK[buf], sV[buf], qf, o, mrow, lrow, kt, kstart, kend, qw, sc, g, li);
     };
     auto run = [&](auto live_tag) {
         constexpr bool LIVE = decltype(live_tag)::value;
@@ -313,4 +318,161 @@
     return hipErrorInvalidValue;
 }
 
-}
+constexpr int GQA_WAVES = 6, GQA_THREADS = 64 * GQA_WAVES;
+template <int HD, int GP>
+__global__ __launch_bounds__(GQA_THREADS) __attribute__((amdgpu_waves_per_eu(3, 3))) void attn_prefill_gqa_kernel(AttnGqaParams p) {
+    constexpr int KS = HD / 32, NO = HD / 16, HALF = HD / 2, VPH = HD / 16, KR = KS / 2;
+    static_assert(HD == 64 || HD == 128, "the rotary partner must be a whole k-step away");
+    extern __shared__ __attribute__((aligned(16))) half_t smem[];
+    const int tid = threadIdx.x, lane = tid & 63;
+    const int wave = __builtin_amdgcn_readfirstlane(tid >> 6);
+    const int g = lane >> 4, li = lane & 15;
+    const int b = blockIdx.x / p.nkv, hk = blockIdx.x % p.nkv;
+    const int T = p.T, Tk = (T + KB - 1) / KB * KB;
+    half_t *sK = smem, *sV = smem + Tk * HD;
+    const int kstart = p.kstart[b];
+    const half_t *rows = p.qkv + (int64_t)b * T * p.ld;
+
+    {
+        constexpr int U = 3;
+        const half_t *kbase = rows + (int64_t)(p.nh + hk) * HD, *vbase = kbase + (int64_t)p.nkv * HD;
+        half_t *kc = p.kc + b * p.cache_sb + hk * p.cache_sh, *vc = p.vc + b * p.cache_sb + hk * p.cache_sh;
+        const int n_items = Tk * VPH;
+        for (int i0 = tid; i0 < n_items; i0 += GQA_THREADS * U) {
+            h8 klo[U], khi[U], vlo[U], vhi[U];
+            f4 cs[U][4];
+#pragma unroll
+            for (int u = 0; u < U; ++u) {
+                const int i = i0 + GQA_THREADS * u, r = i / VPH, v = i % VPH;
+                const h8 z = h8{0, 0, 0, 0, 0, 0, 0, 0};
+                klo[u] = khi[u] = vlo[u] = vhi[u] = z;
+#pragma unroll
+                for (int e = 0; e < 4; ++e) cs[u][e] = f4{0.f, 0.f, 0.f, 0.f};
+                if (r < T) {
+                    const int64_t off = (int64_t)r * p.ld + v * 8;
+                    klo[u] = *reinterpret_cast<const h8 *>(kbase + off);
+                    khi[u] = *reinterpret_cast<const h8 *>(kbase + off + HALF);
+                    vlo[u] = *reinterpret_cast<const h8 *>(vbase + off);
+                    vhi[u] = *reinterpret_cast<const h8 *>(vbase + off + HALF);
+                    int pos = r - kstart;
+                    pos = pos < 0 ? 0 : pos;
+                    const f4 *c4 = reinterpret_cast<const f4 *>(p.cs + ((int64_t)pos * HALF + v * 8) * 2);
+#pragma unroll
+                    for (int e = 0; e < 4; ++e) cs[u][e] = c4[e];
+                }
+            }
+#pragma unroll
+            for (int u = 0; u < U; ++u) {
+                const int i = i0 + GQA_THREADS * u, r = i / VPH, v = i % VPH;
+                if (i >= n_items) continue;
+                h8 olo = klo[u], ohi = khi[u];
+                if (r < T) {
+                    rope8_rot(klo[u], khi[u], reinterpret_cast<const float *>(cs[u]), 1.0f, olo, ohi);
+                    const int64_t co = (int64_t)r * HD + v * 8;
+                    *reinterpret_cast<h8 *>(kc + co) = olo;
+                    *reinterpret_cast<h8 *>(kc + co + HALF) = ohi;
+                    *reinterpret_cast<h8 *>(vc + co) = vlo[u];
+                    *reinterpret_cast<h8 *>(vc + co + HALF) = vhi[u];
+                }
+                *reinterpret_cast<h8 *>(sK + r * HD + kswz<HD>(r, v) * 8) = olo;
+                *reinterpret_cast<h8 *>(sK + r * HD + kswz<HD>(r, v + VPH) * 8) = ohi;
+                *reinterpret_cast<h8 *>(sV + r * HD + (v ^ vswz<HD>(r)) * 8) = vlo[u];
+                *reinterpret_cast<h8 *>(sV + r * HD + ((v + VPH) ^ vswz<HD>(r)) * 8) = vhi[u];
+            }
+        }
+    }
+    __syncthreads();
+
+    const int nqt = (T + 15) / 16, ntiles = nqt * GP;
+    const int k_lo = kstart / KB * KB;
+    const float sc = p.scale * 1.4426950408889634f;
+    h8 raw[KS];
+    f4 qcs[KR][4];
+    auto load_q = [&](int j) {
+        const int qt = j / GP, hq = j % GP;
+        int t = 16 * qt + li;
+        t = t < T ? t : T - 1;
+        const half_t *src = rows + (int64_t)t * p.ld + (int64_t)(hk * GP + hq) * HD + 8 * g;
+#pragma unroll
+        for (int s = 0; s < KS; ++s) raw[s] = *reinterpret_cast<const h8 *>(src + 32 * s);
+    };
+    auto load_cs = [&](int j) {
+        int t = 16 * (j / GP) + li;
+        t = t < T ? t : T - 1;
+        int pos = t - kstart;
+        pos = pos < 0 ? 0 : pos;
+        const f4 *c4 = reinterpret_cast<const f4 *>(p.cs + ((int64_t)pos * HALF + 8 * g) * 2);
+#pragma unroll
+        for (int s = 0; s < KR; ++s)
+#pragma unroll
+            for (int e = 0; e < 4; ++e) qcs[s][e] = c4[16 * s + e];
+    };
+    if (wave < ntiles) load_q(wave);
+    for (int j = wave; j < ntiles; j += GQA_WAVES) {
+        const int qt = j / GP, hq = j % GP, qw = 16 * qt;
+        load_cs(j);
+        h8 qf[1][KS];
+#pragma unroll
+        for (int s = 0; s < KR; ++s) rope8_rot(raw[s], raw[s + KR], reinterpret_cast<const float *>(qcs[s]), 1.0f, qf[0][s], qf[0][s + KR]);
+        if (j + GQA_WAVES < ntiles) load_q(j + GQA_WAVES);
+        f4 o[1][NO];
+        float mrow[1] = {-INFINITY}, lrow[1] = {0.f};
+#pragma unroll
+        for (int n = 0; n < NO; ++n) o[0][n] = f4{0.f, 0.f, 0.f, 0.f};
+        const int k_hi = qw + 16 < T ? qw + 16 : T;
+        int kt = k_lo;
+        for (; k_hi - kt > 32; kt += KB) attn_tile<HD, true, 1, 4>(sK + kt * HD, sV + kt * HD, qf, o, mrow, lrow, kt, kstart, T, qw, sc, g, li);
+        if (kt < k_hi) {
+            if (k_hi - kt > 16) attn_tile<HD, true, 1, 2>(sK + kt * HD, sV + kt * HD, qf, o, mrow, lrow, kt, kstart, T, qw, sc, g, li);
+            else attn_tile<HD, true, 1, 1>(sK + kt * HD, sV + kt * HD, qf, o, mrow, lrow, kt, kstart, T, qw, sc, g, li);
+        }
+        float l = lrow[0];
+        l += __shfl_xor(l, 16, 64);
+        l += __shfl_xor(l, 32, 64);
+        const int qi = qw + li;
+        if (qi < T) {
+            const float inv = l > 0.f ? 1.0f / l : 0.f;
+            half_t *dst = p.O + ((int64_t)b * T + qi) * p.o_st + (int64_t)(hk * GP + hq) * HD;
+#pragma unroll
+            for (int n = 0; n < NO; ++n)
+                *reinterpret_cast<h4 *>(dst + 16 * n + 4 * g) =
+                    h4{(half_t)(o[0][n][0] * inv), (half_t)(o[0][n][1] * inv), (half_t)(o[0][n][2] * inv), (half_t)(o[0][n][3] * inv)};
+        }
+    }
+}
+
+constexpr int GQA_LDS_BYTES = 128 * 1024;
+int attn_prefill_gqa_cap(int head_dim) { return head_dim == 64 || head_dim == 128 ? GQA_LDS_BYTES / (4 * head_dim) : 0; }
+
+template <int HD, int GP>
+static hipError_t launch_gqa(const AttnGqaParams &p, hipStream_t s) {
+    const size_t lds = (size_t)cdiv(p.T, KB) * KB * HD * 2 * sizeof(half_t);
+    hipError_t e = ensure_dyn_lds(reinterpret_cast<const void *>(&attn_prefill_gqa_kernel<HD, GP>), lds);
+    if (e != hipSuccess) return e;
+    OPUS_LAUNCH(KC_ATTN_PREFILL, (attn_prefill_gqa_kernel<HD, GP>), dim3(p.B * p.nkv), dim3(GQA_THREADS), lds, s, p);
+    return hipGetLastError();
+}
+bool attn_prefill_gqa_takes(const AttnGqaParams &p) {
+    if (g_knobs.no_prefill_attn_fusion) return false;
+    if (p.T <= 0 || p.B <= 0 || p.nkv <= 0 || p.nh % p.nkv || p.T > attn_prefill_gqa_cap(p.head_dim)) return false;
+    const int gp = p.nh / p.nkv;
+    if (gp != 1 && gp != 2 && gp != 4 && gp != 8) return false;
+    return !((p.ld & 7) || (p.o_st & 3) || (p.cache_sb & 7) || (p.cache_sh & 7));
+}
+template <int HD>
+static hipError_t launch_gqa_hd(const AttnGqaParams &p, hipStream_t s) {
+    switch (p.nh / p.nkv) {
+        case 1: return launch_gqa<HD, 1>(p, s);
+        case 2: return launch_gqa<HD, 2>(p, s);
+        case 4: return launch_gqa<HD, 4>(p, s);
+        case 8: return launch_gqa<HD, 8>(p, s);
+    }
+    return hipErrorInvalidValue;
+}
+hipError_t launch_attn_prefill_gqa(const AttnGqaParams &p, hipStream_t s, bool *taken) {
+    *taken = attn_prefill_gqa_takes(p);
+    if (!*taken) return hipSuccess;
+    return p.head_dim == 64 ? launch_gqa_hd<64>(p, s) : launch_gqa_hd<128>(p, s);
+}
+
+}
diff --git a/opus-pllm_amd/csrc/common.h b/opus-pllm_amd/csrc/common.h
--- a/opus-pllm_amd/csrc/common.h
+++ b/opus-pllm_amd/csrc/common.h
@@ -68,6 +68,18 @@
     lo = __builtin_fmaf(a, c, -__fmul_rn(b, sn));
     hi = __builtin_fmaf(b, c, __fmul_rn(a, sn));
     asm volatile("" : "+v"(lo), "+v"(hi));
+}
+
+__device__ __forceinline__ void rope8_rot(h8 lo, h8 hi, const float *cs, float scale, h8 &olo, h8 &ohi) {
+#pragma unroll
+    for (int j = 0; j < 8; ++j) {
+        const float c = cs[2 * j], sn = cs[2 * j + 1];
+        const float a = (float)lo[j] * scale, b = (float)hi[j] * scale;
+        float rl, rh;
+        rotate_pair(a, b, c, sn, rl, rh);
+        olo[j] = (half_t)rl;
+        ohi[j] = (half_t)rh;
+    }
 }
 
 __host__ __device__ __forceinline__ int64_t tiled_off(int row, int k, int K) {
@@ -216,6 +228,7 @@
     int debug_a_tiled = 0;
     int pp_gm = 8;
     int enc_full_last_layer = 0;
+    int no_prefill_attn_fusion = 0;
     int misc[8] = {0, 0, 0, 0, 0, 0, 0, 0};
 };
 extern Knobs g_knobs;
@@ -254,6 +267,21 @@
 bool gemm_goes_wide(int M, int N);
 bool gemm_goes_pp(int M, int N);
 hipError_t launch_attn_prefill(const AttnParams &p, hipStream_t s);
+struct AttnGqaParams {
+    const half_t *qkv;
+    int64_t ld;
+    const float *cs;
+    const int32_t *kstart;
+    half_t *kc, *vc;
+    int64_t cache_sb, cache_sh;
+    half_t *O;
+    int64_t o_st;
+    int B, T, nh, nkv, head_dim;
+    float scale;
+};
+int attn_prefill_gqa_cap(int head_dim);
+bool attn_prefill_gqa_takes(const AttnGqaParams &p);
+hipError_t launch_attn_prefill_gqa(const AttnGqaParams &p, hipStream_t s, bool *taken);
 int attn_prefill_query_tiles(const AttnParams &p);
 struct AttnPrefixParams {
     const half_t *kc, *vc;
diff --git a/opus-pllm_amd/csrc/elementwise.hip b/opus-pllm_amd/csrc/elementwise.hip
--- a/opus-pllm_amd/csrc/elementwise.hip
+++ b/opus-pllm_amd/csrc/elementwise.hip
@@ -63,15 +63,7 @@
     h8 lo = *reinterpret_cast<h8 *>(base);
     h8 hi = *reinterpret_cast<h8 *>(base + half);
     h8 olo, ohi;
-#pragma unroll
-    for (int j = 0; j < 8; ++j) {
-        const float c = cs[2 * j], sn = cs[2 * j + 1];
-        const float a = (float)lo[j] * scale, b = (float)hi[j] * scale;
-        float rl, rh;
-        rotate_pair(a, b, c, sn, rl, rh);
-        olo[j] = (half_t)rl;
-        ohi[j] = (half_t)rh;
-    }
+    rope8_rot(lo, hi, cs, scale, olo, ohi);
     *reinterpret_cast<h8 *>(base) = olo;
     *reinterpret_cast<h8 *>(base + half) = ohi;
 }
diff --git a/opus-pllm_amd/csrc/gemm.hip b/opus-pllm_amd/csrc/gemm.hip
--- a/opus-pllm_amd/csrc/gemm.hip
+++ b/opus-pllm_amd/csrc/gemm.hip
@@ -15,6 +15,7 @@
         snprintf(name, sizeof(name), "OPUS_KNOB_MISC%d", i);
         if (const char *v = getenv(name)) k.misc[i] = atoi(v);
     }
+    if (const char *v = getenv("OPUS_NO_PREFILL_ATTN_FUSION")) k.no_prefill_attn_fusion = atoi(v);
     return k;
 }
 Knobs g_knobs = knobs_from_env();
```
